# TencentARC/ViT-Lens

Measured on AMD Instinct MI355X. Metric: modality-pairs/sec (ViT-L, 224^2 patches), higher is better.
Workload: dtype bf16; 1 GPU; C3: ViT-L Lens(depth)->ViT + image + text tri-modal InfoNCE TRAINING step (fwd+bwd+AdamW), batch 1024/GPU in micro-batches of 256, first 4 blocks + adapter trainable; global_batch=1024, residual_dtype=bf16, accumulate=fp32, parallelism=dp1, gemm_cfg=-1, via=step, text_tower_operands=fp16, layernorm=folded into the GEMMs (frozen blocks), frozen_towers=second HIP stream beside the trainable tower's forward, backward=two halves of the micro-batches on two HIP streams

## Files before the change

include/vitlens_hip.h:

```cpp
#ifndef VITLENS_HIP_H
#define VITLENS_HIP_H

#include <stdint.h>

#ifdef __cplusplus
extern "C" {
#endif

#ifndef __HIP_PLATFORM_AMD__
typedef struct ihipStream_t* hipStream_t;
#endif

#define VL_EPI_BF16 0
#define VL_EPI_F32 1
#define VL_EPI_RES_F32 2
#define VL_EPI_RES_BF16 3
#define VL_EPI_GEGLU 5
#define VL_EPI_DGELU 6
#define VL_EPI_DGEGLU 7
#define VL_ACT_NONE 0
#define VL_ACT_GELU 1
#define VL_ACT_RELU 2
#define VL_ACT_GELU_DSAVE 4
#define VL_ACT_QGELU 5
#define VL_ACT_QGELU_DSAVE 6

#define VL_F32 0
#define VL_BF16 1
#define VL_F16 2

#define VL_GEMM_AUTO (-1)
#define VL_GEMM_PERSIST 8
#define VL_GEMM_PINGPONG 10

const char* vl_last_error(void);
#define VL_ABI_VERSION 607
int vl_version(void);

int vl_gemm_bf16(const void* A, const void* W, const float* bias, void* out, const void* res,
                 int M, int N, int K, int lda, int ldw, int ldo, float alpha, int epi, int act,
                 int cfg, hipStream_t stream);

int vl_gemm_splitk_accum_f32(const void* A, const void* W, float* out, int M, int N, int K, int lda, int ldw, long ldo,
                             float alpha, int splits, float* ws, hipStream_t stream);
int vl_gemm_tn_splitk_accum_f32(const void* At, const void* Bt, float* out, int M, int N, int K, int lda, int ldb, long ldo,
                                float alpha, int splits, float* ws, hipStream_t stream);
int vl_gemm_bf16_ex(const void* A, const void* W, const float* bias, void* out, const void* res, void* out2,
                    int M, int N, int K, int lda, int ldw, int ldo, float alpha, int epi, int act,
                    int res_div, int cfg, hipStream_t stream);

int vl_gemm_f16(const void* A, const void* W, const float* bias, void* out, const void* res, int M, int N, int K,
                int lda, int ldw, int ldo, float alpha, int epi, int act, hipStream_t stream);
int vl_attn_fwd_f16(const void* q, const void* k, const void* v, const long* strides, void* out, float* lse,
                    int B, int H, int Lq, int Lk, int dh, float qscale, int causal, hipStream_t stream);

int vl_gemm_f32(const float* A, const float* W, const float* bias, float* out, const float* res, int M, int N, int K,
                int lda, int ldw, int ldo, float alpha, int act, hipStream_t stream);
int vl_attn_fwd_f32(const float* q, const float* k, const float* v, const long* strides, float* out, float* lse,
                    int B, int H, int Lq, int Lk, int dh, float scale, int causal, hipStream_t stream);
int vl_im2col_f32(const float* x, float* patches, int N, int C, int H, int W, int kh, int kw, int sh, int sw,
                  int Kp, int transpose_hw, hipStream_t stream);
int vl_gemm_f32_ex(const float* A, const float* W, const float* bias, float* out, const float* res, int M, int N, int K,
                   int lda, int ldw, int ldo, float alpha, int act, int res_div, int res_pre, int geglu, hipStream_t stream);
int vl_knn_group_f32(const float* xyz, const int64_t* center_idx, int* nidx, float* patches, int B, int N, int G,
                     int k, int Kp, hipStream_t stream);
int vl_group_max_f32(const float* x, long ldx, float* out, long ldo, long groups, int M, int C, hipStream_t stream);
int vl_pad3_f32(const float* c, float* out, long R, int Kp, hipStream_t stream);

int vl_device_info(int device, char* arch, int arch_len, int* cus, int* clock_khz, long* hbm_bytes);

int vl_attn_fwd_bf16(const void* q, const void* k, const void* v, const long* strides, void* out, float* lse,
                     int B, int H, int Lq, int Lk, int dh, float qscale, int causal, hipStream_t stream);

int vl_gemm_main_rows(int M, int N);
int vl_gemm_lnfold_bf16(const void* A, const void* Wg, const float* bias_f, const float* ln_c, const float* ln_mean,
                        const float* ln_rstd, void* out, void* out2, int M, int N, int K, int lda, int ldw, int ldo, int act,
                        hipStream_t stream);
int vl_gemm_res_rowstats_bf16(const void* A, const void* W, const float* bias, void* out, const void* res, float* row_part,
                              int M, int N, int K, int lda, int ldw, int ldo, hipStream_t stream);
int vl_ln_row_stats(const float* row_part, int P, const void* x_bf16, long x_row_stride, int D, int m_main, int rows, float eps,
                    float* mean, float* rstd, const float* ln_w, const float* ln_b, void* y_left, long y_row_stride, int y_row0,
                    hipStream_t stream);

int vl_layernorm_fwd(const void* x, int x_dtype, long x_row_stride, const int64_t* row_index, long row_mul,
                     const float* w, const float* b, void* y, int y_dtype, long y_row_stride,
                     float* mean, float* rstd, int rows, int D, float eps, hipStream_t stream);

int vl_assemble_ln_pre(const void* tokens, int tok_dtype, const float* cls, const float* pos, const float* pos2,
                       const float* w, const float* b, void* y, int y_dtype, float* xpre, float* mean, float* rstd,
                       int B, int T, int D, float eps, hipStream_t stream);

int vl_l2_normalize(const float* x, float* y, void* y_bf16, float* norms, int rows, int D, float eps,
                    hipStream_t stream);
int vl_l2_normalize_bwd(const float* f, const float* df, const float* norms, float* dx, int rows, int D, float eps,
                        hipStream_t stream);

int vl_im2col_bf16(const float* x, void* patches, int N, int C, int H, int W, int kh, int kw, int sh, int sw,
                   int Kp, int transpose_hw, hipStream_t stream);

int vl_text_embed(const int64_t* ids, const float* tok_emb, const float* pos, void* out, int out_dtype,
                  int B, int L, int D, int vocab, hipStream_t stream);

int vl_cast_f32_bf16(const float* x, void* y, long n, hipStream_t stream);
int vl_add_rows(const void* x, int x_dtype, const float* table, void* y, int y_dtype, long rows, int T, int D,
                hipStream_t stream);
int vl_transpose_to_bf16(const void* in, int in_dtype, long ldi, int R, int C, void* out, long ldo, hipStream_t stream);
int vl_transpose_colsum_bf16(const void* in, int in_dtype, long ldi, int R, int C, void* out, long ldo,
                             float* colsum_out, float colsum_scale, float* ws, hipStream_t stream);

int vl_split_bf16x3(const float* x, void* out, long rows, int D, int pattern, hipStream_t stream);
int vl_ce_stats(const float* logits, long ld, int R, int C, int label_off, float* row_lse, float* col_lse,
                float* diag, float* col_ws, hipStream_t stream);
int vl_ce_loss_accum(const float* row_lse, const float* col_lse, const float* diag, int R, int C, int label_off,
                     float w_row, float w_col, float* loss_inout, hipStream_t stream);
int vl_ce_grad(const float* logits, long ld, int R, int C, int label_off, const float* row_lse, const float* col_lse,
               float w_row, float w_col, void* G, long ldg, void* GT, long ldgt, float logit_scale,
               float* dscale_inout, float* ws, hipStream_t stream);
long vl_ce_grad_ws_floats(int R, int C, long ldg, long ldgt);
int vl_ce_stats_masked(const float* logits, long ld, int R, int C, int label_off, float* row_lse, float* col_lse,
                       float* diag, float* col_ws, const float* sim, long ld_sim, float thres, hipStream_t stream);
int vl_ce_grad_masked(const float* logits, long ld, int R, int C, int label_off, const float* row_lse, const float* col_lse,
                      float w_row, float w_col, void* G, long ldg, void* GT, long ldgt, float logit_scale,
                      float* dscale_inout, float* ws, const float* sim, long ld_sim, float thres, hipStream_t stream);

int vl_layernorm_bwd(const void* dy, int dy_dtype, long dy_stride, const void* x, int x_dtype, long x_stride,
                     const float* mean, const float* rstd, const float* w, const float* dres, float* dx,
                     void* dx_bf16, long dx_stride, int rows, int D, hipStream_t stream);
int vl_layernorm_bwd_g(const void* dy, int dy_dtype, long dy_stride, const void* x, int x_dtype, long x_stride,
                       const float* mean, const float* rstd, const float* w, const void* dres, void* dx, int g_dtype,
                       void* dx_bf16, long dx_stride, int rows, int D, hipStream_t stream);
int vl_layernorm_bwd_sres(const void* dy, int dy_dtype, long dy_stride, const void* x, int x_dtype, long x_stride,
                          const float* mean, const float* rstd, const float* w, const void* dres, int dres_every,
                          long dres_stride, void* dx, int g_dtype, void* dx_bf16, long dx_stride, int rows, int D,
                          hipStream_t stream);
long vl_colreduce_ws_floats(int rows, int cols, int planes);
int vl_layernorm_bwd_params(const void* dy, int dy_dtype, long dy_stride, const void* x, int x_dtype, long x_stride,
                            const float* mean, const float* rstd, float* dw, float* db, int rows, int D,
                            float* ws, hipStream_t stream);
int vl_colsum(const void* a, int a_dtype, long lda, float* out, int rows, int cols, float scale, float* ws, hipStream_t stream);
int vl_gelu_bf16(const void* u, void* y, long n, hipStream_t stream);
int vl_geglu_bf16(const void* h, void* y, long rows, int n_out, hipStream_t stream);
int vl_attn_bwd_bf16(const void* q, const void* k, const void* v, const void* dO, const void* o, const long* strides,
                     const float* lse, float* delta, void* dq, void* dk, void* dv, long ld_dq, long ld_dkv,
                     int B, int H, int Lq, int Lk, int dh, float qscale, int causal, float scale, hipStream_t stream);
int vl_attn_bwd_fused_supported(int Lq, int Lk, int dh, int causal);
int vl_attn_bwd_fused_bf16(const void* q, const void* k, const void* v, const void* dO, const void* o, const long* strides,
                           const float* lse, void* dq, void* dk, void* dv, long ld_dq, long ld_dkv, int B, int H, int L, int dh,
                           float qscale, float scale, hipStream_t stream);
int vl_attn_fwd_q1(const void* q, const void* k, const void* v, const long* strides, void* out, long ld_out, float* lse,
                   int B, int H, int L, int dh, int qrow, float qscale, hipStream_t stream);
int vl_attn_bwd_q1(const void* q, const void* k, const void* v, const long* strides, const void* dO, long ld_do,
                   const void* o, long ld_o, const float* lse, void* dq, void* dk, void* dv, long ld_dq, long ld_dkv,
                   int B, int H, int L, int dh, int qrow, float qscale, float scale, hipStream_t stream);
int vl_kaldi_fbank(const float* wave, long wave_stride, int batch, long n_samples, const float* window, const float* banks,
                   float* out, int target_len, int win, int shift, int nfft, int nmel, float preemph, float mean, float std,
                   hipStream_t stream);
int vl_resample_sinc(const float* in, long in_stride, int batch, long n_in, const int* offsets, const float* taps, int o, int n,
                     int K, float* out, long out_stride, long out_first, long n_out, hipStream_t stream);
int vl_fbank_augment(const float* in, float* out, int batch, int T, int F, const void* params, float mean, float std,
                     hipStream_t stream);
int vl_fps(const float* xyz, const int64_t* start, int64_t* idx, float* centers, int B, int N, int G, hipStream_t stream);
int vl_pc_gather_normalize(const float* pts, const int64_t* idx, float* out, int B, int N, int G, int C, hipStream_t stream);
int vl_resample_h_u8(const uint8_t* src, long row_stride, int W, int C, int row0, int nrows, const int* bounds,
                     const int* kk, int ksize, int xout0, int nxout, uint8_t* dst, hipStream_t stream);
int vl_resample_v_u8_norm(const uint8_t* src, int W, int C, int row0, int nrows, const int* bounds, const int* kk,
                          int ksize, int yout0, int nyout, const float* mean, const float* stdv, float* out,
                          uint8_t* out_u8, hipStream_t stream);
int vl_resample_batch_u8_norm(const int64_t* desc, int n, int C, int crop_h, int crop_w, int max_nrows, const int* tables,
                              uint8_t* tmp, const float* mean, const float* stdv, float* out, hipStream_t stream);
int vl_resample_h_f32(const float* src, long row_stride, int W, int row0, int nrows, const int* bounds,
                      const float* weights, int ksize, int xout0, int nxout, int clamp_on, float clamp_lo,
                      float clamp_hi, float divide_by, float* dst, hipStream_t stream);
int vl_resample_v_f32_norm(const float* src, int W, int H, int row0, const int* bounds, const float* weights, int ksize,
                           int yout0, int nyout, float mean, float stdv, float* out, hipStream_t stream);
int vl_knn_group(const float* xyz, const int64_t* center_idx, int* nidx, void* patches, int B, int N, int G,
                 int k, int Kp, hipStream_t stream);
int vl_ball_group(const float* xyz, const float* feats, const int64_t* center_idx, int* idx, void* patches, int B, int N,
                  int S, int D, float radius2, int nsample, int Kp, hipStream_t stream);
int vl_group_max(const void* x, long ldx, void* out, int out_dtype, long ldo, long groups, int M, int C, hipStream_t stream);
int vl_pad3_bf16(const float* c, void* out, long R, int Kp, hipStream_t stream);
int vl_bn_stats(const void* x, long ldx, int R, int C, float* ws, int nchunk, float* mean, float* var,
                float* running_mean, float* running_var, float momentum, hipStream_t stream);
int vl_bn_stats_local(const void* x, long ldx, int R, int C, float* ws, int nchunk, float* local, hipStream_t stream);
int vl_bn_stats_merge(const float* gathered, int W, int C, float* mean, float* var, float* running_mean,
                      float* running_var, float momentum, int* total, hipStream_t stream);
int vl_bn_bwd_reduce(const void* dy, long lddy, const void* x, long ldx, const float* mean, const float* var,
                     const float* gamma, const float* beta, float eps, int relu, float* ws, int nchunk, float* dgamma,
                     float* dbeta, float* sums, int R, int C, hipStream_t stream);
int vl_bn_bwd_apply(const void* dy, long lddy, const void* x, long ldx, const float* mean, const float* var,
                    const float* gamma, const float* beta, float eps, int relu, const float* sums, const int* total,
                    void* dx, long lddx, int R, int C, hipStream_t stream);
int vl_bn_apply(const void* x, long ldx, const float* mean, const float* var, const float* gamma, const float* beta,
                float eps, int relu, void* out, long ldo, long R, int C, hipStream_t stream);
int vl_bn_bwd(const void* dy, long lddy, const void* x, long ldx, const float* mean, const float* var,
              const float* gamma, const float* beta, float eps, int relu, int train, float* ws, int nchunk,
              float* dgamma, float* dbeta, void* dx, long lddx, int R, int C, hipStream_t stream);
int vl_group_max_bwd(const void* f, long ldf, const void* dg, long lddg, const void* base, long ldb, void* out,
                     long ldo, long groups, int M, int C, hipStream_t stream);
int vl_group_sum(const void* x, long ldx, void* out, long ldo, long groups, int M, int C, hipStream_t stream);
int vl_adamw_step(float* p, const float* g, float* m, float* v, long n, float lr, float beta1, float beta2,
                  float eps, float weight_decay, int step, float grad_scale, hipStream_t stream);
long vl_sumsq_ws_floats(void);
int vl_sumsq_f32(const float* x, long n, float* out, float* ws, hipStream_t stream);
typedef struct vl_adamw_slot {
  float* p; const float* g; float* m; float* v;
  long n;
  float weight_decay;
// ... 24 lines not shown
```

vit-lens_amd/csrc/vl_attn.hip:

```cpp
#include "vl_attn_common.h"
#include "vitlens_hip.h"

namespace {
using namespace vlattn;

constexpr int KC = 288;
constexpr int VSP = KC + 8;
constexpr int NWMAX = 8;
constexpr float RESCALE_THR = 8.0f;

struct AttnP {
  TV q, k, v;
  float qscale;
  bf16_t* out;
  float* lse;
  int B, H, Lq, Lk, causal;
  int dh;
  VL_PROF_FIELD
  int lq_main;
};

template <int DH, bool TAILQ, bool MULTI, bool F16 = false, bool DMA = false>
__global__ void __launch_bounds__(NWMAX * 64, DH == 128 ? 2 : 4) attn_fwd_kernel(const AttnP p) {
  static_assert(!F16 || (!TAILQ && DH == 64), "half operands: head dim 64, no shared last row (the text tower's shape)");
  static_assert(!DMA || (DH == 64 && !MULTI && !F16), "LDS-DMA staging: head dim 64, one key chunk, bf16");
  constexpr int RB = DH * 2;
  constexpr int CH = RB / 16;
  constexpr int RSH = Rsh<DH>::v;
  constexpr bool PAD = DH == 128;
  constexpr int KS = DH / 16;
  constexpr int DT = DH / 32;
  extern __shared__ __attribute__((aligned(16))) unsigned char smem[];
  unsigned char* sK = smem;
  bf16_t* sV = (bf16_t*)(smem + KC * RB);
  float* sP = (float*)(sV + DH * VSP);
  float* sPart = sP + NWMAX * 32;
  bf16_t* sTailQ = (bf16_t*)(sPart + (KC / 32) * (2 + DH));

  const int b = blockIdx.z, h = blockIdx.y;
  const int tid = threadIdx.x, nthr = blockDim.x;
  const int lane = tid & 63;
  const int wid = __builtin_amdgcn_readfirstlane(tid >> 6);
  const int nwq = nthr >> 6;
  const int fr = lane & 31, fg = lane >> 5;
  const size_t bh = (size_t)b * p.H + h;
  const bf16_t* Kg = p.k.p + b * p.k.sb + h * p.k.sh;
  const bf16_t* Vg = p.v.p + b * p.v.sb + h * p.v.sh;
  const bf16_t* Qb = p.q.p + b * p.q.sb + h * p.q.sh;

  const int q0 = (blockIdx.x * nwq + wid) * 32;
  const bool wave_active = q0 < p.lq_main;
  int qrow = q0 + fr; if (qrow >= p.lq_main) qrow = p.lq_main - 1;
  const int qidx = q0 + fr;
  const int dhr = PAD ? p.dh : DH;
  const int nch = dhr >> 3;

  VL_PROF_STAMP(p, 0);
  u32x4 qraw[KS];
  {
    const bf16_t* Qg = Qb + (long)qrow * p.q.sr;
#pragma unroll
    for (int ks = 0; ks < KS; ++ks) {
      qraw[ks] = u32x4{0u, 0u, 0u, 0u};
      if (!PAD || ks * 2 + fg < nch) qraw[ks] = *(const u32x4*)(Qg + ks * 16 + fg * 8);
    }
  }
  [[maybe_unused]] u32x4 tailraw = {0u, 0u, 0u, 0u};
  if constexpr (TAILQ) {
    if constexpr (!PAD) tailraw = *(const u32x4*)(Qb + (long)(p.Lq - 1) * p.q.sr + (tid & (CH - 1)) * 8);
    else if (tid < nch) tailraw = *(const u32x4*)(Qb + (long)(p.Lq - 1) * p.q.sr + tid * 8);
  }
  unsigned char* const sVr = (unsigned char*)sV;
  auto vswz = [](int row) { const int x = (row >> 1) & 7; return ((x & 1) << 2) | (x >> 1); };
  if constexpr (DMA) {
    typedef __attribute__((address_space(3))) void* lds_p;
    const int nrows = ((p.Lk + 31) >> 5) << 5;
    const __amdgpu_buffer_rsrc_t rsK = __builtin_amdgcn_make_buffer_rsrc((void*)Kg, 0, 0x7ffffff0, 0x00020000);
    const __amdgpu_buffer_rsrc_t rsV = __builtin_amdgcn_make_buffer_rsrc((void*)Vg, 0, 0x7ffffff0, 0x00020000);
    for (int u = wid; u * 8 < p.Lk; u += nwq) {
      const int row = u * 8 + (lane >> 3), sl = lane & 7;
      if (row < p.Lk) {
        const unsigned offK = (unsigned)(row * (int)p.k.sr + ((sl ^ ((row >> 1) & 7)) << 3)) * 2u;
        const unsigned offV = (unsigned)(row * (int)p.v.sr + ((sl ^ vswz(row)) << 3)) * 2u;
        __builtin_amdgcn_raw_ptr_buffer_load_lds(rsK, (lds_p)(sK + u * 1024), 16, offK, 0, 0, 0);
        __builtin_amdgcn_raw_ptr_buffer_load_lds(rsV, (lds_p)(sVr + u * 1024), 16, offV, 0, 0, 0);
      }
    }
    for (int i = tid; i < (nrows - p.Lk) * 8; i += nthr)
      *(u32x4*)(sVr + (p.Lk + (i >> 3)) * 128 + ((i & 7) << 4)) = u32x4{0u, 0u, 0u, 0u};
    asm volatile("s_waitcnt vmcnt(0)" ::: "memory");
  } else {
  stage2<DH, KC, true, false, false, true>(StageSrc{sK, nullptr, Kg, p.k.sr, 1.f, nch}, StageSrc{nullptr, sV, Vg, p.v.sr, 1.f, nch},
                                           0, p.Lk, tid, nthr);
  }
  if constexpr (TAILQ) {
    if constexpr (!PAD) *(u32x4*)(sTailQ + (tid & (CH - 1)) * 8) = tailraw;
    else if (tid < CH) *(u32x4*)(sTailQ + tid * 8) = tailraw;
  }
  VL_PROF_STAMP(p, 1);
  [[maybe_unused]] const int li = lane & 15, lb3 = (li >> 3) & 1;
  [[maybe_unused]] const unsigned aTr = (unsigned)((fg * 4 + (li >> 2)) * 128) +
                                        (((unsigned)(((lane >> 4) & 1) * 2 + ((li >> 1) & 1)) ^ (unsigned)((lb3 << 2) | fg)) << 4) + (unsigned)((li & 1) << 3);
  auto trV = [&](int tile, int c, int t) {
    typedef __attribute__((ext_vector_type(4))) short s16x4;
    typedef __attribute__((address_space(3))) s16x4* lds_s16x4;
    struct { s16x4 lo, hi; } f;
    const unsigned a = (aTr + (unsigned)(tile * 4096)) ^ (unsigned)(t * 64);
    f.lo = __builtin_amdgcn_ds_read_tr16_b64_v4i16((lds_s16x4)(sVr + a + c * 2048));
    f.hi = __builtin_amdgcn_ds_read_tr16_b64_v4i16((lds_s16x4)(sVr + (a ^ 32u) + c * 2048 + 1024));
    return __builtin_bit_cast(bf16x8, f);
  };
  bf16x8 qf[KS];
#pragma unroll
  for (int ks = 0; ks < KS; ++ks)
    qf[ks] = __builtin_bit_cast(bf16x8, p.qscale != 1.0f ? scale_x8<F16>(qraw[ks], p.qscale) : qraw[ks]);

  float m_run = 0.f;
  vl_f32x2 l2 = {0.f, 0.f};
  f32x16 negm;
  f32x16 o[DT];
#pragma unroll
  for (int r = 0; r < 16; ++r) negm[r] = 0.f;
#pragma unroll
  for (int t = 0; t < DT; ++t)
#pragma unroll
    for (int r = 0; r < 16; ++r) o[t][r] = 0.f;
  bool first = true;

  auto tail_partials = [&]() {
    if constexpr (TAILQ) {
    const int qT = p.Lq - 1;
    const int ntile = (p.Lk + 31) >> 5;
    const int ksw = (fr >> RSH) & (CH - 1);
    bf16x8 qa[KS];
#pragma unroll
    for (int ks = 0; ks < KS; ++ks) {
#pragma unroll
      for (int e = 0; e < 8; ++e) qa[ks][e] = (__bf16)0.f;
      if (fr == 0) {
        u32x4 raw = *(const u32x4*)(sTailQ + ks * 16 + fg * 8);
        if (p.qscale != 1.0f) raw = scale_bf16x8(raw, p.qscale);
        qa[ks] = __builtin_bit_cast(bf16x8, raw);
      }
    }
    for (int kt = wid; kt < ntile; kt += nwq) {
      f32x16 st;
#pragma unroll
      for (int r = 0; r < 16; ++r) st[r] = 0.f;
      const unsigned char* kbase = sK + (kt * 32 + fr) * RB;
#pragma unroll
      for (int ks = 0; ks < KS; ++ks)
        st = __builtin_amdgcn_mfma_f32_32x32x16_bf16(qa[ks], *(const bf16x8*)(kbase + (((ks * 2 + fg) ^ ksw) * 16)), st, 0, 0, 0);
      const bool valid = fg == 0 && kt * 32 + fr < p.Lk;
      const float sv = valid ? st[0] : -INFINITY;
      const float mw = wave_max_dpp(sv);
      const float pw = valid ? __builtin_amdgcn_exp2f(sv - mw) : 0.f;
      const float lw = wave_sum_dpp(pw);
      float* myP = sP + wid * 32;
      if (fg == 0) myP[fr] = pw;
      __builtin_amdgcn_fence(__ATOMIC_RELEASE, "wavefront");
      __builtin_amdgcn_wave_barrier();
      __builtin_amdgcn_fence(__ATOMIC_ACQUIRE, "wavefront");
      f32x16 ot[DT];
#pragma unroll
      for (int t = 0; t < DT; ++t)
#pragma unroll
        for (int r = 0; r < 16; ++r) ot[t][r] = 0.f;
#pragma unroll
      for (int c = 0; c < 2; ++c) {
        bf16x8 pa;
#pragma unroll
        for (int e = 0; e < 8; ++e) pa[e] = (__bf16)0.f;
        if (fr == 0) {
          const f32x4 lo = *(const f32x4*)(myP + c * 16 + fg * 4);
          const f32x4 hi = *(const f32x4*)(myP + c * 16 + 8 + fg * 4);
#pragma unroll
          for (int e = 0; e < 4; ++e) { pa[e] = (__bf16)lo[e]; pa[4 + e] = (__bf16)hi[e]; }
        }
#pragma unroll
        for (int t = 0; t < DT; ++t)
          ot[t] = __builtin_amdgcn_mfma_f32_32x32x16_bf16(
              pa, DMA ? trV(kt, c, t) : *(const bf16x8*)(sV + (t * 32 + fr) * VSP + kt * 32 + c * 16 + fg * 8), ot[t], 0, 0, 0);
      }
      __builtin_amdgcn_wave_barrier();
      float* part = sPart + kt * (2 + DH);
      if (lane == 0) { part[0] = mw; part[1] = lw; }
      if (fg == 0) {
#pragma unroll
        for (int t = 0; t < DT; ++t) part[2 + t * 32 + fr] = ot[t][0];
      }
    }
    }
  };
  auto tail_merge = [&]() {
    if constexpr (TAILQ) {
      const int qT = p.Lq - 1;
      const int ntile = (p.Lk + 31) >> 5;
      if (wid == 0) {
        float M = -INFINITY;
        for (int kt = 0; kt < ntile; ++kt) M = fmaxf(M, sPart[kt * (2 + DH)]);
        for (int d = lane; d < dhr; d += 64) {
          float L = 0.f, acc = 0.f;
          for (int kt = 0; kt < ntile; ++kt) {
            const float* part = sPart + kt * (2 + DH);
            const float w = __builtin_amdgcn_exp2f(part[0] - M);
            L = fmaf(part[1], w, L);
            acc = fmaf(part[2 + d], w, acc);
          }
          p.out[((size_t)b * p.Lq + qT) * (p.H * dhr) + h * dhr + d] = f2bf(acc / L);
          if (p.lse && d == 0) p.lse[bh * p.Lq + qT] = (M + __log2f(L)) * 0.6931471805599453f;
        }
      }
    }
  };
  const int q_hi = q0 + 31;
  const int blk_q_hi = min(p.lq_main - 1, (int)(blockIdx.x * nwq + nwq) * 32 - 1);

  for (int kc0 = 0; kc0 < (MULTI ? p.Lk : 1); kc0 += KC) {
    if (MULTI && p.causal && kc0 > blk_q_hi) break;
    if constexpr (MULTI) {
      if (kc0 > 0) {
        __syncthreads();
        stage2<DH, KC, true, false, false, true, 1>(StageSrc{sK, nullptr, Kg, p.k.sr, 1.f, nch},
                                                    StageSrc{nullptr, sV, Vg, p.v.sr, 1.f, nch}, kc0, p.Lk, tid, nthr);
      }
    }
    __syncthreads();
    VL_PROF_STAMP(p, 2);
    if constexpr (TAILQ) { tail_partials(); __syncthreads(); }
    if (!wave_active) continue;

    int ntile = (min(p.Lk - kc0, KC) + 31) >> 5;
    if (p.causal) ntile = min(ntile, ((q_hi - kc0) >> 5) + 1);
    const int ksw = (fr >> RSH) & (CH - 1);
    for (int kt = 0; kt < ntile; ++kt) {
      const unsigned char* kbase = sK + (kt * 32 + fr) * RB;
      bf16x8 kf[KS];
#pragma unroll
      for (int ks = 0; ks < KS; ++ks) kf[ks] = *(const bf16x8*)(kbase + (((ks * 2 + fg) ^ ksw) * 16));
      f32x16 s = mfma32<F16>(kf[0], qf[0], negm);
#pragma unroll
      for (int ks = 1; ks < KS; ++ks) s = mfma32<F16>(kf[ks], qf[ks], s);
      bf16x8 vf0[DT];
#pragma unroll
      for (int t = 0; t < DT; ++t) {
        if constexpr (DMA) vf0[t] = trV(kt, 0, t);
        else vf0[t] = *(const bf16x8*)(sV + (t * 32 + fr) * VSP + kt * 32 + fg * 8);
      }
      const int key0 = kc0 + kt * 32 + fg * 4;
      const bool need_mask = (key0 - fg * 4 + 32 > p.Lk) || (p.causal && key0 - fg * 4 + 31 > q0);
      if (need_mask) {
#pragma unroll
        for (int r = 0; r < 16; ++r) {
          const int key = key0 + (r & 3) + 8 * (r >> 2);
          if (key >= p.Lk || (p.causal && key > qidx)) s[r] = -INFINITY;
        }
      }
      float mx = fmaxf(fmaxf(s[0], s[1]), s[2]);
#pragma unroll
      for (int r = 3; r < 15; r += 2) mx = fmaxf(fmaxf(mx, s[r]), s[r + 1]);
      mx = fmaxf(mx, s[15]);
      mx = xhalf_max(mx);
      if (__builtin_amdgcn_ballot_w64(first || mx > RESCALE_THR) != 0) {
        const float d = first ? mx : fmaxf(mx, 0.f);
        const float alpha = first ? 0.f : __builtin_amdgcn_exp2f(-d);
        m_run += d;
#pragma unroll
        for (int r = 0; r < 16; ++r) { s[r] -= d; negm[r] -= d; }
#pragma unroll
        for (int t = 0; t < DT; ++t)
#pragma unroll
          for (int r = 0; r < 16; ++r) o[t][r] *= alpha;
        l2 *= alpha;
        first = false;
      }
      float pv[16];
#pragma unroll
      for (int r = 0; r < 16; ++r) pv[r] = __builtin_amdgcn_exp2f(s[r]);
      {
        vl_f32x2 a0 = {pv[0], pv[1]}, a1 = {pv[2], pv[3]}, a2 = {pv[4], pv[5]}, a3 = {pv[6], pv[7]};
        const vl_f32x2 a4 = {pv[8], pv[9]}, a5 = {pv[10], pv[11]}, a6 = {pv[12], pv[13]}, a7 = {pv[14], pv[15]};
        a0 += a4; a1 += a5; a2 += a6; a3 += a7;
        a0 += a2; a1 += a3;
        l2 += a0 + a1;
      }
      bf16x8 vf1[DT];
#pragma unroll
      for (int t = 0; t < DT; ++t) {
        if constexpr (DMA) vf1[t] = trV(kt, 1, t);
        else vf1[t] = *(const bf16x8*)(sV + (t * 32 + fr) * VSP + kt * 32 + 16 + fg * 8);
      }
      {
        const bf16x8 pf = pack8x<F16>(pv);
#pragma unroll
        for (int t = 0; t < DT; ++t) o[t] = mfma32<F16>(vf0[t], pf, o[t]);
      }
      {
        const bf16x8 pf = pack8x<F16>(pv + 8);
#pragma unroll
        for (int t = 0; t < DT; ++t) o[t] = mfma32<F16>(vf1[t], pf, o[t]);
      }
    }
  }

  VL_PROF_STAMP(p, 3);
  if (wave_active) {
    const float l_tot = xhalf_sum(l2[0] + l2[1]);
    const float inv = 1.0f / l_tot;
    store_rows_t<DT, F16>(o, inv, p.out + ((size_t)b * p.Lq + qrow) * (p.H * dhr) + h * dhr, fg, qidx < p.lq_main, nch);
    if (p.lse && fg == 0 && qidx < p.lq_main)
      p.lse[bh * p.Lq + qidx] = (m_run + __log2f(l_tot)) * 0.6931471805599453f;
  }

  VL_PROF_STAMP(p, 4);
  tail_merge();
  VL_PROF_STAMP(p, 5);
}

}

extern "C" int vl_set_error(const char* msg);

template <int DH, bool TAILQ, bool MULTI, bool F16 = false, bool DMA = false>
static int launch_fwd(const AttnP& p, int gx, int nwq, hipStream_t stream) {
  const size_t smem = (size_t)KC * DH * 2 + (size_t)DH * VSP * 2 + (size_t)NWMAX * 32 * 4 + (size_t)(KC / 32) * (2 + DH) * 4 +
                      (size_t)DH * 2;
  static const hipError_t attr = hipFuncSetAttribute((const void*)attn_fwd_kernel<DH, TAILQ, MULTI, F16, DMA>,
                                                     hipFuncAttributeMaxDynamicSharedMemorySize, (int)smem);
  if (attr != hipSuccess) return vl_set_error(hipGetErrorString(attr));
  hipLaunchKernelGGL((attn_fwd_kernel<DH, TAILQ, MULTI, F16, DMA>), dim3(gx, p.H, p.B), dim3(nwq * 64), smem, stream, p);
  const hipError_t e = hipGetLastError();
  return e == hipSuccess ? 0 : vl_set_error(hipGetErrorString(e));
}

extern "C" int vl_attn_fwd_bf16(const void* q, const void* k, const void* v, const long* strides, void* out, float* lse,
                                int B, int H, int Lq, int Lk, int dh, float qscale, int causal, hipStream_t stream) {
  if (B <= 0 || H <= 0 || Lq <= 0 || Lk <= 0) return vl_set_error("vl_attn_fwd_bf16: empty problem");
  if (dh != 32 && dh != 64 && !(dh > 64 && dh <= 128 && (dh & 7) == 0))
    return vl_set_error("vl_attn_fwd_bf16: head dim must be 32, 64, or a multiple of 8 in (64, 128] (run zero-padded to 128)");
  if (!strides) return vl_set_error("vl_attn_fwd_bf16: strides required");
  for (int i = 0; i < 9; ++i)
    if (strides[i] & 7) return vl_set_error("vl_attn_fwd_bf16: operand strides must be multiples of 8 elements (16-byte rows)");
  if ((((uintptr_t)q) | ((uintptr_t)k) | ((uintptr_t)v)) & 15) return vl_set_error("vl_attn_fwd_bf16: operands must be 16-byte aligned");
  AttnP p{TV{(const bf16_t*)q, strides[0], strides[1], strides[2]}, TV{(const bf16_t*)k, strides[3], strides[4], strides[5]},
          TV{(const bf16_t*)v, strides[6], strides[7], strides[8]}, qscale, (bf16_t*)out, lse, B, H, Lq, Lk, causal, dh,
#ifdef VL_ATTN_PROF
          vl_attn_prof_buf,
#endif
          Lq};
  const bool tailq = (Lq % 32 == 1) && Lq > 32 && Lq - 1 <= NWMAX * 32 && Lk <= KC && (!causal || Lk <= Lq);
  if (tailq) p.lq_main = Lq - 1;
  const int qtiles = (p.lq_main + 31) / 32;
  const int nwq = qtiles < NWMAX ? qtiles : NWMAX;
  const int gx = (qtiles + nwq - 1) / nwq;
  const bool multi = Lk > KC;
#define VL_FWD(DHV)                                                                  \
  (tailq ? launch_fwd<DHV, true, false>(p, gx, nwq, stream)                          \
         : (multi ? launch_fwd<DHV, false, true>(p, gx, nwq, stream) : launch_fwd<DHV, false, false>(p, gx, nwq, stream)))
  if (dh == 64 && !multi)
    return tailq ? launch_fwd<64, true, false, false, true>(p, gx, nwq, stream) : launch_fwd<64, false, false, false, true>(p, gx, nwq, stream);
  return dh == 64 ? VL_FWD(64) : (dh == 32 ? VL_FWD(32) : VL_FWD(128));
#undef VL_FWD
}

extern "C" int vl_attn_fwd_f16(const void* q, const void* k, const void* v, const long* strides, void* out, float* lse,
                               int B, int H, int Lq, int Lk, int dh, float qscale, int causal, hipStream_t stream) {
  if (B <= 0 || H <= 0 || Lq <= 0 || Lk <= 0) return vl_set_error("vl_attn_fwd_f16: empty problem");
  if (dh != 64) return vl_set_error("vl_attn_fwd_f16: head dim must be 64");
  if (Lk > KC) return vl_set_error("vl_attn_fwd_f16: at most 288 keys");
  if (!strides) return vl_set_error("vl_attn_fwd_f16: strides required");
  for (int i = 0; i < 9; ++i)
    if (strides[i] & 7) return vl_set_error("vl_attn_fwd_f16: operand strides must be multiples of 8 elements (16-byte rows)");
  if ((((uintptr_t)q) | ((uintptr_t)k) | ((uintptr_t)v)) & 15) return vl_set_error("vl_attn_fwd_f16: operands must be 16-byte aligned");
  AttnP p{TV{(const bf16_t*)q, strides[0], strides[1], strides[2]}, TV{(const bf16_t*)k, strides[3], strides[4], strides[5]},
          TV{(const bf16_t*)v, strides[6], strides[7], strides[8]}, qscale, (bf16_t*)out, lse, B, H, Lq, Lk, causal, dh,
#ifdef VL_ATTN_PROF
          vl_attn_prof_buf,
#endif
          Lq};
  const int qtiles = (Lq + 31) / 32;
  const int nwq = qtiles < NWMAX ? qtiles : NWMAX;
  const int gx = (qtiles + nwq - 1) / nwq;
  return launch_fwd<64, false, false, true>(p, gx, nwq, stream);
}
```

vit-lens_amd/csrc/vl_attn_common.h:

```cpp
#pragma once
#include "vl_common.h"

#ifdef VL_ATTN_PROF
extern "C" long* vl_attn_prof_buf;
#define VL_PROF_FIELD long* prof;
#define VL_PROF_STAMP(p, i)                                                                                    \
  do {                                                                                                         \
    if ((p).prof && threadIdx.x == 0)                                                                          \
      (p).prof[((blockIdx.z * gridDim.y + blockIdx.y) * gridDim.x + blockIdx.x) * 8 + (i)] = __builtin_amdgcn_s_memtime(); \
  } while (0)
#else
#define VL_PROF_FIELD
#define VL_PROF_STAMP(p, i) do { } while (0)
#endif

namespace vlattn {

struct TV {
  const bf16_t* p;
  long sb, sh, sr;
};

__device__ __forceinline__ int vpos16(int j) { return (j & 3) | ((j & 4) << 1) | ((j & 8) >> 1); }

__device__ __forceinline__ u32x4 scale_bf16x8(u32x4 v, float s) {
#pragma unroll
  for (int e = 0; e < 4; ++e)
    v[e] = pack2bf(bf2f((bf16_t)(v[e] & 0xffffu)) * s, bf2f((bf16_t)(v[e] >> 16)) * s);
  return v;
}

template <bool F16>
__device__ __forceinline__ u32x4 scale_x8(u32x4 v, float s) {
  if constexpr (F16) {
#pragma unroll
    for (int e = 0; e < 4; ++e) v[e] = pack2h(h2f((uint16_t)(v[e] & 0xffffu)) * s, h2f((uint16_t)(v[e] >> 16)) * s);
    return v;
  } else {
    return scale_bf16x8(v, s);
  }
}
template <bool F16>
__device__ __forceinline__ f32x16 mfma32(bf16x8 a, bf16x8 b, f32x16 c) {
  if constexpr (F16) return __builtin_amdgcn_mfma_f32_32x32x16_f16(__builtin_bit_cast(f16x8, a), __builtin_bit_cast(f16x8, b), c, 0, 0, 0);
  else return __builtin_amdgcn_mfma_f32_32x32x16_bf16(a, b, c, 0, 0, 0);
}

struct StageSrc {
  unsigned char* rows;
  bf16_t* t;
  const bf16_t* src;
  long sr;
  float scale;
  int nch = 0;
};

template <int DH> struct Rsh { static constexpr int v = DH == 32 ? 2 : (DH == 64 ? 1 : 0); };

template <int DH, int NR, bool ROWS, bool TRANS>
__device__ __forceinline__ void stage_write(const StageSrc& m, int i, u32x4 a, u32x4 bq) {
  constexpr int RB = DH * 2, CH = RB / 16, RSH = Rsh<DH>::v, TS = NR + 8;
  const int rp = i / CH, c = i % CH;
  const int rl = 2 * rp;
  if (m.scale != 1.0f) { a = scale_bf16x8(a, m.scale); bq = scale_bf16x8(bq, m.scale); }
  if constexpr (ROWS) {
    *(u32x4*)(m.rows + rl * RB + ((c ^ ((rl >> RSH) & (CH - 1))) * 16)) = a;
    *(u32x4*)(m.rows + (rl + 1) * RB + ((c ^ (((rl + 1) >> RSH) & (CH - 1))) * 16)) = bq;
  }
  if constexpr (TRANS) {
    unsigned int* dst = (unsigned int*)(m.t + (c * 8) * TS + (rl & ~15) + vpos16(rl & 15));
#pragma unroll
    for (int w = 0; w < 4; ++w) {
      dst[(2 * w) * (TS / 2)] = (a[w] & 0xffffu) | (bq[w] << 16);
      dst[(2 * w + 1) * (TS / 2)] = (a[w] >> 16) | (bq[w] & 0xffff0000u);
    }
  }
}

template <int DH, int NR, bool ROWS0, bool TRANS0, bool ROWS1, bool TRANS1, int U = 3>
__device__ __forceinline__ void stage2(const StageSrc& m0, const StageSrc& m1, int row0, int L, int tid, int nthr) {
  constexpr int CH = DH / 8, NP = (NR / 2) * CH;
  for (int base = 0; base < NP; base += U * nthr) {
    u32x4 a0[U], b0[U], a1[U], b1[U];
#pragma unroll
    for (int u = 0; u < U; ++u) {
      const int i = base + u * nthr + tid;
      const int rp = i / CH, c = i % CH;
      const int row = row0 + 2 * rp;
      const u32x4 z = {0u, 0u, 0u, 0u};
      a0[u] = z; b0[u] = z; a1[u] = z; b1[u] = z;
      const unsigned o0 = ((unsigned)row * (unsigned)m0.sr + c * 8) * 2u, o1 = ((unsigned)row * (unsigned)m1.sr + c * 8) * 2u;
      const bool cok = DH != 128 || c < m0.nch;
      if (i < NP && row < L && cok) {
        a0[u] = *(const u32x4*)((const unsigned char*)m0.src + o0);
        a1[u] = *(const u32x4*)((const unsigned char*)m1.src + o1);
      }
      if (i < NP && row + 1 < L && cok) {
        b0[u] = *(const u32x4*)((const unsigned char*)m0.src + (o0 + (unsigned)m0.sr * 2u));
        b1[u] = *(const u32x4*)((const unsigned char*)m1.src + (o1 + (unsigned)m1.sr * 2u));
      }
    }
#pragma unroll
    for (int u = 0; u < U; ++u) {
      const int i = base + u * nthr + tid;
      if (i >= NP) continue;
      stage_write<DH, NR, ROWS0, TRANS0>(m0, i, a0[u], b0[u]);
      stage_write<DH, NR, ROWS1, TRANS1>(m1, i, a1[u], b1[u]);
    }
  }
}

__device__ __forceinline__ float xhalf_max(float v) {
  const unsigned u = __builtin_bit_cast(unsigned, v);
  auto r = __builtin_amdgcn_permlane32_swap(u, u, false, false);
  const unsigned lo = r[0], hi = r[1];
  return fmaxf(__builtin_bit_cast(float, lo), __builtin_bit_cast(float, hi));
}
__device__ __forceinline__ float xhalf_sum(float v) {
  const unsigned u = __builtin_bit_cast(unsigned, v);
  auto r = __builtin_amdgcn_permlane32_swap(u, u, false, false);
  const unsigned lo = r[0], hi = r[1];
  return __builtin_bit_cast(float, lo) + __builtin_bit_cast(float, hi);
}
template <int CTRL>
__device__ __forceinline__ float dpp_f(float v) {
  return __builtin_bit_cast(float, __builtin_amdgcn_update_dpp(0, __builtin_bit_cast(int, v), CTRL, 0xf, 0xf, true));
}
__device__ __forceinline__ float lane_f(float v, int lane) {
  return __builtin_bit_cast(float, __builtin_amdgcn_readlane(__builtin_bit_cast(int, v), lane));
}
__device__ __forceinline__ float wave_max_dpp(float v) {
  v = fmaxf(v, dpp_f<0xB1>(v)); v = fmaxf(v, dpp_f<0x4E>(v)); v = fmaxf(v, dpp_f<0x141>(v)); v = fmaxf(v, dpp_f<0x140>(v));
  return fmaxf(fmaxf(lane_f(v, 0), lane_f(v, 16)), fmaxf(lane_f(v, 32), lane_f(v, 48)));
}
__device__ __forceinline__ float wave_sum_dpp(float v) {
  v += dpp_f<0xB1>(v); v += dpp_f<0x4E>(v); v += dpp_f<0x141>(v); v += dpp_f<0x140>(v);
  return (lane_f(v, 0) + lane_f(v, 16)) + (lane_f(v, 32) + lane_f(v, 48));
}

template <int DT, bool F16 = false>
__device__ __forceinline__ void store_rows_t(const f32x16* acc, float mul, bf16_t* dst, int fg, bool valid, int npiece = 4 * DT) {
  auto pk = [](float a, float b) { if constexpr (F16) return pack2h(a, b); else return pack2bf(a, b); };
#pragma unroll
  for (int t = 0; t < DT; ++t)
#pragma unroll
    for (int pp = 0; pp < 2; ++pp) {
      unsigned ev[2], od[2];
#pragma unroll
      for (int j = 0; j < 2; ++j) {
        ev[j] = pk(acc[t][(2 * pp) * 4 + 2 * j] * mul, acc[t][(2 * pp) * 4 + 2 * j + 1] * mul);
        od[j] = pk(acc[t][(2 * pp + 1) * 4 + 2 * j] * mul, acc[t][(2 * pp + 1) * 4 + 2 * j + 1] * mul);
      }
      auto r0 = __builtin_amdgcn_permlane32_swap(ev[0], od[0], false, false);
      auto r1 = __builtin_amdgcn_permlane32_swap(ev[1], od[1], false, false);
      const unsigned w0 = r0[0], w1 = r1[0], w2 = r0[1], w3 = r1[1];
      const u32x4 w = {w0, w1, w2, w3};
      if (valid && t * 4 + 2 * pp + fg < npiece) *(u32x4*)(dst + t * 32 + (2 * pp + fg) * 8) = w;
    }
}

template <int DH>
__device__ __forceinline__ bf16x8 frag_rows(const unsigned char* base, int row, int ks, int fg) {
  constexpr int RB = DH * 2, CH = RB / 16, RSH = Rsh<DH>::v;
  return *(const bf16x8*)(base + row * RB + (((ks * 2 + fg) ^ ((row >> RSH) & (CH - 1))) * 16));
}
template <int NR>
__device__ __forceinline__ bf16x8 frag_t(const bf16_t* base, int d, int tile, int c, int fg) {
  return *(const bf16x8*)(base + d * (NR + 8) + tile * 32 + c * 16 + fg * 8);
}

__device__ __forceinline__ f32x16 zero16() {
  f32x16 z;
#pragma unroll
  for (int r = 0; r < 16; ++r) z[r] = 0.f;
  return z;
}
__device__ __forceinline__ bf16x8 zero_bf8() {
  bf16x8 z;
#pragma unroll
  for (int e = 0; e < 8; ++e) z[e] = (__bf16)0.f;
  return z;
}
__device__ __forceinline__ bf16x8 pack8(const float* v) {
  bf16x8 r;
#pragma unroll
  for (int e = 0; e < 8; ++e) r[e] = (__bf16)v[e];
  return r;
}
template <bool F16>
__device__ __forceinline__ bf16x8 pack8x(const float* v) {
  if constexpr (F16) {
    f16x8 r;
#pragma unroll
    for (int e = 0; e < 8; ++e) r[e] = (_Float16)v[e];
    return __builtin_bit_cast(bf16x8, r);
  } else {
    return pack8(v);
  }
}
__device__ __forceinline__ float dot8(bf16x8 a, bf16x8 b, float acc) {
#pragma unroll
  for (int e = 0; e < 8; ++e) acc = fmaf((float)a[e], (float)b[e], acc);
  return acc;
}

}
```

vit-lens_amd/vitlens_hip/_lib.py:

```python
import ctypes as C
import os

_HERE = os.path.dirname(os.path.abspath(__file__))
_LIB = None


class LibraryNotBuilt(ImportError):
    pass


def lib_path() -> str:
    return os.path.join(_HERE, "libvitlens_hip.so")


P, I, L, F = C.c_void_p, C.c_int, C.c_long, C.c_float

ABI_VERSION = 607

SIGNATURES = {
    "vl_version": [],
    "vl_device_info": [I, C.c_char_p, I, C.POINTER(I), C.POINTER(I), C.POINTER(L)],
    "vl_gemm_bf16": [P, P, P, P, P, I, I, I, I, I, I, F, I, I, I, P],
    "vl_gemm_splitk_accum_f32": [P, P, P, I, I, I, I, I, L, F, I, P, P],
    "vl_gemm_tn_splitk_accum_f32": [P, P, P, I, I, I, I, I, L, F, I, P, P],
    "vl_attn_fwd_bf16": [P, P, P, P, P, P, I, I, I, I, I, F, I, P],
    "vl_gemm_f16": [P, P, P, P, P, I, I, I, I, I, I, F, I, I, P],
    "vl_gemm_f32": [P, P, P, P, P, I, I, I, I, I, I, F, I, P],
    "vl_attn_fwd_f32": [P, P, P, P, P, P, I, I, I, I, I, F, I, P],
    "vl_im2col_f32": [P, P, I, I, I, I, I, I, I, I, I, I, P],
    "vl_gemm_f32_ex": [P, P, P, P, P, I, I, I, I, I, I, F, I, I, I, I, P],
    "vl_knn_group_f32": [P, P, P, P, I, I, I, I, I, P],
    "vl_group_max_f32": [P, L, P, L, L, I, I, P],
    "vl_pad3_f32": [P, P, L, I, P],
    "vl_attn_fwd_f16": [P, P, P, P, P, P, I, I, I, I, I, F, I, P],
    "vl_layernorm_fwd": [P, I, L, P, L, P, P, P, I, L, P, P, I, I, F, P],
    "vl_gemm_main_rows": [I, I],
    "vl_gemm_lnfold_bf16": [P, P, P, P, P, P, P, P, I, I, I, I, I, I, I, P],
    "vl_gemm_res_rowstats_bf16": [P, P, P, P, P, P, I, I, I, I, I, I, P],
    "vl_ln_row_stats": [P, I, P, L, I, I, I, F, P, P, P, P, P, L, I, P],
    "vl_assemble_ln_pre": [P, I, P, P, P, P, P, P, I, P, P, P, I, I, I, F, P],
    "vl_l2_normalize": [P, P, P, P, I, I, F, P],
    "vl_l2_normalize_bwd": [P, P, P, P, I, I, F, P],
    "vl_im2col_bf16": [P, P, I, I, I, I, I, I, I, I, I, I, P],
    "vl_text_embed": [P, P, P, P, I, I, I, I, I, P],
    "vl_cast_f32_bf16": [P, P, L, P],
    "vl_add_rows": [P, I, P, P, I, L, I, I, P],
    "vl_transpose_to_bf16": [P, I, L, I, I, P, L, P],
    "vl_transpose_colsum_bf16": [P, I, L, I, I, P, L, P, F, P, P],
    "vl_split_bf16x3": [P, P, L, I, I, P],
    "vl_ce_stats": [P, L, I, I, I, P, P, P, P, P],
    "vl_ce_loss_accum": [P, P, P, I, I, I, F, F, P, P],
    "vl_ce_grad": [P, L, I, I, I, P, P, F, F, P, L, P, L, F, P, P, P],
    "vl_ce_grad_ws_floats": [I, I, L, L],
    "vl_ce_stats_masked": [P, L, I, I, I, P, P, P, P, P, L, F, P],
    "vl_ce_grad_masked": [P, L, I, I, I, P, P, F, F, P, L, P, L, F, P, P, P, L, F, P],
    "vl_gemm_bf16_ex": [P, P, P, P, P, P, I, I, I, I, I, I, F, I, I, I, I, P],
    "vl_kaldi_fbank": [P, L, I, L, P, P, P, I, I, I, I, I, F, F, F, P],
    "vl_resample_sinc": [P, L, I, L, P, P, I, I, I, P, L, L, L, P],
    "vl_fbank_augment": [P, P, I, I, I, P, F, F, P],
    "vl_fps": [P, P, P, P, I, I, I, P],
    "vl_pc_gather_normalize": [P, P, P, I, I, I, I, P],
    "vl_resample_h_u8": [P, L, I, I, I, I, P, P, I, I, I, P, P],
    "vl_resample_v_u8_norm": [P, I, I, I, I, P, P, I, I, I, P, P, P, P, P],
    "vl_resample_batch_u8_norm": [P, I, I, I, I, I, P, P, P, P, P, P],
    "vl_resample_h_f32": [P, L, I, I, I, P, P, I, I, I, I, F, F, F, P, P],
    "vl_resample_v_f32_norm": [P, I, I, I, P, P, I, I, I, F, F, P, P],
    "vl_knn_group": [P, P, P, P, I, I, I, I, I, P],
    "vl_ball_group": [P, P, P, P, P, I, I, I, I, F, I, I, P],
    "vl_group_max": [P, L, P, I, L, L, I, I, P],
    "vl_pad3_bf16": [P, P, L, I, P],
    "vl_bn_stats": [P, L, I, I, P, I, P, P, P, P, F, P],
    "vl_bn_stats_local": [P, L, I, I, P, I, P, P],
    "vl_bn_stats_merge": [P, I, I, P, P, P, P, F, P, P],
    "vl_bn_bwd_reduce": [P, L, P, L, P, P, P, P, F, I, P, I, P, P, P, I, I, P],
    "vl_bn_bwd_apply": [P, L, P, L, P, P, P, P, F, I, P, P, P, L, I, I, P],
    "vl_bn_apply": [P, L, P, P, P, P, F, I, P, L, L, I, P],
    "vl_bn_bwd": [P, L, P, L, P, P, P, P, F, I, I, P, I, P, P, P, L, I, I, P],
    "vl_group_max_bwd": [P, L, P, L, P, L, P, L, L, I, I, P],
    "vl_group_sum": [P, L, P, L, L, I, I, P],
    "vl_layernorm_bwd": [P, I, L, P, I, L, P, P, P, P, P, P, L, I, I, P],
    "vl_layernorm_bwd_g": [P, I, L, P, I, L, P, P, P, P, P, I, P, L, I, I, P],
    "vl_layernorm_bwd_sres": [P, I, L, P, I, L, P, P, P, P, I, L, P, I, P, L, I, I, P],
    "vl_colreduce_ws_floats": [I, I, I],
    "vl_layernorm_bwd_params": [P, I, L, P, I, L, P, P, P, P, I, I, P, P],
    "vl_colsum": [P, I, L, P, I, I, F, P, P],
    "vl_gelu_bf16": [P, P, L, P],
    "vl_geglu_bf16": [P, P, L, I, P],
    "vl_attn_bwd_bf16": [P, P, P, P, P, P, P, P, P, P, P, L, L, I, I, I, I, I, F, I, F, P],
    "vl_attn_bwd_fused_supported": [I, I, I, I],
    "vl_attn_bwd_fused_bf16": [P, P, P, P, P, P, P, P, P, P, L, L, I, I, I, I, F, F, P],
    "vl_attn_fwd_q1": [P, P, P, P, P, L, P, I, I, I, I, I, F, P],
    "vl_attn_bwd_q1": [P, P, P, P, P, L, P, L, P, P, P, P, L, L, I, I, I, I, I, F, F, P],
    "vl_adamw_step": [P, P, P, P, L, F, F, F, F, F, I, F, P],
    "vl_sumsq_ws_floats": [],
    "vl_sumsq_f32": [P, L, P, P, P],
    "vl_adamw_multi_step": [P, I, F, F, F, F, I, F, F, P, P, P],
    "vl_clamp_scalar": [P, F, F, P],
    "vl_axpy_f32": [P, P, F, L, P],
    "vl_scale_exp_f32": [P, P, L, P, F, P],
    "vl_batch_rowsum": [P, P, I, I, I, L, L, P],
    "vl_comm_unique_id": [P],
    "vl_comm_create": [C.POINTER(P), P, I, I],
    "vl_comm_destroy": [P],
    "vl_allgather_embed": [P, P, P, L, P],
    "vl_reducescatter_grad": [P, P, P, L, P],
    "vl_allreduce_grad": [P, P, L, P],
}


_RET = {"vl_colreduce_ws_floats": L, "vl_ce_grad_ws_floats": L, "vl_sumsq_ws_floats": L}


def load_library():
    global _LIB
    if _LIB is not None:
        return _LIB
    path = lib_path()
    if not os.path.exists(path):
        raise LibraryNotBuilt(
            f"{path} is missing: build it with `python -c 'import __graft_entry__ as g; g.build()'` "
            "or `make -C vit-lens_amd/csrc` (hipcc --offload-arch=gfx950). No CPU/eager fallback exists.")
    lib = C.CDLL(path)
    lib.vl_last_error.restype = C.c_char_p
    lib.vl_last_error.argtypes = []
    for name, args in SIGNATURES.items():
        fn = getattr(lib, name)
        fn.argtypes = args
        fn.restype = _RET.get(name, I)
    got = int(lib.vl_version())
    if got != ABI_VERSION:
        raise RuntimeError(f"{path} reports ABI version {got}, this binding was written for {ABI_VERSION} "
                           "(include/vitlens_hip.h: VL_ABI_VERSION): rebuild the library (`make -C vit-lens_amd/csrc`)")
    _LIB = lib
    return lib


def check(status: int):
    if status != 0:
        raise RuntimeError("libvitlens_hip: " + load_library().vl_last_error().decode())
```

vit-lens_amd/vitlens_hip/engine.py:

```python
from dataclasses import dataclass
from typing import Dict, Optional

import os

import torch

from . import ops


@dataclass
class TowerCfg:
    width: int = 1024
    layers: int = 24
    heads: int = 16
    mlp_ratio: float = 4.0
    patch: int = 14
    image_size: int = 224
    embed_dim: int = 768
    in_chans: int = 3
    quick_gelu: bool = False


@dataclass
class TextCfg:
# ... 104 lines not shown

def run_blocks(blocks, ws: _Workspace, B, L, D, H, causal=False, cfg=-1, fold=None, quick_gelu=False, pooled_only=False):
    dh = D // H
    prune = prune_last_ok(D, H, ws.x.dtype, L, pooled_only, causal)
    act = ops.mlp_act(quick_gelu)
    res_epi = ops.EPI_RES_F32 if ws.x.dtype == torch.float32 else ops.EPI_RES_BF16
    if fold is None:
        fold = LN_FOLD
    can_fold = bool(fold) and ws.x.dtype == torch.bfloat16 and ws.part is not None
    folded = [can_fold and "in_f" in w for w in blocks]
    mm = 0
    r_in = r_fc = 0
    if any(folded):
        r_in, r_fc = ops.fold_rows(ws.x, ws.qkv, 3 * D), ops.fold_rows(ws.x, ws.hid, ws.hid.shape[1])
    for i, w in enumerate(blocks):
        nxt = i + 1 < len(blocks) and folded[i + 1]
        pruned = prune and i + 1 == len(blocks)
        if folded[i]:
            k_in = dict(ln_w=w["ln1_w"], ln_b=w["ln1_b"], h_left=ws.h, h_row0=r_in) if mm <= r_in else {}
            ops.ln_row_stats(ws.part, ws.x, mm, ws.mean, ws.rstd, **k_in)
            ops.gemm_lnfold(ws.x, w["in_f"], ws.mean, ws.rstd, ws.qkv, w["in_w"], w["in_b"], w["ln1_w"], w["ln1_b"], ws.h, cfg=cfg,
                            h_ready=bool(k_in))
            if pruned:
                _pooled_block_tail(w, ws, B, L, D, H, act, cfg)
                break
            ops.attn_fwd(ws.q, ws.k, ws.v, ws.a, causal=causal, qscale=dh ** -0.5 * ops.LOG2E)
            mm = ops.gemm_res_rowstats(ws.a, w["out_w"], w["out_b"], ws.x, ws.x, ws.part, cfg=cfg)
            k_fc = dict(ln_w=w["ln2_w"], ln_b=w["ln2_b"], h_left=ws.h, h_row0=r_fc) if mm <= r_fc else {}
            ops.ln_row_stats(ws.part, ws.x, mm, ws.mean, ws.rstd, **k_fc)
            ops.gemm_lnfold(ws.x, w["fc_f"], ws.mean, ws.rstd, ws.hid, w["fc_w"], w["fc_b"], w["ln2_w"], w["ln2_b"], ws.h,
                            act=act, cfg=cfg, h_ready=bool(k_fc))
        else:
            ops.layernorm(ws.x, w["ln1_w"], w["ln1_b"], ws.h, B * L, D)
            ops.gemm(ws.h, w["in_w"], w["in_b"], out=ws.qkv, epi=ops.EPI_BF16, cfg=cfg)
            if pruned:
                _pooled_block_tail(w, ws, B, L, D, H, act, cfg)
                break
            ops.attn_fwd(ws.q, ws.k, ws.v, ws.a, causal=causal, qscale=dh ** -0.5 * ops.LOG2E)
            ops.gemm(ws.a, w["out_w"], w["out_b"], out=ws.x, res=ws.x, epi=res_epi, cfg=cfg)
            ops.layernorm(ws.x, w["ln2_w"], w["ln2_b"], ws.h, B * L, D)
            ops.gemm(ws.h, w["fc_w"], w["fc_b"], out=ws.hid, epi=ops.EPI_BF16, act=act, cfg=cfg)
        if nxt:
            mm = ops.gemm_res_rowstats(ws.hid, w["proj_w"], w["proj_b"], ws.x, ws.x, ws.part, cfg=cfg)
        else:
            ops.gemm(ws.hid, w["proj_w"], w["proj_b"], out=ws.x, res=ws.x, epi=res_epi, cfg=cfg)
            mm = 0


def _hi_lo(w: torch.Tensor, device):
    w = w.detach().float().to(device)
    hi = w.bfloat16()
    lo = (w - hi.float()).bfloat16()
    return hi.contiguous(), lo.contiguous()


def prep_block_wsplit(sd: Dict[str, torch.Tensor], p: str, device) -> Dict[str, torch.Tensor]:
    blk = prep_block(sd, p, device)
    for key, name in (("in_w", "attn.in_proj_weight"), ("fc_w", "mlp.c_fc.weight")):
        hi, lo = _hi_lo(sd[p + name], device)
        blk[key + "2"] = torch.cat([hi, lo], dim=1).contiguous()
    for key, name in (("out_w", "attn.out_proj.weight"), ("proj_w", "mlp.c_proj.weight")):
        blk[key], blk[key + "_lo"] = _hi_lo(sd[p + name], device)
    return blk


def run_blocks_wsplit(blocks, ws: "_Workspace", B, L, D, H, causal=False, cfg=-1, quick_gelu=False):
    dh = D // H
    act = ops.mlp_act(quick_gelu)
    h2 = ws.h2
    for w in blocks:
        ops.layernorm(ws.x, w["ln1_w"], w["ln1_b"], h2[:, :D], B * L, D)
        ops.layernorm(ws.x, w["ln1_w"], w["ln1_b"], h2[:, D:], B * L, D)
        ops.gemm(h2, w["in_w2"], w["in_b"], out=ws.qkv, epi=ops.EPI_BF16, cfg=cfg)
        ops.attn_fwd(ws.q, ws.k, ws.v, ws.a, causal=causal, qscale=dh ** -0.5 * ops.LOG2E)
        ops.gemm(ws.a, w["out_w"], w["out_b"], out=ws.x, res=ws.x, epi=ops.EPI_RES_F32, cfg=cfg)
        ops.gemm(ws.a, w["out_w_lo"], None, out=ws.x, res=ws.x, epi=ops.EPI_RES_F32, cfg=cfg)
        ops.layernorm(ws.x, w["ln2_w"], w["ln2_b"], h2[:, :D], B * L, D)
        ops.layernorm(ws.x, w["ln2_w"], w["ln2_b"], h2[:, D:], B * L, D)
        ops.gemm(h2, w["fc_w2"], w["fc_b"], out=ws.hid, epi=ops.EPI_BF16, act=act, cfg=cfg)
        ops.gemm(ws.hid, w["proj_w"], w["proj_b"], out=ws.x, res=ws.x, epi=ops.EPI_RES_F32, cfg=cfg)
        ops.gemm(ws.hid, w["proj_w_lo"], None, out=ws.x, res=ws.x, epi=ops.EPI_RES_F32, cfg=cfg)


class VitEngine:

    def __init__(self, sd, prefix: str, cfg: TowerCfg, device, res_dtype=torch.float32, gemm_cfg: int = -1,
                 n_tokens: Optional[int] = None):
        self.cfg, self.device, self.res_dtype, self.gemm_cfg = cfg, torch.device(device), res_dtype, gemm_cfg
        self.prefix = prefix
        D = cfg.width
        self.cls = _dev(sd[prefix + "class_embedding"], device)
        self.pos = _dev(sd[prefix + "positional_embedding"], device)
        self.T = self.pos.shape[0] - 1
        self.ln_pre = (_dev(sd[prefix + "ln_pre.weight"], device), _dev(sd[prefix + "ln_pre.bias"], device))
        self.ln_post = (_dev(sd[prefix + "ln_post.weight"], device), _dev(sd[prefix + "ln_post.bias"], device))
        self.projT = _dev(sd[prefix + "proj"].t(), device, torch.bfloat16) if prefix + "proj" in sd else None
        self.blocks = [prep_block(sd, f"{prefix}transformer.resblocks.{i}.", device) for i in range(cfg.layers)]
        self.conv_w = None
        if prefix + "conv1.weight" in sd:
            self.conv_w = conv_weight_as_gemm(sd[prefix + "conv1.weight"], device)
        self._ws = {}

    def update_params(self, sd, names):
        p, dev = self.prefix, self.device
        top = {n for n in names if not n.startswith("transformer.resblocks.")}
        if "class_embedding" in top:
            self.cls.copy_(sd[p + "class_embedding"])
        if "positional_embedding" in top:
            self.pos.copy_(sd[p + "positional_embedding"])
        for nm, pair in (("ln_pre", self.ln_pre), ("ln_post", self.ln_post)):
            if nm + ".weight" in top or nm + ".bias" in top:
                pair[0].copy_(sd[p + nm + ".weight"]); pair[1].copy_(sd[p + nm + ".bias"])
        if "proj" in top and self.projT is not None:
            self.projT.copy_(sd[p + "proj"].t())
        if "conv1.weight" in top and self.conv_w is not None:
            self.conv_w.copy_(conv_weight_as_gemm(sd[p + "conv1.weight"], dev))
        for l in sorted({int(n.split(".")[2]) for n in names if n.startswith("transformer.resblocks.")}):
            copy_tree(self.blocks[l], prep_block(sd, f"{p}transformer.resblocks.{l}.", dev))

    def workspace(self, B, L):
        key = (B, L)
        if key not in self._ws:
            self._ws[key] = _Workspace(B, L, self.cfg.width, self.cfg.heads, int(self.cfg.width * self.cfg.mlp_ratio),
                                       self.device, self.res_dtype)
        return self._ws[key]

    def patch_tokens(self, image: torch.Tensor) -> torch.Tensor:
        p = self.cfg.patch
        cols, gh, gw = ops.im2col(image.contiguous().float(), p, p, p, p, self.conv_w.shape[1])
        return ops.gemm(cols, self.conv_w, None, epi=ops.EPI_BF16, cfg=self.gemm_cfg)

    def trunk(self, tokens: torch.Tensor, B: int, pos2: Optional[torch.Tensor] = None, use_orig_pos=True):
        cfg = self.cfg
        D, T = cfg.width, tokens.shape[0] // B
        L = T + 1
        ws = self.workspace(B, L)
        pos = self.pos if use_orig_pos else torch.zeros_like(self.pos)
        ops.assemble_ln_pre(tokens, self.cls, pos, pos2, self.ln_pre[0], self.ln_pre[1], ws.x, B, T, D)
        run_blocks(self.blocks, ws, B, L, D, cfg.heads, causal=False, cfg=self.gemm_cfg, quick_gelu=cfg.quick_gelu, pooled_only=True)
        pooled = torch.empty(B, D, device=self.device, dtype=torch.bfloat16)
        if self.projT is None:
            pooled = torch.empty(B, D, device=self.device, dtype=torch.float32)
        ops.layernorm(ws.x, self.ln_post[0], self.ln_post[1], pooled, B, D, x_row_stride=L * D)
        if self.projT is None:
            return pooled
        return ops.gemm(pooled, self.projT, None, epi=ops.EPI_F32, cfg=self.gemm_cfg)

    def encode_image(self, image: torch.Tensor, normalize: bool = False) -> torch.Tensor:
        B = image.shape[0]
        f = self.trunk(self.patch_tokens(image), B)
        return ops.l2_normalize(f) if normalize else f


def prep_block_f16(sd: Dict[str, torch.Tensor], p: str, device) -> Dict[str, torch.Tensor]:
    hf = torch.float16
    return {
        "ln1_w": _dev(sd[p + "ln_1.weight"], device), "ln1_b": _dev(sd[p + "ln_1.bias"], device),
        "in_w": _dev(sd[p + "attn.in_proj_weight"], device, hf), "in_b": _dev(sd[p + "attn.in_proj_bias"], device),
        "out_w": _dev(sd[p + "attn.out_proj.weight"], device, hf), "out_b": _dev(sd[p + "attn.out_proj.bias"], device),
        "ln2_w": _dev(sd[p + "ln_2.weight"], device), "ln2_b": _dev(sd[p + "ln_2.bias"], device),
        "fc_w": _dev(sd[p + "mlp.c_fc.weight"], device, hf), "fc_b": _dev(sd[p + "mlp.c_fc.bias"], device),
        "proj_w": _dev(sd[p + "mlp.c_proj.weight"], device, hf), "proj_b": _dev(sd[p + "mlp.c_proj.bias"], device),
    }


class _WorkspaceF16:

    def __init__(self, B, L, D, H, device):
        hf = torch.float16
        self.rows = B * L
        self.Mp = (self.rows + 255) // 256 * 256
        self.Bp = (B + 255) // 256 * 256
        z = lambda *shape, dt=hf: torch.zeros(*shape, device=device, dtype=dt)
        self.x = z(self.Mp, D, dt=torch.float32)
        self.h, self.qkv, self.a, self.hid = z(self.Mp, D), z(self.Mp, 3 * D), z(self.Mp, D), z(self.Mp, 4 * D)
        dh = D // H
        hv = lambda i: ops.heads_view(self.qkv, B, L, H, dh, i * D)
        self.q, self.k, self.v = hv(0), hv(1), hv(2)
        self.pooled = z(self.Bp, D)


class TextEngine:

    def __init__(self, sd, cfg: TextCfg, device, res_dtype=torch.float32, gemm_cfg: int = -1, wsplit: Optional[bool] = None,
                 arith: str = "f16"):
        self.cfg, self.device, self.gemm_cfg = cfg, torch.device(device), gemm_cfg
        if wsplit is not None:
            arith = "bf16x2" if wsplit else "bf16"
        if arith not in ("f16", "bf16x2", "bf16"):
            raise ValueError(f"TextEngine: arith must be 'f16', 'bf16x2' or 'bf16', got {arith!r}")
        if arith == "f16" and (cfg.width % 256 or cfg.width < 512 or cfg.width // cfg.heads != 64 or cfg.embed_dim % 256
                               or cfg.context_length > 288):
            arith = "bf16x2"
        self.arith = arith
        self.wsplit = arith == "bf16x2"
        self.res_dtype = res_dtype if arith == "bf16" else torch.float32
        self.tok = _dev(sd["token_embedding.weight"], device)
        self.pos = _dev(sd["positional_embedding"], device)
        self.ln_final = (_dev(sd["ln_final.weight"], device), _dev(sd["ln_final.bias"], device))
        if arith == "f16":
            self.projT = _dev(sd["text_projection"].t(), device, torch.float16)
            self.blocks = [prep_block_f16(sd, f"transformer.resblocks.{i}.", device) for i in range(cfg.layers)]
        elif self.wsplit:
            hi, lo = _hi_lo(sd["text_projection"].t(), device)
            self.projT = torch.cat([hi, lo], dim=1).contiguous()
            self.blocks = [prep_block_wsplit(sd, f"transformer.resblocks.{i}.", device) for i in range(cfg.layers)]
        else:
            self.projT = _dev(sd["text_projection"].t(), device, torch.bfloat16)
            self.blocks = [_prep_block_plain(sd, f"transformer.resblocks.{i}.", device) for i in range(cfg.layers)]
        self._ws = {}

    def _encode_f16(self, text: torch.Tensor) -> torch.Tensor:
        cfg = self.cfg
        B, L = text.shape
        D, H = cfg.width, cfg.heads
        key = ("f16", B, L)
        if key not in self._ws:
            self._ws[key] = _WorkspaceF16(B, L, D, H, self.device)
        ws = self._ws[key]
        rows = ws.rows
        ops.text_embed(text, self.tok, self.pos, ws.x[:rows])
        eot = text.argmax(dim=-1).contiguous()
        qs = (D // H) ** -0.5 * ops.LOG2E
        act = ops.mlp_act(cfg.quick_gelu)
        for w in self.blocks:
            ops.layernorm(ws.x, w["ln1_w"], w["ln1_b"], ws.h, rows, D)
            ops.gemm_f16(ws.h, w["in_w"], w["in_b"], out=ws.qkv)
            ops.attn_fwd(ws.q, ws.k, ws.v, ws.a, causal=True, qscale=qs)
            ops.gemm_f16(ws.a, w["out_w"], w["out_b"], out=ws.x, res=ws.x, epi=ops.EPI_RES_F32)
            ops.layernorm(ws.x, w["ln2_w"], w["ln2_b"], ws.h, rows, D)
            ops.gemm_f16(ws.h, w["fc_w"], w["fc_b"], out=ws.hid, act=act)
            ops.gemm_f16(ws.hid, w["proj_w"], w["proj_b"], out=ws.x, res=ws.x, epi=ops.EPI_RES_F32)
        ops.layernorm(ws.x, self.ln_final[0], self.ln_final[1], ws.pooled, B, D, x_row_stride=D, row_index=eot, row_mul=L)
        f = torch.zeros(ws.Bp, self.projT.shape[0], device=self.device, dtype=torch.float32)
        ops.gemm_f16(ws.pooled, self.projT, None, out=f, res=f, epi=ops.EPI_RES_F32)
        return f[:B]

    def encode_text(self, text: torch.Tensor, normalize: bool = False) -> torch.Tensor:
        cfg = self.cfg
        B, L = text.shape
        D = cfg.width
        text = text.to(self.device).contiguous()
        if self.arith == "f16":
            f = self._encode_f16(text)
            return ops.l2_normalize(f) if normalize else f.contiguous()
        key = (B, L)
        if key not in self._ws:
            self._ws[key] = _Workspace(B, L, D, cfg.heads, 4 * D, self.device, self.res_dtype)
        ws = self._ws[key]
        ops.text_embed(text, self.tok, self.pos, ws.x)
        eot = text.argmax(dim=-1).contiguous()
        if self.wsplit:
            if not hasattr(ws, "h2"):
                ws.h2 = torch.empty(B * L, 2 * D, device=self.device, dtype=torch.bfloat16)
            run_blocks_wsplit(self.blocks, ws, B, L, D, cfg.heads, causal=True, cfg=self.gemm_cfg, quick_gelu=cfg.quick_gelu)
            pooled = torch.empty(B, 2 * D, device=self.device, dtype=torch.bfloat16)
            for half in (pooled[:, :D], pooled[:, D:]):
                ops.layernorm(ws.x, self.ln_final[0], self.ln_final[1], half, B, D, x_row_stride=D, row_index=eot, row_mul=L)
        else:
            run_blocks(self.blocks, ws, B, L, D, cfg.heads, causal=True, cfg=self.gemm_cfg, fold=False, quick_gelu=cfg.quick_gelu)
            pooled = torch.empty(B, D, device=self.device, dtype=torch.bfloat16)
            ops.layernorm(ws.x, self.ln_final[0], self.ln_final[1], pooled, B, D, x_row_stride=D, row_index=eot, row_mul=L)
        f = ops.gemm(pooled, self.projT, None, epi=ops.EPI_F32, cfg=self.gemm_cfg)
        return ops.l2_normalize(f) if normalize else f


@dataclass
class LensCfg:
    modality: str = "depth"
    perceiver_identity: bool = True
    depth: int = 2
    self_per_cross: int = 3
    num_latents: int = 256
    latent_dim: int = 1024
    input_chan: int = 1024
    cross_heads: int = 1
    cross_dim_head: int = 64
    latent_heads: int = 16
    latent_dim_head: int = 64
    audio_fstride: int = 10
    audio_tstride: int = 10
    audio_mel_bins: int = 128
    audio_target_length: int = 512
    pc_num_group: int = 512
    pc_group_size: int = 32
    pc_encoder_dims: int = 256
    pc_trans_dim: int = 384
    pc_tokenizer: str = "pointbert"
    pc_radius: float = 0.2
    pc_in_dim: int = 3
    use_orig_pos: bool = True
    disable_adapter_pos: bool = False
    eeg_chans: int = 128
    eeg_time_len: int = 512
    eeg_window_size: int = 1
    eeg_stride: int = 1
    weight_tie_layers: bool = False


def _interleave_geglu(w: torch.Tensor, b: torch.Tensor):
    half = w.shape[0] // 2
    wi = torch.stack([w[:half], w[half:]], dim=1).reshape(w.shape[0], w.shape[1])
    bi = torch.stack([b[:half], b[half:]], dim=1).reshape(-1)
    return wi, bi


def prep_lens_attn(sd, p, device, packed_self: bool):
    bf = torch.bfloat16
    d = {"to_out_w": _dev(sd[p + "to_out.weight"], device, bf), "to_out_b": _dev(sd[p + "to_out.bias"], device)}
    if packed_self:
        d["qkv_w"] = _dev(torch.cat([sd[p + "to_q.weight"], sd[p + "to_kv.weight"]], 0), device, bf)
    else:
        d["q_w"] = _dev(sd[p + "to_q.weight"], device, bf)
        d["kv_w"] = _dev(sd[p + "to_kv.weight"], device, bf)
    return d


def prep_lens_ff(sd, p, device):
    w0, b0 = _interleave_geglu(sd[p + "net.0.weight"].detach().float(), sd[p + "net.0.bias"].detach().float())
    return {"w0": _dev(w0, device, torch.bfloat16), "b0": _dev(b0, device),
            "w2": _dev(sd[p + "net.2.weight"], device, torch.bfloat16), "b2": _dev(sd[p + "net.2.bias"], device)}


class PerceiverEngine:

    def __init__(self, sd, prefix: str, cfg: LensCfg, device, gemm_cfg=-1):
        self.cfg, self.device, self.gemm_cfg = cfg, torch.device(device), gemm_cfg
        self.latents = _dev(sd[prefix + "latents"], device)
        ln = lambda q: (_dev(sd[q + ".weight"], device), _dev(sd[q + ".bias"], device))
        self.layers = []
        for i in range(cfg.depth):
            if cfg.weight_tie_layers and i >= 2:
                self.layers.append(self.layers[1])
                continue
            q = f"{prefix}layers.{i}."
            lay = {"x_norm": ln(q + "0.norm"), "x_norm_ctx": ln(q + "0.norm_context"),
                   "x_attn": prep_lens_attn(sd, q + "0.fn.", device, False),
                   "x_ff_norm": ln(q + "1.norm"), "x_ff": prep_lens_ff(sd, q + "1.fn.", device), "selfs": []}
            for j in range(cfg.self_per_cross):
                r = f"{q}2.{j}."
                lay["selfs"].append({"norm": ln(r + "0.norm"), "attn": prep_lens_attn(sd, r + "0.fn.", device, True),
                                     "ff_norm": ln(r + "1.norm"), "ff": prep_lens_ff(sd, r + "1.fn.", device)})
            self.layers.append(lay)
        self._ws = {}

    def update_params(self, sd, prefix: str):
        fresh = PerceiverEngine(sd, prefix, self.cfg, self.device, self.gemm_cfg)
        self.latents.copy_(fresh.latents)
        copy_tree(self.layers, fresh.layers)

    def _workspace(self, B, Tc):
        key = (B, Tc)
        if key in self._ws:
            return self._ws[key]
        c, dev, bf = self.cfg, self.device, torch.bfloat16
        n, D = c.num_latents, c.latent_dim
        f = lambda *s, dt=bf: torch.empty(*s, device=dev, dtype=dt)
        ws = {
            "x": f(B * n, D, dt=torch.float32), "h": f(B * n, D), "ctx": f(B * Tc, c.input_chan),
            "xq2": f(B * n, c.cross_heads * c.cross_dim_head), "xkv2": f(B * Tc, 2 * c.cross_heads * c.cross_dim_head),
            "xa": f(B * n, c.cross_heads * c.cross_dim_head),
            "sqkv2": f(B * n, 3 * c.latent_heads * c.latent_dim_head),
            "sa": f(B * n, c.latent_heads * c.latent_dim_head), "hid": f(B * n, 4 * D),
        }
        xi, si = c.cross_heads * c.cross_dim_head, c.latent_heads * c.latent_dim_head
        ws["xq"] = ops.heads_view(ws["xq2"], B, n, c.cross_heads, c.cross_dim_head)
        ws["xk"] = ops.heads_view(ws["xkv2"], B, Tc, c.cross_heads, c.cross_dim_head)
        ws["xv"] = ops.heads_view(ws["xkv2"], B, Tc, c.cross_heads, c.cross_dim_head, xi)
        for i, nm in enumerate(("sq", "sk", "sv")):
            ws[nm] = ops.heads_view(ws["sqkv2"], B, n, c.latent_heads, c.latent_dim_head, i * si)
        self._ws[key] = ws
        return ws

    def _ff(self, ws, norm, ff, rows, D):
        ops.layernorm(ws["x"], norm[0], norm[1], ws["h"], rows, D)
        ops.gemm(ws["h"], ff["w0"], ff["b0"], out=ws["hid"], epi=ops.EPI_GEGLU, cfg=self.gemm_cfg)
        ops.gemm(ws["hid"], ff["w2"], ff["b2"], out=ws["x"], res=ws["x"], epi=ops.EPI_RES_F32, cfg=self.gemm_cfg)

    def forward(self, data: torch.Tensor, B: int) -> torch.Tensor:
        c = self.cfg
        Tc, n, D = data.shape[0] // B, c.num_latents, c.latent_dim
        ws = self._workspace(B, Tc)
        ws["x"].view(B, n, D).copy_(self.latents)
        rows = B * n
        for lay in self.layers:
            a = lay["x_attn"]
            ops.layernorm(ws["x"], lay["x_norm"][0], lay["x_norm"][1], ws["h"], rows, D)
            ops.layernorm(data, lay["x_norm_ctx"][0], lay["x_norm_ctx"][1], ws["ctx"], B * Tc, c.input_chan)
            ops.gemm(ws["h"], a["q_w"], None, out=ws["xq2"], epi=ops.EPI_BF16, cfg=self.gemm_cfg)
            ops.gemm(ws["ctx"], a["kv_w"], None, out=ws["xkv2"], epi=ops.EPI_BF16, cfg=self.gemm_cfg)
            ops.attn_fwd(ws["xq"], ws["xk"], ws["xv"], ws["xa"], qscale=c.cross_dim_head ** -0.5 * ops.LOG2E)
            ops.gemm(ws["xa"], a["to_out_w"], a["to_out_b"], out=ws["x"], res=ws["x"], epi=ops.EPI_RES_F32, cfg=self.gemm_cfg)
            self._ff(ws, lay["x_ff_norm"], lay["x_ff"], rows, D)
            for sl in lay["selfs"]:
                a = sl["attn"]
                ops.layernorm(ws["x"], sl["norm"][0], sl["norm"][1], ws["h"], rows, D)
# ... 97 lines not shown
```

vit-lens_amd/vitlens_hip/ops.py:

```python
import ctypes as C
import threading

import torch

from ._lib import load_library, check

F32, BF16, F16 = 0, 1, 2
EPI_BF16, EPI_F32, EPI_RES_F32, EPI_RES_BF16, EPI_GEGLU, EPI_DGELU, EPI_DGEGLU = 0, 1, 2, 3, 5, 6, 7
ACT_NONE, ACT_GELU, ACT_RELU = 0, 1, 2
ACT_GELU_DSAVE = 4
ACT_QGELU = 5
ACT_QGELU_DSAVE = 6


def mlp_act(quick_gelu: bool, dsave: bool = False) -> int:
    if quick_gelu:
        return ACT_QGELU_DSAVE if dsave else ACT_QGELU
    return ACT_GELU_DSAVE if dsave else ACT_GELU
LOG2E = 1.4426950408889634

_lib = load_library()


def _stream():
# ... 198 lines not shown
    if mm < M:
        gemm(a[mm:], w, b, out=out[mm:], res=res[mm:], epi=EPI_RES_BF16, cfg=_leftover_cfg(M - mm, N, cfg) if mm else cfg)
    return mm


def fold_rows(x, out, N):
    return _fold_rows(x, out, N, x.shape[1])


def ln_row_stats(part, x, m_main, mean, rstd, eps=1e-5, ln_w=None, ln_b=None, h_left=None, h_row0=None):
    rows, D = x.shape
    if h_left is not None:
        if h_row0 is None or h_row0 < m_main or h_left.dtype != torch.bfloat16 or h_left.shape[0] < rows - h_row0:
            raise ValueError("ln_row_stats: h_left needs h_row0 >= m_main and a bf16 buffer of at least rows - h_row0 rows")
    check(_lib.vl_ln_row_stats(_p(part) if m_main else None, D // 64, _p(x), x.stride(0), D, m_main, rows, float(eps), _p(mean),
                               _p(rstd), _p(ln_w), _p(ln_b), _p(h_left), h_left.stride(0) if h_left is not None else 0,
                               int(h_row0 or 0), _stream()))


def logits_gemm(xb, yb, scale):
    Cn = yb.shape[0]
    Cp = (Cn + 3) // 4 * 4
    if Cp != Cn:
        yb = torch.cat([yb, torch.zeros(Cp - Cn, yb.shape[1], device=yb.device, dtype=yb.dtype)], 0)
    out = gemm(xb, yb, None, epi=EPI_F32, alpha=scale)
    return out if Cp == Cn else out[:, :Cn]


def gemm_dw(dyt, xt, g, cfg=-1, alpha=1.0):
    _chk2d(dyt, "dyt", torch.bfloat16); _chk2d(xt, "xt", torch.bfloat16); _chk2d(g, "g", torch.float32)
    M, K = dyt.shape
    N = xt.shape[0]
    nk = K // 64
    if K % 64 == 0 and M % 256 == 0 and N % 256 == 0 and nk >= 64:
        t256 = (M // 256) * (N // 256)
        for splits in (1, 2, 4, 8, 16):
            if nk % splits == 0 and t256 * splits >= 192 and nk // splits >= 16:
                ws = torch.empty(splits * M * N, device=g.device, dtype=torch.float32)
                check(_lib.vl_gemm_splitk_accum_f32(_p(dyt), _p(xt), _p(g), M, N, K, dyt.stride(0), xt.stride(0), g.stride(0),
                                                    float(alpha), splits, _p(ws), _stream()))
                return g
    tiles = ((M + 127) // 128) * ((N + 127) // 128)
    if K % 64 == 0 and tiles * 2 <= 256 and nk >= 32:
        splits = max(1, min(512 // tiles, nk // 16))
        if splits > 1:
            ws = torch.empty(splits * M * N, device=g.device, dtype=torch.float32)
            check(_lib.vl_gemm_splitk_accum_f32(_p(dyt), _p(xt), _p(g), M, N, K, dyt.stride(0), xt.stride(0), g.stride(0),
                                                float(alpha), splits, _p(ws), _stream()))
            return g
    return gemm(dyt, xt, None, out=g, res=g, epi=EPI_RES_F32, cfg=cfg, alpha=alpha)


def gemm_dw_tn(dy, x, g, alpha=1.0):
    if dy.dtype != torch.bfloat16 or x.dtype != torch.bfloat16 or g.dtype != torch.float32 or dy.dim() != 2 or x.dim() != 2:
        return False
    R, M = dy.shape
    N = x.shape[1]
    if x.shape[0] != R or R % 64 or M % 256 or N % 256 or dy.stride(1) != 1 or x.stride(1) != 1 or g.stride(1) != 1:
        return False
    if dy.stride(0) % 8 or x.stride(0) % 8 or g.stride(0) % 4 or dy.data_ptr() % 16 or x.data_ptr() % 16 or tuple(g.shape) != (M, N):
        return False
    splits = tn_splits(R // 64, (M // 256) * (N // 256))
    if not splits:
        return False
    ws = torch.empty(splits * M * N, device=g.device, dtype=torch.float32)
    check(_lib.vl_gemm_tn_splitk_accum_f32(_p(dy), _p(x), _p(g), M, N, R, dy.stride(0), x.stride(0), g.stride(0),
                                           float(alpha), splits, _p(ws), _stream()))
    return True


def tn_splits(nk: int, tiles: int, few_tiles_ok: bool = False) -> int:
    valid = lambda splits: (nk // splits >= 16 and nk - (-(-nk // (-(-nk // splits))) - 1) * (-(-nk // splits)) >= 4)
    cands = (1, 2, 4, 8, 16, 32, 64) if few_tiles_ok else (1, 2, 4, 8, 16)
    best = 0
    for splits in cands:
        if not valid(splits):
            continue
        if tiles * splits >= 192:
            return splits
        best = splits
    return best if few_tiles_ok else 0


_pad_cache = {}


def _zero_padded(t, cols, tag):
    key = (tag, t.device, torch.cuda.current_stream(t.device).cuda_stream, threading.get_ident(), t.shape[0], t.shape[1], cols)
    buf = _pad_cache.get(key)
    if buf is None:
        buf = torch.zeros(t.shape[0], cols, device=t.device, dtype=torch.bfloat16)
        _pad_cache[key] = buf
    buf[:, :t.shape[1]].copy_(t)
    return buf


def gemm_dw_tn_any(dy, x, g, alpha=1.0):
    if dy.dtype != torch.bfloat16 or x.dtype != torch.bfloat16 or g.dtype != torch.float32 or dy.dim() != 2 or x.dim() != 2:
        return False
    R, M = dy.shape
    N = x.shape[1]
    if x.shape[0] != R or R % 64 or tuple(g.shape) != (M, N) or dy.stride(1) != 1 or x.stride(1) != 1:
        return False
    Mp, Np = (M + 255) // 256 * 256, (N + 255) // 256 * 256
    if Mp == M and Np == N and gemm_dw_tn(dy, x, g, alpha):
        return True
    if dy.stride(0) % 8 or x.stride(0) % 8 or dy.data_ptr() % 16 or x.data_ptr() % 16:
        return False
    splits = tn_splits(R // 64, (Mp // 256) * (Np // 256), few_tiles_ok=True)
    if not splits:
        return False
    dyp = dy if Mp == M else _zero_padded(dy, Mp, "dy")
    xp = x if Np == N else _zero_padded(x, Np, "x")
    direct = Mp == M and Np == N and g.stride(1) == 1 and g.stride(0) % 4 == 0
    gp = g if direct else torch.zeros(Mp, Np, device=g.device, dtype=torch.float32)
    ws = torch.empty(splits * Mp * Np, device=g.device, dtype=torch.float32)
    check(_lib.vl_gemm_tn_splitk_accum_f32(_p(dyp), _p(xp), _p(gp), Mp, Np, R, dyp.stride(0), xp.stride(0), gp.stride(0),
                                           float(alpha), splits, _p(ws), _stream()))
    if not direct:
        g += gp[:M, :N]
    return True


def _bhld_strides(*views):
    import ctypes
    vals = []
    for t in views:
        if t.dim() != 4 or t.stride(3) != 1 or t.dtype != views[0].dtype or t.dtype not in (torch.bfloat16, torch.float16):
            raise ValueError("attention operands must be bf16 (or, forward only, fp16) [B,H,L,dh] views of one dtype with unit last stride")
        vals += [t.stride(0), t.stride(1), t.stride(2)]
    return (ctypes.c_long * len(vals))(*vals)


def heads_view(x2d, B, L, H, dh, col0=0):
    W = x2d.stride(0)
    return x2d.as_strided((B, H, L, dh), (L * W, dh, W, 1), x2d.storage_offset() + col0)


def attn_fwd(q, k, v, out, lse=None, causal=False, qscale=1.0):
    B, H, Lq, dh = q.shape
    Lk = k.shape[2]
    st = _bhld_strides(q, k, v)
    if q.dtype == torch.float16:
        if k.dtype != q.dtype or v.dtype != q.dtype or out.dtype != q.dtype:
            raise TypeError("attn_fwd: fp16 q needs fp16 k, v and out")
        check(_lib.vl_attn_fwd_f16(_p(q), _p(k), _p(v), st, _p(out), _p(lse), B, H, Lq, Lk, dh, float(qscale),
                                   1 if causal else 0, _stream()))
        return out
    check(_lib.vl_attn_fwd_bf16(_p(q), _p(k), _p(v), st, _p(out), _p(lse), B, H, Lq, Lk, dh, float(qscale),
                                1 if causal else 0, _stream()))
    return out


def _q1_rows(t, H, name):
    if t.dim() != 2 or t.stride(1) != 1 or t.dtype != torch.bfloat16 or t.shape[1] != H * 64:
        raise ValueError(f"{name}: need a bf16 [B, H*64] matrix with unit column stride, got {tuple(t.shape)} {t.dtype}")


def attn_fwd_q1(q, k, v, out, lse=None, qrow=0, qscale=1.0):
    B, H, L, dh = q.shape
    if k.shape != q.shape or v.shape != q.shape or q.dtype != torch.bfloat16:
        raise ValueError("attn_fwd_q1: q, k, v must be bf16 views of one [B,H,L,dh] shape (self-attention)")
    _q1_rows(out, H, "attn_fwd_q1: out")
    if out.shape[0] != B or (lse is not None and (lse.dtype != torch.float32 or not lse.is_contiguous() or lse.numel() != B * H)):
        raise ValueError("attn_fwd_q1: out must have B rows, lse must be a contiguous f32 [B, H]")
    check(_lib.vl_attn_fwd_q1(_p(q), _p(k), _p(v), _bhld_strides(q, k, v), _p(out), out.stride(0), _p(lse), B, H, L, dh,
                              int(qrow), float(qscale), _stream()))
    return out


def layernorm(x, w, b, out, rows, D, x_row_stride=None, row_index=None, row_mul=0, mean=None, rstd=None,
              eps=1e-5):
    xs = D if x_row_stride is None else x_row_stride
    check(_lib.vl_layernorm_fwd(_p(x), _dt(x), xs, _p(row_index), row_mul, _p(w), _p(b), _p(out), _dt(out),
                                out.stride(-2) if out.dim() >= 2 else D, _p(mean), _p(rstd), rows, D,
                                float(eps), _stream()))
    return out


def assemble_ln_pre(tokens, cls, pos, pos2, w, b, out, B, T, D, eps=1e-5, xpre=None, mean=None, rstd=None):
    check(_lib.vl_assemble_ln_pre(_p(tokens), _dt(tokens), _p(cls), _p(pos), _p(pos2), _p(w), _p(b), _p(out),
                                  _dt(out), _p(xpre), _p(mean), _p(rstd), B, T, D, float(eps), _stream()))
    return out


def l2_normalize(x, out=None, out_bf16=None, norms=None, eps=1e-12):
    _chk2d(x, "x", torch.float32)
    if out is None:
        out = torch.empty_like(x)
    check(_lib.vl_l2_normalize(_p(x), _p(out), _p(out_bf16), _p(norms), x.shape[0], x.shape[1], float(eps),
                               _stream()))
    return out


def l2_normalize_bwd(f, df, norms, eps=1e-12):
    dx = torch.empty_like(f)
    check(_lib.vl_l2_normalize_bwd(_p(f), _p(df), _p(norms), _p(dx), f.shape[0], f.shape[1], float(eps),
                                   _stream()))
    return dx


def im2col(x, kh, kw, sh, sw, Kp, transpose_hw=False, out=None):
    if x.dtype != torch.float32 or not x.is_contiguous():
        raise ValueError("im2col: need contiguous f32 input")
    N, Cc = x.shape[0], x.shape[1]
    H, W = (x.shape[3], x.shape[2]) if transpose_hw else (x.shape[2], x.shape[3])
    gh, gw = (H - kh) // sh + 1, (W - kw) // sw + 1
    if out is None:
        out = torch.empty(N * gh * gw, Kp, device=x.device, dtype=torch.bfloat16)
    check(_lib.vl_im2col_bf16(_p(x), _p(out), N, Cc, H, W, kh, kw, sh, sw, Kp, 1 if transpose_hw else 0,
                              _stream()))
    return out, gh, gw


def text_embed(ids, tok_emb, pos, out):
    B, L = ids.shape
    check(_lib.vl_text_embed(_p(ids), _p(tok_emb), _p(pos), _p(out), _dt(out), B, L, tok_emb.shape[1],
                             tok_emb.shape[0], _stream()))
    return out


def cast_bf16(x, out=None):
    if out is None:
        out = torch.empty(x.shape, device=x.device, dtype=torch.bfloat16)
    check(_lib.vl_cast_f32_bf16(_p(x), _p(out), x.numel(), _stream()))
    return out


def add_rows(x, table, out, rows, T, D):
    check(_lib.vl_add_rows(_p(x), _dt(x), _p(table), _p(out), _dt(out), rows, T, D, _stream()))
    return out


def transpose_to_bf16(x, ldo=None, out=None):
    _chk2d(x, "x")
    R, Cc = x.shape
    ldo = R if ldo is None else ldo
    if out is None:
        out = torch.empty(Cc, ldo, device=x.device, dtype=torch.bfloat16)
    check(_lib.vl_transpose_to_bf16(_p(x), _dt(x), x.stride(0), R, Cc, _p(out), ldo, _stream()))
    return out


def transpose_colsum(x, ldo, colsum_out=None, scale=1.0, out=None):
    _chk2d(x, "x")
    R, Cc = x.shape
    ok = Cc % 64 == 0 and ldo % 8 == 0 and x.stride(0) % 8 == 0 and R >= 256 and x.data_ptr() % 16 == 0
    if not ok:
        out = transpose_to_bf16(x, ldo=ldo, out=out)
        if colsum_out is not None:
            colsum(x, colsum_out, scale)
        return out
    if out is None:
        out = torch.empty(Cc, ldo, device=x.device, dtype=torch.bfloat16)
    ws = _ws_for(x.device, ldo, Cc, 1) if colsum_out is not None else None
    check(_lib.vl_transpose_colsum_bf16(_p(x), _dt(x), x.stride(0), R, Cc, _p(out), ldo, _p(colsum_out), float(scale), _p(ws),
                                        _stream()))
    return out


def split_bf16x3(x, pattern):
    _chk2d(x, "x", torch.float32)
    out = torch.empty(x.shape[0], 3 * x.shape[1], device=x.device, dtype=torch.bfloat16)
    check(_lib.vl_split_bf16x3(_p(x.contiguous()), _p(out), x.shape[0], x.shape[1], pattern, _stream()))
    return out


def _chk_sim(logits, sim, thres, who):
    if thres is None:
        raise ValueError(f"{who}: sim needs thres")
    if not torch.is_tensor(sim) or sim.dtype != torch.float32 or sim.dim() != 2 or tuple(sim.shape) != tuple(logits.shape):
        raise ValueError(f"{who}: sim must be an f32 tensor of the logits' shape {tuple(logits.shape)}")
    if sim.device != logits.device or sim.stride(1) != 1:
        raise ValueError(f"{who}: sim must live on the logits' device with contiguous rows")


def ce_stats(logits, label_off=0, want_cols=True, sim=None, thres=None):
    _chk2d(logits, "logits", torch.float32)
    if sim is None and thres is not None:
        raise ValueError("ce_stats: thres needs sim")
    if sim is not None:
        _chk_sim(logits, sim, thres, "ce_stats")
    R, Cc = logits.shape
    dev = logits.device
    row_lse = torch.empty(R, device=dev, dtype=torch.float32)
    diag = torch.empty(R, device=dev, dtype=torch.float32)
    col_lse = torch.empty(Cc, device=dev, dtype=torch.float32) if want_cols else None
    ws = torch.empty(2 * ((R + 63) // 64) * Cc, device=dev, dtype=torch.float32) if want_cols else None
    if sim is None:
        check(_lib.vl_ce_stats(_p(logits), logits.stride(0), R, Cc, label_off, _p(row_lse), _p(col_lse), _p(diag),
                               _p(ws), _stream()))
    else:
        check(_lib.vl_ce_stats_masked(_p(logits), logits.stride(0), R, Cc, label_off, _p(row_lse), _p(col_lse), _p(diag),
                                      _p(ws), _p(sim), sim.stride(0), float(thres), _stream()))
    return row_lse, col_lse, diag


def ce_loss_accum(loss, row_lse, col_lse, diag, R, Cc, label_off, w_row, w_col):
    check(_lib.vl_ce_loss_accum(_p(row_lse), _p(col_lse), _p(diag), R, Cc, label_off, float(w_row), float(w_col),
                                _p(loss), _stream()))


def ce_grad(logits, row_lse, col_lse, label_off, w_row, w_col, logit_scale, dscale, need_g=True, need_gt=True, sim=None,
            thres=None):
    if sim is None and thres is not None:
        raise ValueError("ce_grad: thres needs sim")
# ... 356 lines not shown
```

vit-lens_amd/vitlens_hip/step.py:

```python
import math
from typing import Dict, Optional

import torch

from . import ops
from .engine import LensCfg, LensEngine, TextCfg, TextEngine, TowerCfg, VitEngine
from .train import AdamW, DepthLensTrainer


class TorchComm:

    def all_gather(self, out: torch.Tensor, inp: torch.Tensor):
        import torch.distributed as dist
        if inp.is_cuda:
            dist.all_gather_into_tensor(out, inp)
        else:
            dist.all_gather(list(out.chunk(dist.get_world_size(), dim=0)), inp.contiguous())

    def all_reduce_sum(self, t: torch.Tensor):
        import torch.distributed as dist
        dist.all_reduce(t, op=dist.ReduceOp.SUM)

    def reduce_scatter_sum(self, out: torch.Tensor, inp: torch.Tensor):
        import torch.distributed as dist
# ... 16 lines not shown
        import ctypes as C
        from ._lib import check, load_library
        self._lib, self._check, self._C = load_library(), check, C
        self.rank, self.world = rank, world
        if device is not None:
            torch.cuda.set_device(device)
        if unique_id is None:
            if world != 1:
                raise ValueError("AbiComm: ranks > 0 need the unique id rank 0 made (AbiComm.make_unique_id / over_torch_distributed)")
            unique_id = self.make_unique_id()
        if len(unique_id) != 128:
            raise ValueError("AbiComm: the unique id is 128 bytes")
        self._h = C.c_void_p()
        buf = C.create_string_buffer(bytes(unique_id), 128)
        check(self._lib.vl_comm_create(C.byref(self._h), buf, rank, world))
        self._stream = None

    @staticmethod
    def make_unique_id() -> bytes:
        import ctypes as C
        from ._lib import check, load_library
        buf = C.create_string_buffer(128)
        check(load_library().vl_comm_unique_id(buf))
        return buf.raw

    @classmethod
    def over_torch_distributed(cls, device=None):
        import torch.distributed as dist
        rank, world = dist.get_rank(), dist.get_world_size()
        box = [cls.make_unique_id() if rank == 0 else None]
        dist.broadcast_object_list(box, src=0)
        return cls(rank, world, box[0], device)

    def close(self):
        if getattr(self, "_h", None) is not None and self._h.value:
            self._lib.vl_comm_destroy(self._h)
            self._h = self._C.c_void_p()

    def __del__(self):
        try:
            self.close()
        except Exception:
            pass

    def _s(self):
        return self._C.c_void_p(torch.cuda.current_stream().cuda_stream)

    @staticmethod
    def _f32(t, name):
        if t.dtype != torch.float32 or not t.is_contiguous() or not t.is_cuda:
            raise ValueError(f"AbiComm.{name}: contiguous fp32 GPU tensors only")
        return t

    def all_gather(self, out: torch.Tensor, inp: torch.Tensor):
        self._f32(out, "all_gather"); inp = self._f32(inp.contiguous(), "all_gather")
        self._check(self._lib.vl_allgather_embed(self._h, inp.data_ptr(), out.data_ptr(), inp.numel(), self._s()))

    def all_reduce_sum(self, t: torch.Tensor):
        self._f32(t, "all_reduce_sum")
        self._check(self._lib.vl_allreduce_grad(self._h, t.data_ptr(), t.numel(), self._s()))

    def reduce_scatter_sum(self, out: torch.Tensor, inp: torch.Tensor):
        self._f32(out, "reduce_scatter_sum"); inp = self._f32(inp.contiguous(), "reduce_scatter_sum")
        self._check(self._lib.vl_reducescatter_grad(self._h, inp.data_ptr(), out.data_ptr(), out.numel(), self._s()))

    def all_reduce_sum_async(self, t: torch.Tensor):
        self._f32(t, "all_reduce_sum_async")
        if self._stream is None:
            self._stream = torch.cuda.Stream()
        main = torch.cuda.current_stream()
        ready, done = torch.cuda.Event(), torch.cuda.Event()
        ready.record(main)
        self._stream.wait_event(ready)
        with torch.cuda.stream(self._stream):
            self.all_reduce_sum(t)
            done.record(self._stream)

        class _Handle:
            def wait(self_h):
                torch.cuda.current_stream().wait_event(done)
        return _Handle()


def _master_from_sd(name: str, sd, like: torch.Tensor) -> torch.Tensor:
    from .engine import _interleave_geglu, conv_weight_as_gemm
    dev = like.device
    f32 = lambda k: sd[k].detach().float().to(dev).clone()
    if name.endswith("conv1.weight_gemm"):
        return conv_weight_as_gemm(sd[name[:-5]], dev, torch.float32)
    if name.endswith("net.0.weight_il") or name.endswith("net.0.bias_il"):
        base = name[:name.rindex("net.0.")] + "net.0."
        w, b = _interleave_geglu(f32(base + "weight"), f32(base + "bias"))
        return (w if name.endswith("weight_il") else b).contiguous()
    if name.endswith("fn.to_qkv.weight"):
        return torch.cat([f32(name.replace("to_qkv", "to_q")), f32(name.replace("to_qkv", "to_kv"))], 0).contiguous()
    return f32(name).reshape(like.shape).contiguous()


def _master_to_sd(name: str, m: torch.Tensor, base_sd, cfg) -> Dict[str, torch.Tensor]:
    from .train import deinterleave_geglu
    if name.endswith("conv1.weight_gemm"):
        ref = base_sd[name[:-5]]
        return {name[:-5]: m[:, :ref[0].numel()].reshape(ref.shape)}
    if name.endswith("_il"):
        return {name[:-3]: deinterleave_geglu(m)}
    if name.endswith("fn.to_qkv.weight"):
        inner = cfg.latent_heads * cfg.latent_dim_head
        return {name.replace("to_qkv", "to_q"): m[:inner], name.replace("to_qkv", "to_kv"): m[inner:]}
    return {name: m.reshape(base_sd[name].shape)}


class _StepState:

    def _init_host(self, sd, device, micro_batch, rank, world_size, comm=None, local_loss=False, gather_with_grad=False,
                   force_comm=False, overlap_frozen=False, overlap_backward=True, grad_clip_norm=None):
        self.dev, self.mb, self.rank, self.world = torch.device(device), micro_batch, rank, world_size
        self._force_comm = bool(force_comm)
        self.comm = comm or TorchComm()
        self.local_loss, self.gather_with_grad = local_loss, gather_with_grad
        self.overlap_frozen = bool(overlap_frozen)
        self.overlap_backward = bool(overlap_backward)
        self._side = None
        self._base_sd = {k: v.detach() for k, v in sd.items()}
        self.logit_scale = sd["logit_scale"].detach().float().reshape(1).to(device).clone()
        self.masters: Dict[str, torch.Tensor] = {"logit_scale": self.logit_scale}
        self.bf16_targets = {}
        self.refresh = []
        self.trainers = []
        self.flat_grad, self.grads = None, {}
        self._pending, self._reduced_upto, self._reduce_done = [], None, False
        if grad_clip_norm is not None and not float(grad_clip_norm) > 0.0:
            raise ValueError(f"grad_clip_norm must be positive (or None), got {grad_clip_norm}")
        self.grad_clip_norm = None if grad_clip_norm is None else float(grad_clip_norm)
        self._sumsq = None

    @property
    def last_grad_norm(self):
        return self.opt.last_grad_norm

    def _clipped_optimizer_step(self):
        self.finish_reduce()
        if self._sumsq is None:
            self._sumsq = torch.zeros(1, device=self.dev, dtype=torch.float32)
        ops.grad_sumsq(self.flat_grad, out=self._sumsq)
        self.opt.step(self.grads, grad_scale=1.0 / self.world, max_norm=self.grad_clip_norm, sumsq=self._sumsq)

    @property
    def dist(self) -> bool:
        return self.world > 1 or self._force_comm

    @property
    def _overlap_active(self) -> bool:
        return self.overlap_frozen and self.dev.type == "cuda"

    def _side_by_side(self, beside, here):
        frozen, trainable = beside, here
        if not self._overlap_active:
            frozen(); trainable()
            return
        if self._side is None:
            self._side = torch.cuda.Stream(device=self.dev)
        main = torch.cuda.current_stream(self.dev)
        ready, done = torch.cuda.Event(), torch.cuda.Event()
        ready.record(main)
        self._side.wait_event(ready)
        with torch.cuda.stream(self._side):
            frozen()
            done.record(self._side)
        trainable()
        main.wait_event(done)

    def state_dict(self) -> Dict[str, torch.Tensor]:
        out = {k: v.detach().clone() for k, v in self._base_sd.items()}
        cfg = getattr(self.lens, "lens", None)
        for name, m in self.masters.items():
            for k, v in _master_to_sd(name, m.detach(), self._base_sd, cfg).items():
                out[k] = v.to(device=self._base_sd[k].device, dtype=self._base_sd[k].dtype).clone()
        if cfg is not None and getattr(cfg, "weight_tie_layers", False):
            P1 = "visual.perceiver.layers.1."
            for k in [k for k in out if k.startswith(P1)]:
                for li in range(2, cfg.depth):
                    out[f"visual.perceiver.layers.{li}." + k[len(P1):]] = out[k].clone()
        tok = getattr(self, "tok", None)
        if tok is not None:
            for k, (rm, rv) in tok.running.items():
                out["visual.visual_adapter." + k + ".running_mean"] = rm.detach().cpu().clone()
                out["visual.visual_adapter." + k + ".running_var"] = rv.detach().cpu().clone()
        return out

    def optimizer_state_dict(self):
        return {"step": self.opt.t, "exp_avg": {k: v.detach().clone() for k, v in self.opt.m.items()},
                "exp_avg_sq": {k: v.detach().clone() for k, v in self.opt.v.items()}}

    def load_state_dict(self, sd):
        for name, m in self.masters.items():
            m.copy_(_master_from_sd(name, sd, m))
        tok = getattr(self, "tok", None)
        if tok is not None:
            for k, (rm, rv) in tok.running.items():
                rm.copy_(sd["visual.visual_adapter." + k + ".running_mean"].float()); rv.copy_(sd["visual.visual_adapter." + k + ".running_var"].float())
        if not self.trainers:
            self._trainer(0)
        self._refresh_operands()
        self._base_sd = {k: v.detach() for k, v in sd.items()}

    def load_optimizer_state_dict(self, st):
        self.opt.t = int(st["step"])
        for k in self.opt.m:
            self.opt.m[k].copy_(st["exp_avg"][k]); self.opt.v[k].copy_(st["exp_avg_sq"][k])


LOGITS_CHUNK_ELEMS = 1 << 26
LOGITS_CHUNK_ROWS = 2048


def _chunk_rows(R: int, Cn: int, chunk_rows: Optional[int]) -> int:
    if chunk_rows is None:
        chunk_rows = LOGITS_CHUNK_ROWS if R * Cn >= LOGITS_CHUNK_ELEMS else 0
    return 0 if chunk_rows <= 0 or chunk_rows >= R else int(chunk_rows)


def _is_dev_scale(scale) -> bool:
    return torch.is_tensor(scale)


def _mask_operands(mask, R: int, Cn: int):
    trow, tcol, thres = mask
    if trow.shape[0] != R or tcol.shape[0] != Cn or trow.shape[1] != tcol.shape[1]:
        raise ValueError(f"pair loss mask: teacher features {tuple(trow.shape)} x {tuple(tcol.shape)} do not describe the "
                         f"{R} x {Cn} logits")
    return (ops.split_bf16x3(trow.detach().float().contiguous(), 0), ops.split_bf16x3(tcol.detach().float().contiguous(), 1),
            float(thres))


def _label_columns_only(col_lse, label_off: int, R: int):
    if col_lse is not None and (label_off > 0 or label_off + R < col_lse.shape[0]):
        col_lse[:max(label_off, 0)] = float("inf")
        col_lse[label_off + R:] = float("inf")
    return col_lse


def pair_forward(x, y, scale, label_off: int = 0, w_row: float = 0.5, w_col: float = 0.5,
                 chunk_rows: Optional[int] = None, mask=None):
    R, Cn = x.shape[0], y.shape[0]
    rb = _chunk_rows(R, Cn, chunk_rows)
    dev_scale = _is_dev_scale(scale)
    alpha = 1.0 if dev_scale else scale
    xb = ops.split_bf16x3(ops.scale_exp(x.contiguous(), scale) if dev_scale else x, 0)
    yb = ops.split_bf16x3(y, 1)
    tr = tc = thres = None
    if mask is not None:
        tr, tc, thres = _mask_operands(mask, R, Cn)
    if rb == 0:
        logits = ops.logits_gemm(xb, yb, alpha)
        if mask is None:
            sim = None
            row_lse, col_lse, diag = ops.ce_stats(logits, label_off, want_cols=(w_col != 0.0))
        else:
            sim = ops.logits_gemm(tr, tc, 1.0)
            row_lse, col_lse, diag = ops.ce_stats(logits, label_off, want_cols=(w_col != 0.0), sim=sim, thres=thres)
        col_lse = _label_columns_only(col_lse, label_off, R)
        loss = torch.zeros(1, device=x.device, dtype=torch.float32)
        ops.ce_loss_accum(loss, row_lse if w_row != 0.0 else None, col_lse, diag, R, Cn, label_off, w_row, w_col)
        return loss, (x, y, logits, row_lse, col_lse, label_off, w_row, w_col, scale, 0, None, None, sim, None, thres)
    row_lse = torch.empty(R, device=x.device); diag = torch.empty(R, device=x.device)
    col_parts = []
    for r0 in range(0, R, rb):
        r1 = min(R, r0 + rb)
        lg = ops.logits_gemm(xb[r0:r1], yb, alpha)
        if mask is None:
            rl, cl, dg = ops.ce_stats(lg, label_off + r0, want_cols=(w_col != 0.0))
        else:
            sm = ops.logits_gemm(tr[r0:r1], tc, 1.0)
            rl, cl, dg = ops.ce_stats(lg, label_off + r0, want_cols=(w_col != 0.0), sim=sm, thres=thres)
            del sm
        row_lse[r0:r1] = rl; diag[r0:r1] = dg
        if cl is not None:
            col_parts.append(cl)
        del lg
    col_lse = _label_columns_only(torch.logsumexp(torch.stack(col_parts), dim=0), label_off, R) if col_parts else None
    loss = torch.zeros(1, device=x.device, dtype=torch.float32)
    ops.ce_loss_accum(loss, row_lse if w_row != 0.0 else None, col_lse, diag, R, Cn, label_off, w_row, w_col)
    return loss, (x, y, None, row_lse, col_lse, label_off, w_row, w_col, scale, rb, xb, yb, tr, tc, thres)


def pair_backward(ctx, g: float = 1.0, need_dx=True, need_dy=True):
    x, y, logits, row_lse, col_lse, label_off, w_row, w_col, scale, rb, xb, yb, sim, tc, thres = ctx
    mk = (lambda sm: {}) if thres is None else (lambda sm: dict(sim=sm, thres=thres))
    dscale = torch.zeros(1, device=x.device, dtype=torch.float32)
    dev_scale = _is_dev_scale(scale)
    alpha, cscale = (1.0, 1.0) if dev_scale else (scale, scale)
    fin = (lambda t: ops.scale_exp(t, scale, out=t)) if dev_scale else (lambda t: t)
    if rb == 0:
        G, GT = ops.ce_grad(logits, row_lse if w_row != 0.0 else None, col_lse, label_off, w_row * g, w_col * g, cscale,
                            dscale, need_g=need_dx, need_gt=need_dy, **mk(sim))
        dx = dy = None
        if need_dx:
            dx = fin(ops.gemm(G, ops.transpose_to_bf16(y, ldo=G.shape[1]), None, epi=ops.EPI_F32, alpha=alpha))
        if need_dy:
            dy = fin(ops.gemm(GT, ops.transpose_to_bf16(x, ldo=GT.shape[1]), None, epi=ops.EPI_F32, alpha=alpha))
        return dx, dy, dscale
    R, Cn = x.shape[0], y.shape[0]
    dx = torch.empty(R, x.shape[1], device=x.device) if need_dx else None
    dy = torch.zeros(Cn, y.shape[1], device=x.device) if need_dy else None
    yt = None
    tr = sim
# ... 32 lines not shown
        dxl, d_ay, ds1 = pair_backward(c1, need_dx=need_x, need_dy=need_y and gather_with_grad)
        dyl, d_ax, ds2 = pair_backward(c2, need_dx=need_y, need_dy=need_x and gather_with_grad)
        loss, ds = l1 + l2, ds1 + ds2
    else:
        loss, c = pair_forward(ax, ay, scale, **({} if ta is None else dict(mask=(ta, ta, sim_thres))))
        d_ax, d_ay, ds = pair_backward(c, need_dx=need_x, need_dy=need_y)
        dxl = dyl = None

    def fold(dl, d_all):
        if d_all is None:
            return dl
        if not dist:
            g = d_all
        elif gather_with_grad:
            g = torch.empty(b, d_all.shape[1], device=d_all.device, dtype=d_all.dtype)
            comm.reduce_scatter_sum(g, d_all.contiguous())
        else:
            g = d_all[rank * b:(rank + 1) * b].contiguous()
        return g if dl is None else dl + g
    return loss, (fold(dxl, d_ax) if need_x else None), (fold(dyl, d_ay) if need_y else None), ds


class TriModalDepthStep(_StepState):
    def __init__(self, sd: Dict[str, torch.Tensor], tower: TowerCfg, text: TextCfg, device, micro_batch: int = 256,
                 unlock_first_n: int = 4, lr: float = 5e-4, betas=(0.9, 0.98), eps: float = 1e-6, weight_decay: float = 0.2,
                 rank: int = 0, world_size: int = 1, gemm_cfg: int = -1, comm=None, frozen_res_dtype=torch.float32,
                 local_loss: bool = False, gather_with_grad: bool = False, train_res_dtype=torch.float32,
                 grad_checkpointing: bool = False, force_comm: bool = False, text_wsplit: Optional[bool] = None, text_arith: str = "f16",
                 overlap_frozen: bool = True, overlap_backward: bool = True,
                 grad_clip_norm: Optional[float] = None):
        self._init_host(sd, device, micro_batch, rank, world_size, comm, local_loss, gather_with_grad, force_comm, overlap_frozen,
                        overlap_backward, grad_clip_norm)
        self.grad_checkpointing = bool(grad_checkpointing)
        self.unlock_first_n = unlock_first_n
        self._build(sd, tower, text, gemm_cfg=gemm_cfg, frozen_res_dtype=frozen_res_dtype, train_res_dtype=train_res_dtype,
                    text_wsplit=text_wsplit, text_arith=text_arith)
        self.opt = AdamW(self.masters, lr=lr, betas=betas, eps=eps, weight_decay=weight_decay)

    def _build(self, sd, tower, text, gemm_cfg=-1, frozen_res_dtype=torch.float32, train_res_dtype=torch.float32,
               text_wsplit=None, text_arith="f16"):
        device, unlock_first_n = self.dev, self.unlock_first_n
        self.image = VitEngine(sd, "image.", tower, device, gemm_cfg=gemm_cfg, res_dtype=frozen_res_dtype)
        self.text = TextEngine(sd, text, device, gemm_cfg=gemm_cfg, res_dtype=frozen_res_dtype, wsplit=text_wsplit, arith=text_arith)
        self.lens = LensEngine(sd, "visual.", tower, LensCfg(modality="depth", perceiver_identity=True), device, gemm_cfg=gemm_cfg,
                               res_dtype=train_res_dtype)
        eng = self.lens.vit
        for l in range(unlock_first_n):
            p = f"visual.transformer.resblocks.{l}."
            w = eng.blocks[l]
            w.pop("in_f", None); w.pop("fc_f", None)
            for nm, key in (("attn.in_proj_weight", "in_w"), ("attn.out_proj.weight", "out_w"), ("mlp.c_fc.weight", "fc_w"),
                            ("mlp.c_proj.weight", "proj_w")):
                self.masters[p + nm] = sd[p + nm].detach().float().to(device).contiguous().clone()
                self.bf16_targets[p + nm] = (l, key)
            for nm, key in (("ln_1.weight", "ln1_w"), ("ln_1.bias", "ln1_b"), ("ln_2.weight", "ln2_w"), ("ln_2.bias", "ln2_b"),
                            ("attn.in_proj_bias", "in_b"), ("attn.out_proj.bias", "out_b"), ("mlp.c_fc.bias", "fc_b"),
                            ("mlp.c_proj.bias", "proj_b")):
                self.masters[p + nm] = w[key]
        self.masters["visual.visual_adapter.pos_emb"] = self.lens.adapter_pos
        from .engine import conv_weight_as_gemm
        self.masters["visual.visual_adapter.conv1.weight_gemm"] = conv_weight_as_gemm(
            sd["visual.visual_adapter.conv1.weight"], device, torch.float32)

    def _trainer(self, i):
        while len(self.trainers) <= i:
            t = DepthLensTrainer(self.lens, tower_kw=dict(train_blocks=range(self.unlock_first_n), checkpoint=self.grad_checkpointing))
            if self.trainers:
                t.tower.wT = self.trainers[0].tower.wT
                t.tower.proj = self.trainers[0].tower.proj
                t.tower.grads = self.trainers[0].tower.grads
            self.trainers.append(t)
        return self.trainers[i]

    def _alloc_flat_grads(self):
        al = lambda n: (n + 3) // 4 * 4
        self.flat_grad = torch.zeros(sum(al(v.numel()) for v in self.masters.values()), device=self.dev, dtype=torch.float32)
        off = 0
        for k, v in self.masters.items():
            self.grads[k] = self.flat_grad[off:off + v.numel()].view(v.shape)
            off += al(v.numel())
        self.flat_grad_b = torch.zeros_like(self.flat_grad)
        self.grads_b, off = {}, 0
        for k, v in self.masters.items():
            self.grads_b[k] = self.flat_grad_b[off:off + v.numel()].view(v.shape)
            off += al(v.numel())
        for t in self.trainers:
            t.tower.grads = self.grads

    def _refresh_operands(self):
        eng = self.lens.vit
        if not self.trainers:
            self._trainer(0)
        for name, (l, key) in self.bf16_targets.items():
            m = self.masters[name]
            ops.cast_bf16(m, out=eng.blocks[l][key])
            ops.transpose_to_bf16(m, ldo=m.shape[0], out=self.trainers[0].tower.wT[l][key])
        ops.cast_bf16(self.masters["visual.visual_adapter.conv1.weight_gemm"], out=self.lens.conv_w)

    def step(self, images: torch.Tensor, texts: torch.Tensor, depths: torch.Tensor) -> torch.Tensor:
        loss = self.forward_backward(images, texts, depths)
        self.optimizer_step()
        return loss

    def finish_reduce(self):
        if not self.dist or self._reduce_done:
            return
        for h in self._pending:
            h.wait()
        self._pending = []
        if self._reduced_upto is None:
            self.comm.all_reduce_sum(self.flat_grad)
        else:
            lo, hi = self._rest_ranges()
            for a, b in ((0, lo), (hi, self.flat_grad.numel())):
                if b > a:
                    self.comm.all_reduce_sum(self.flat_grad[a:b])
        self._reduced_upto = None
        self._reduce_done = True

    def reduced_grads(self):
        self.finish_reduce()
        return self.grads

    def optimizer_step(self):
        if self.grad_clip_norm is not None:
            self._clipped_optimizer_step()
        elif self.dist:
            self.finish_reduce()
            self.opt.step(self.grads, grad_scale=1.0 / self.world)
        else:
            self.opt.step(self.grads)
        self._refresh_operands()
        ops.clamp_scalar(self.logit_scale, 0.0, math.log(100.0))

    def _block_range(self, l):
        p = f"visual.transformer.resblocks.{l}."
        names = [k for k in self.masters if k.startswith(p)]
        base = self.flat_grad.data_ptr()
        lo = min((self.grads[k].data_ptr() - base) // 4 for k in names)
        hi = max((self.grads[k].data_ptr() - base) // 4 + self.grads[k].numel() for k in names)
        return lo, min((hi + 3) // 4 * 4, self.flat_grad.numel())

    def _rest_ranges(self):
        rs = [self._block_range(l) for l in range(self.unlock_first_n)]
        return min(r[0] for r in rs), max(r[1] for r in rs)

    def _start_block_reduce(self, l):
        if self.dist and hasattr(self.comm, "all_reduce_sum_async"):
            lo, hi = self._block_range(l)
            self._pending.append(self.comm.all_reduce_sum_async(self.flat_grad[lo:hi]))
            self._reduced_upto = l

    def forward_backward(self, images: torch.Tensor, texts: torch.Tensor, depths: torch.Tensor) -> torch.Tensor:
        B = images.shape[0]
        mb = min(self.mb, B)
        assert B % mb == 0, "per-GPU batch must be a multiple of the micro-batch"
        nmb = B // mb
        if self.flat_grad is None:
            for i in range(nmb):
                self._trainer(i)
            self._alloc_flat_grads()
        for h in self._pending:
            h.wait()
        self._pending, self._reduced_upto, self._reduce_done = [], None, False
        self.flat_grad.zero_()
        E = self.image.cfg.embed_dim
        fi = torch.empty(B, E, device=self.dev); ft = torch.empty(B, E, device=self.dev)
        fv = torch.empty(B, E, device=self.dev); vraw = torch.empty(B, E, device=self.dev)
        vnorm = torch.empty(B, device=self.dev)
        def frozen():
            ops.l2_normalize(self.text.encode_text(texts), out=ft)
            for i in range(nmb):
                s = slice(i * mb, (i + 1) * mb)
                ops.l2_normalize(self.image.encode_image(images[s]), out=fi[s])

        def trainable():
            for i in range(nmb):
                s = slice(i * mb, (i + 1) * mb)
                vraw[s] = self._trainer(i).forward(depths[s])
        self._side_by_side(frozen, trainable)
        ops.l2_normalize(vraw, out=fv, norms=vnorm)
        scale = self.logit_scale
        if self.dist:
            packed = torch.cat([fi, ft, fv], dim=1)
            allp = torch.empty(self.world * B, 3 * E, device=self.dev)
            self.comm.all_gather(allp, packed)
            ai, at, av = [t.contiguous() for t in allp.split(E, dim=1)]
        else:
            ai, at, av = fi, ft, fv
        kw = dict(local_loss=self.local_loss, gather_with_grad=self.gather_with_grad, need_x=False, dist=self.dist)
        l1, _, dv1, ds1 = pair_loss_and_grads(self.comm, self.rank, self.world, fi, fv, ai, av, scale, **kw)
        l2, _, dv2, ds2 = pair_loss_and_grads(self.comm, self.rank, self.world, ft, fv, at, av, scale, **kw)
        loss = l1 + l2
        dvraw = ops.l2_normalize_bwd(fv, dv1 + dv2, vnorm)
        self._backward_all(dvraw, nmb, mb)
        self.grads["logit_scale"] += ds1 + ds2
        return loss

    def _backward_all(self, dvraw, nmb, mb):
        dist_cb = self.dist and self.unlock_first_n > 0
        dv = lambda i: dvraw[i * mb:(i + 1) * mb].contiguous()
        half = nmb // 2
        for i in range(nmb):
            self._trainer(i).tower.grads = self.grads_b if i < half else self.grads
        if half == 0:
            self._trainer(0).backward(dv(0), self._start_block_reduce if dist_cb else None)
            return
        self.flat_grad_b.zero_()
        two_streams = self._overlap_active and self.overlap_backward
        passed = {}

        def first_done(l):
            if two_streams:
                passed[l] = torch.cuda.Event()
                passed[l].record()

        def second_done(l):
            if two_streams:
                torch.cuda.current_stream(self.dev).wait_event(passed[l])
            lo, hi = self._block_range(l)
            ops.axpy(self.flat_grad[lo:hi], self.flat_grad_b[lo:hi])
            if dist_cb:
                self._start_block_reduce(l)

        def first_half():
            for i in range(half):
                self._trainer(i).backward(dv(i), first_done if i == half - 1 else None)

        def second_half():
            for i in range(half, nmb):
                self._trainer(i).backward(dv(i), second_done if i == nmb - 1 else None)
        if two_streams:
            self._side_by_side(first_half, second_half)
        else:
            first_half(); second_half()
        n = self.flat_grad.numel()
        lo, hi = self._rest_ranges() if self.unlock_first_n > 0 else (0, 0)
        for a, b in ((0, lo), (hi, n)):
            if b > a:
                ops.axpy(self.flat_grad[a:b], self.flat_grad_b[a:b])


class _PerceiverLensStep(_StepState):

    def _collect_perceiver(self, sd):
        pe, P = self.lens.perceiver, "visual.perceiver."
        f32 = lambda k: sd[k].detach().float().to(self.dev).contiguous().clone()
        self.masters[P + "latents"] = pe.latents
        for li, lay in enumerate(pe.layers):
            if li >= 2 and lay is pe.layers[1]:
                continue
            q = f"{P}layers.{li}."
            self._attn(q + "0.", lay["x_attn"], lay["x_norm"], (li, "x"), sd, f32, ctx_norm=lay["x_norm_ctx"])
            self._ff(q + "1.", lay["x_ff"], lay["x_ff_norm"], (li, "xff"), sd, f32)
            for sj, sl in enumerate(lay["selfs"]):
                r = f"{q}2.{sj}."
                self._attn(r + "0.", sl["attn"], sl["norm"], (li, "selfs", sj), sd, f32)
                self._ff(r + "1.", sl["ff"], sl["ff_norm"], (li, "selfs", sj), sd, f32)

    def _attn(self, p, a, norm, path, sd, f32, ctx_norm=None):
        self.masters[p + "norm.weight"], self.masters[p + "norm.bias"] = norm
        if ctx_norm is not None:
            self.masters[p + "norm_context.weight"], self.masters[p + "norm_context.bias"] = ctx_norm
            self.masters[p + "fn.to_q.weight"] = f32(p + "fn.to_q.weight"); self.refresh.append((p + "fn.to_q.weight", a["q_w"], path + ("q",)))
            self.masters[p + "fn.to_kv.weight"] = f32(p + "fn.to_kv.weight"); self.refresh.append((p + "fn.to_kv.weight", a["kv_w"], path + ("kv",)))
        else:
            self.masters[p + "fn.to_qkv.weight"] = torch.cat([f32(p + "fn.to_q.weight"), f32(p + "fn.to_kv.weight")], 0)
            self.refresh.append((p + "fn.to_qkv.weight", a["qkv_w"], path + ("qkv",)))
        self.masters[p + "fn.to_out.weight"] = f32(p + "fn.to_out.weight"); self.refresh.append((p + "fn.to_out.weight", a["to_out_w"], path + ("out",)))
        self.masters[p + "fn.to_out.bias"] = a["to_out_b"]

    def _ff(self, p, ff, norm, path, sd, f32):
        from .engine import _interleave_geglu
        self.masters[p + "norm.weight"], self.masters[p + "norm.bias"] = norm
        w0, _ = _interleave_geglu(f32(p + "fn.net.0.weight"), f32(p + "fn.net.0.bias"))
        self.masters[p + "fn.net.0.weight_il"] = w0.contiguous(); self.refresh.append((p + "fn.net.0.weight_il", ff["w0"], path + ("w0",)))
        self.masters[p + "fn.net.0.bias_il"] = ff["b0"]
        self.masters[p + "fn.net.2.weight"] = f32(p + "fn.net.2.weight"); self.refresh.append((p + "fn.net.2.weight", ff["w2"], path + ("w2",)))
        self.masters[p + "fn.net.2.bias"] = ff["b2"]

    def _trainer(self, i):
        while len(self.trainers) <= i:
            t = self._mk()
            if self.trainers:
                t.tower.wT, t.tower.proj = self.trainers[0].tower.wT, self.trainers[0].tower.proj
                t.perc.wT = self.trainers[0].perc.wT
            self.trainers.append(t)
        return self.trainers[i]

    def _bind_grads(self, t, grads=None):
        g = self.grads if grads is None else grads
        t.tower.grads = g; t.perc.grads = g

    def _alloc_flat_grads(self):
        al = lambda n: (n + 3) // 4 * 4
        self.flat_grad = torch.zeros(sum(al(v.numel()) for v in self.masters.values()), device=self.dev, dtype=torch.float32)
        self.flat_grad_b = torch.zeros_like(self.flat_grad)
        self.grads_b, off = {}, 0
        for k, v in self.masters.items():
            self.grads[k] = self.flat_grad[off:off + v.numel()].view(v.shape)
            self.grads_b[k] = self.flat_grad_b[off:off + v.numel()].view(v.shape)
            off += al(v.numel())
        for t in self.trainers:
            self._bind_grads(t)

    def reference_named_grads(self):
        return self.trainers[0].perc.reference_named_grads(self.grads)

    def _backward_all(self, dvraw, nmb, mb):
        dv = lambda i: dvraw[i * mb:(i + 1) * mb].contiguous()
        half = nmb // 2
        for i in range(nmb):
            self._bind_grads(self._trainer(i), self.grads_b if i < half else self.grads)
        if half == 0:
            self._trainer(0).backward(dv(0))
            return
        self.flat_grad_b.zero_()

        def first_half():
            for i in range(half):
                self._trainer(i).backward(dv(i))

        def second_half():
            for i in range(half, nmb):
                self._trainer(i).backward(dv(i))
        if getattr(self, "_one_stream_backward", False) or not self.overlap_backward:
            first_half(); second_half()
        else:
            self._side_by_side(first_half, second_half)
        ops.axpy(self.flat_grad, self.flat_grad_b)

    def _prepare(self, B):
        mb = min(self.mb, B)
        assert B % mb == 0, "per-GPU batch must be a multiple of the micro-batch"
        nmb = B // mb
        if self.flat_grad is None:
            for i in range(nmb):
                self._trainer(i)
            self._alloc_flat_grads()
        self._reduce_done = False
        self.flat_grad.zero_()
        return mb, nmb

    def _refresh_perceiver(self):
        wT = self.trainers[0].perc.wT
        for name, fwd, path in self.refresh:
            m = self.masters[name]
            ops.cast_bf16(m, out=fwd)
            node = wT[path[0]]
            for k in path[1:-1]:
                node = node[k]
            ops.transpose_to_bf16(m, ldo=m.shape[0], out=node[path[-1]])

    def _refresh_operands(self):
        self._refresh_perceiver()

    def finish_reduce(self):
        if self.dist and not self._reduce_done:
            self.comm.all_reduce_sum(self.flat_grad)
            self._reduce_done = True

    def reduced_grads(self):
        self.finish_reduce()
        return self.grads

    def optimizer_step(self):
        if self.grad_clip_norm is not None:
            self._clipped_optimizer_step()
        elif self.dist:
            self.finish_reduce()
            self.opt.step(self.grads, grad_scale=1.0 / self.world)
        else:
            self.opt.step(self.grads)
        self._refresh_operands()
        ops.clamp_scalar(self.logit_scale, 0.0, math.log(100.0))


class DualAudioStep(_PerceiverLensStep):

    def __init__(self, sd, tower: TowerCfg, text: TextCfg, lens: LensCfg, device, micro_batch: int = 256, lr: float = 2e-4,
                 betas=(0.9, 0.98), eps: float = 1e-6, weight_decay: float = 0.2, rank: int = 0, world_size: int = 1,
                 gemm_cfg: int = -1, comm=None, frozen_res_dtype=torch.float32, local_loss: bool = False,
                 gather_with_grad: bool = False, train_res_dtype=torch.float32, force_comm: bool = False, text_wsplit: Optional[bool] = None, text_arith: str = "f16",
                 overlap_frozen: bool = True, overlap_backward: bool = True,
                 grad_clip_norm: Optional[float] = None, contra_loss_type: str = "general", sim_thres: float = 0.8):
        if contra_loss_type not in ("general", "sim_mask"):
            raise NotImplementedError(f"DualAudioStep: contra_loss_type is 'general' or 'sim_mask', got {contra_loss_type!r} "
                                      "(label_mask cannot run in the reference's drivers either)")
        self.contra_loss_type, self.sim_thres = contra_loss_type, float(sim_thres)
        self._init_host(sd, device, micro_batch, rank, world_size, comm, local_loss, gather_with_grad, force_comm, overlap_frozen,
                        overlap_backward, grad_clip_norm)
        self._build(sd, tower, text, lens, gemm_cfg=gemm_cfg, frozen_res_dtype=frozen_res_dtype, train_res_dtype=train_res_dtype,
                    text_wsplit=text_wsplit, text_arith=text_arith)
        self.opt = AdamW(self.masters, lr=lr, betas=betas, eps=eps, weight_decay=weight_decay)

    def _build(self, sd, tower, text, lens, gemm_cfg=-1, frozen_res_dtype=torch.float32, train_res_dtype=torch.float32,
               text_wsplit=None, text_arith="f16"):
        from .train import AudioLensTrainer
        device = self.dev
        self.text = TextEngine(sd, text, device, gemm_cfg=gemm_cfg, res_dtype=frozen_res_dtype, wsplit=text_wsplit, arith=text_arith)
        self.lens = LensEngine(sd, "visual.", tower, lens, device, gemm_cfg=gemm_cfg, res_dtype=train_res_dtype)
        self._mk = lambda: AudioLensTrainer(self.lens)
        self.masters["visual.class_embedding"] = self.lens.vit.cls
        self.masters["visual.visual_adapter.pos_emb"] = self.lens.adapter_pos
        from .engine import conv_weight_as_gemm
        self.masters["visual.visual_adapter.conv1.weight_gemm"] = conv_weight_as_gemm(
            sd["visual.visual_adapter.conv1.weight"], device, torch.float32)
        self._collect_perceiver(sd)

    def _refresh_operands(self):
        self._refresh_perceiver()
        ops.cast_bf16(self.masters["visual.visual_adapter.conv1.weight_gemm"], out=self.lens.conv_w)

    def forward_backward(self, audio: torch.Tensor, texts: torch.Tensor) -> torch.Tensor:
        B = audio.shape[0]
        mb, nmb = self._prepare(B)
        E = self.lens.tower.embed_dim
        ft = torch.empty(B, E, device=self.dev); fv = torch.empty(B, E, device=self.dev)
        vraw = torch.empty(B, E, device=self.dev); vnorm = torch.empty(B, device=self.dev)
        def frozen():
            ops.l2_normalize(self.text.encode_text(texts), out=ft)

        def trainable():
            for i in range(nmb):
                s = slice(i * mb, (i + 1) * mb)
                vraw[s] = self._trainer(i).forward(audio[s])
        self._side_by_side(frozen, trainable)
        ops.l2_normalize(vraw, out=fv, norms=vnorm)
        scale = self.logit_scale
        if self.dist:
            allp = torch.empty(self.world * B, 2 * E, device=self.dev)
            self.comm.all_gather(allp, torch.cat([fv, ft], dim=1))
            av, at = [t.contiguous() for t in allp.split(E, dim=1)]
        else:
            av, at = fv, ft
        mk = dict(sim_teacher="y", sim_thres=self.sim_thres) if self.contra_loss_type == "sim_mask" else {}
        loss, dv, _, ds = pair_loss_and_grads(self.comm, self.rank, self.world, fv, ft, av, at, scale,
                                              local_loss=self.local_loss, gather_with_grad=self.gather_with_grad, need_y=False, dist=self.dist,
                                              **mk)
        dvraw = ops.l2_normalize_bwd(fv, dv, vnorm)
        self._backward_all(dvraw, nmb, mb)
        self.grads["logit_scale"] += ds
        return loss

    def step(self, audio, texts):
        loss = self.forward_backward(audio, texts)
        self.optimizer_step()
        return loss


class TriModalPCStep(_PerceiverLensStep):

    def __init__(self, sd, tower: TowerCfg, text: TextCfg, lens: LensCfg, device, micro_batch: int = 32, lr: float = 2e-4,
                 betas=(0.9, 0.98), eps: float = 1e-6, weight_decay: float = 0.2, rank: int = 0, world_size: int = 1,
                 gemm_cfg: int = -1, bn_training: bool = True, unlock_cls: bool = False, comm=None,
                 frozen_res_dtype=torch.float32, local_loss: bool = False, gather_with_grad: bool = False,
                 train_res_dtype=torch.float32, bn_sync: bool = False, force_comm: bool = False, text_wsplit: Optional[bool] = None, text_arith: str = "f16",
                 overlap_frozen: bool = True, overlap_backward: bool = True,
                 grad_clip_norm: Optional[float] = None):
        self._init_host(sd, device, micro_batch, rank, world_size, comm, local_loss, gather_with_grad, force_comm, overlap_frozen,
                        overlap_backward, grad_clip_norm)
        self._build(sd, tower, text, lens, gemm_cfg=gemm_cfg, frozen_res_dtype=frozen_res_dtype, train_res_dtype=train_res_dtype,
                    text_wsplit=text_wsplit, text_arith=text_arith, bn_training=bn_training, bn_sync=bn_sync, unlock_cls=unlock_cls)
        self.opt = AdamW(self.masters, lr=lr, betas=betas, eps=eps, weight_decay=weight_decay)

    def _build(self, sd, tower, text, lens, gemm_cfg=-1, frozen_res_dtype=torch.float32, train_res_dtype=torch.float32,
               text_wsplit=None, text_arith="f16", bn_training=True, bn_sync=False, unlock_cls=False):
        from .points import PointTokenizerTrainer
        from .train import PCLensTrainer
        device = self.dev
        self.image = VitEngine(sd, "image.", tower, device, gemm_cfg=gemm_cfg, res_dtype=frozen_res_dtype)
        self.text = TextEngine(sd, text, device, gemm_cfg=gemm_cfg, res_dtype=frozen_res_dtype, wsplit=text_wsplit, arith=text_arith)
        self.lens = LensEngine(sd, "visual.", tower, lens, device, gemm_cfg=gemm_cfg, res_dtype=train_res_dtype)
        self.tok = PointTokenizerTrainer(sd, "visual.visual_adapter.", lens, device, gemm_cfg=gemm_cfg, bn_training=bn_training,
                                         bn_sync=self.comm if bn_sync and self.dist else None, world_size=self.world)
        self._one_stream_backward = bool(bn_sync and self.dist)
        self._mk = lambda: PCLensTrainer(self.lens, self.tok, train_cls=unlock_cls)
        if unlock_cls:
            self.masters["visual.class_embedding"] = self.lens.vit.cls
        self.masters.update(self.tok.masters)
        self._collect_perceiver(sd)

    def _bind_grads(self, t, grads=None):
        g = self.grads if grads is None else grads
        t.tower.grads = g; t.perc.grads = g; t.tok.grads = g
        self.tok.grads = self.grads

    def _refresh_operands(self):
        self._refresh_perceiver()
        self.tok.refresh_operands()
        for t in self.trainers:
            t.tok.op = self.tok.op

    def forward_backward(self, images, texts, points, fps_start=None) -> torch.Tensor:
        B = images.shape[0]
        mb, nmb = self._prepare(B)
        E = self.image.cfg.embed_dim
        fi = torch.empty(B, E, device=self.dev); ft = torch.empty(B, E, device=self.dev)
        fv = torch.empty(B, E, device=self.dev); vraw = torch.empty(B, E, device=self.dev)
        vnorm = torch.empty(B, device=self.dev)
        def frozen():
            ops.l2_normalize(self.text.encode_text(texts), out=ft)
            for i in range(nmb):
                s = slice(i * mb, (i + 1) * mb)
                ops.l2_normalize(self.image.encode_image(images[s]), out=fi[s])

        def trainable():
            for i in range(nmb):
                s = slice(i * mb, (i + 1) * mb)
                vraw[s] = self._trainer(i).forward(points[s], None if fps_start is None else fps_start[s])
        self._side_by_side(frozen, trainable)
        ops.l2_normalize(vraw, out=fv, norms=vnorm)
        scale = self.logit_scale
        if self.dist:
            allp = torch.empty(self.world * B, 3 * E, device=self.dev)
            self.comm.all_gather(allp, torch.cat([fi, ft, fv], dim=1))
            ai, at, av = [t.contiguous() for t in allp.split(E, dim=1)]
        else:
            ai, at, av = fi, ft, fv
        kw = dict(local_loss=self.local_loss, gather_with_grad=self.gather_with_grad, need_x=False, dist=self.dist)
        l1, _, dv1, ds1 = pair_loss_and_grads(self.comm, self.rank, self.world, fi, fv, ai, av, scale, **kw)
        l2, _, dv2, ds2 = pair_loss_and_grads(self.comm, self.rank, self.world, ft, fv, at, av, scale, **kw)
        dvraw = ops.l2_normalize_bwd(fv, dv1 + dv2, vnorm)
        self._backward_all(dvraw, nmb, mb)
        self.grads["logit_scale"] += ds1 + ds2
        return l1 + l2

    def step(self, images, texts, points, fps_start=None):
        loss = self.forward_backward(images, texts, points, fps_start)
        self.optimizer_step()
        return loss
```

Measured before the change: 1820 modality-pairs/sec.

## Pack text tokens by actual length and run varlen attention in the text tower

Adds a packing plan that computes per-caption token lengths on device, embeds only the real tokens into a packed row buffer, and runs the frozen text tower's GEMMs, layernorms and a new variable-length fp16 attention kernel over packed rows rather than padded B×77. The aim is to skip compute on padding tokens in the frozen text encoder, which runs on a side stream next to the trainable tower. The attention body is moved into a shared include so the dense and varlen kernels reuse it. The cost is extra plan and embed kernels, and possibly a host sync to learn the packed row count. Any gain depends on how much the text stream sits on the critical path.

Result: faster. 1858 modality-pairs/sec (median of 6 runs) (+2.1%).

```diff
diff --git a/include/vitlens_hip.h b/include/vitlens_hip.h
--- a/include/vitlens_hip.h
+++ b/include/vitlens_hip.h
@@ -34,7 +34,7 @@
 #define VL_GEMM_PINGPONG 10
 
 const char* vl_last_error(void);
-#define VL_ABI_VERSION 607
+#define VL_ABI_VERSION 608
 int vl_version(void);
 
 int vl_gemm_bf16(const void* A, const void* W, const float* bias, void* out, const void* res,
@@ -53,6 +53,14 @@
                 int lda, int ldw, int ldo, float alpha, int epi, int act, hipStream_t stream);
 int vl_attn_fwd_f16(const void* q, const void* k, const void* v, const long* strides, void* out, float* lse,
                     int B, int H, int Lq, int Lk, int dh, float qscale, int causal, hipStream_t stream);
+
+int vl_text_pack_plan(const int64_t* ids, int* len, int* start, int64_t* last_row, int* total, int B, int L,
+                      hipStream_t stream);
+int vl_text_embed_packed(const int64_t* ids, const int* start, const int* len, const float* tok_emb, const float* pos,
+                         float* out, int B, int L, int D, int vocab, int rows, int rows_pad, hipStream_t stream);
+int vl_attn_fwd_varlen_f16(const void* q, const void* k, const void* v, const long* strides, const int* start,
+                           const int* len, void* out, float* lse, int B, int H, int max_len, int dh, float qscale,
+                           hipStream_t stream);
 
 int vl_gemm_f32(const float* A, const float* W, const float* bias, float* out, const float* res, int M, int N, int K,
                 int lda, int ldw, int ldo, float alpha, int act, hipStream_t stream);
diff --git a/vit-lens_amd/csrc/vl_attn.hip b/vit-lens_amd/csrc/vl_attn.hip
--- a/vit-lens_amd/csrc/vl_attn.hip
+++ b/vit-lens_amd/csrc/vl_attn.hip
@@ -5,6 +5,7 @@
 using namespace vlattn;
 
 constexpr int KC = 288;
+constexpr int KC_DENSE = KC;
 constexpr int VSP = KC + 8;
 constexpr int NWMAX = 8;
 constexpr float RESCALE_THR = 8.0f;
@@ -19,302 +20,40 @@
   VL_PROF_FIELD
   int lq_main;
 };
+struct AttnPV : AttnP {
+  const int* vstart;
+  const int* vlen;
+};
 
 template <int DH, bool TAILQ, bool MULTI, bool F16 = false, bool DMA = false>
 __global__ void __launch_bounds__(NWMAX * 64, DH == 128 ? 2 : 4) attn_fwd_kernel(const AttnP p) {
   static_assert(!F16 || (!TAILQ && DH == 64), "half operands: head dim 64, no shared last row (the text tower's shape)");
   static_assert(!DMA || (DH == 64 && !MULTI && !F16), "LDS-DMA staging: head dim 64, one key chunk, bf16");
-  constexpr int RB = DH * 2;
-  constexpr int CH = RB / 16;
-  constexpr int RSH = Rsh<DH>::v;
-  constexpr bool PAD = DH == 128;
-  constexpr int KS = DH / 16;
-  constexpr int DT = DH / 32;
-  extern __shared__ __attribute__((aligned(16))) unsigned char smem[];
-  unsigned char* sK = smem;
-  bf16_t* sV = (bf16_t*)(smem + KC * RB);
-  float* sP = (float*)(sV + DH * VSP);
-  float* sPart = sP + NWMAX * 32;
-  bf16_t* sTailQ = (bf16_t*)(sPart + (KC / 32) * (2 + DH));
+  constexpr bool VARLEN = false;
+  [[maybe_unused]] constexpr long row0 = 0;
+#include "vl_attn_fwd_body.inc"
+}
 
-  const int b = blockIdx.z, h = blockIdx.y;
-  const int tid = threadIdx.x, nthr = blockDim.x;
-  const int lane = tid & 63;
-  const int wid = __builtin_amdgcn_readfirstlane(tid >> 6);
-  const int nwq = nthr >> 6;
-  const int fr = lane & 31, fg = lane >> 5;
-  const size_t bh = (size_t)b * p.H + h;
-  const bf16_t* Kg = p.k.p + b * p.k.sb + h * p.k.sh;
-  const bf16_t* Vg = p.v.p + b * p.v.sb + h * p.v.sh;
-  const bf16_t* Qb = p.q.p + b * p.q.sb + h * p.q.sh;
-
-  const int q0 = (blockIdx.x * nwq + wid) * 32;
-  const bool wave_active = q0 < p.lq_main;
-  int qrow = q0 + fr; if (qrow >= p.lq_main) qrow = p.lq_main - 1;
-  const int qidx = q0 + fr;
-  const int dhr = PAD ? p.dh : DH;
-  const int nch = dhr >> 3;
-
-  VL_PROF_STAMP(p, 0);
-  u32x4 qraw[KS];
+template <int KCT>
+__global__ void __launch_bounds__(NWMAX * 64, 4) attn_fwd_varlen_kernel(const AttnPV pin) {
+  static_assert(KCT % 32 == 0 && KCT >= 32 && KCT <= KC_DENSE, "LDS chunk: whole key tiles, at most the dense chunk");
+  constexpr int DH = 64;
+  constexpr bool TAILQ = false, MULTI = false, F16 = true, DMA = false, VARLEN = true;
+  constexpr int KC = KCT;
+  constexpr int VSP = KC + 8;
+  AttnP pcap = pin;
+  long row0;
   {
-    const bf16_t* Qg = Qb + (long)qrow * p.q.sr;
-#pragma unroll
-    for (int ks = 0; ks < KS; ++ks) {
-      qraw[ks] = u32x4{0u, 0u, 0u, 0u};
-      if (!PAD || ks * 2 + fg < nch) qraw[ks] = *(const u32x4*)(Qg + ks * 16 + fg * 8);
-    }
+    const int b = blockIdx.z;
+    const int len = min(pin.vlen[b], KC);
+    if (len <= 0 || (int)((blockIdx.x * (blockDim.x >> 6)) * 32) >= len) return;
+    row0 = pin.vstart[b];
+    pcap.Lq = pcap.Lk = pcap.lq_main = len;
+    pcap.q.p += row0 * pin.q.sr; pcap.k.p += row0 * pin.k.sr; pcap.v.p += row0 * pin.v.sr;
+    pcap.q.sb = pcap.k.sb = pcap.v.sb = 0;
   }
-  [[maybe_unused]] u32x4 tailraw = {0u, 0u, 0u, 0u};
-  if constexpr (TAILQ) {
-    if constexpr (!PAD) tailraw = *(const u32x4*)(Qb + (long)(p.Lq - 1) * p.q.sr + (tid & (CH - 1)) * 8);
-    else if (tid < nch) tailraw = *(const u32x4*)(Qb + (long)(p.Lq - 1) * p.q.sr + tid * 8);
-  }
-  unsigned char* const sVr = (unsigned char*)sV;
-  auto vswz = [](int row) { const int x = (row >> 1) & 7; return ((x & 1) << 2) | (x >> 1); };
-  if constexpr (DMA) {
-    typedef __attribute__((address_space(3))) void* lds_p;
-    const int nrows = ((p.Lk + 31) >> 5) << 5;
-    const __amdgpu_buffer_rsrc_t rsK = __builtin_amdgcn_make_buffer_rsrc((void*)Kg, 0, 0x7ffffff0, 0x00020000);
-    const __amdgpu_buffer_rsrc_t rsV = __builtin_amdgcn_make_buffer_rsrc((void*)Vg, 0, 0x7ffffff0, 0x00020000);
-    for (int u = wid; u * 8 < p.Lk; u += nwq) {
-      const int row = u * 8 + (lane >> 3), sl = lane & 7;
-      if (row < p.Lk) {
-        const unsigned offK = (unsigned)(row * (int)p.k.sr + ((sl ^ ((row >> 1) & 7)) << 3)) * 2u;
-        const unsigned offV = (unsigned)(row * (int)p.v.sr + ((sl ^ vswz(row)) << 3)) * 2u;
-        __builtin_amdgcn_raw_ptr_buffer_load_lds(rsK, (lds_p)(sK + u * 1024), 16, offK, 0, 0, 0);
-        __builtin_amdgcn_raw_ptr_buffer_load_lds(rsV, (lds_p)(sVr + u * 1024), 16, offV, 0, 0, 0);
-      }
-    }
-    for (int i = tid; i < (nrows - p.Lk) * 8; i += nthr)
-      *(u32x4*)(sVr + (p.Lk + (i >> 3)) * 128 + ((i & 7) << 4)) = u32x4{0u, 0u, 0u, 0u};
-    asm volatile("s_waitcnt vmcnt(0)" ::: "memory");
-  } else {
-  stage2<DH, KC, true, false, false, true>(StageSrc{sK, nullptr, Kg, p.k.sr, 1.f, nch}, StageSrc{nullptr, sV, Vg, p.v.sr, 1.f, nch},
-                                           0, p.Lk, tid, nthr);
-  }
-  if constexpr (TAILQ) {
-    if constexpr (!PAD) *(u32x4*)(sTailQ + (tid & (CH - 1)) * 8) = tailraw;
-    else if (tid < CH) *(u32x4*)(sTailQ + tid * 8) = tailraw;
-  }
-  VL_PROF_STAMP(p, 1);
-  [[maybe_unused]] const int li = lane & 15, lb3 = (li >> 3) & 1;
-  [[maybe_unused]] const unsigned aTr = (unsigned)((fg * 4 + (li >> 2)) * 128) +
-                                        (((unsigned)(((lane >> 4) & 1) * 2 + ((li >> 1) & 1)) ^ (unsigned)((lb3 << 2) | fg)) << 4) + (unsigned)((li & 1) << 3);
-  auto trV = [&](int tile, int c, int t) {
-    typedef __attribute__((ext_vector_type(4))) short s16x4;
-    typedef __attribute__((address_space(3))) s16x4* lds_s16x4;
-    struct { s16x4 lo, hi; } f;
-    const unsigned a = (aTr + (unsigned)(tile * 4096)) ^ (unsigned)(t * 64);
-    f.lo = __builtin_amdgcn_ds_read_tr16_b64_v4i16((lds_s16x4)(sVr + a + c * 2048));
-    f.hi = __builtin_amdgcn_ds_read_tr16_b64_v4i16((lds_s16x4)(sVr + (a ^ 32u) + c * 2048 + 1024));
-    return __builtin_bit_cast(bf16x8, f);
-  };
-  bf16x8 qf[KS];
-#pragma unroll
-  for (int ks = 0; ks < KS; ++ks)
-    qf[ks] = __builtin_bit_cast(bf16x8, p.qscale != 1.0f ? scale_x8<F16>(qraw[ks], p.qscale) : qraw[ks]);
-
-  float m_run = 0.f;
-  vl_f32x2 l2 = {0.f, 0.f};
-  f32x16 negm;
-  f32x16 o[DT];
-#pragma unroll
-  for (int r = 0; r < 16; ++r) negm[r] = 0.f;
-#pragma unroll
-  for (int t = 0; t < DT; ++t)
-#pragma unroll
-    for (int r = 0; r < 16; ++r) o[t][r] = 0.f;
-  bool first = true;
-
-  auto tail_partials = [&]() {
-    if constexpr (TAILQ) {
-    const int qT = p.Lq - 1;
-    const int ntile = (p.Lk + 31) >> 5;
-    const int ksw = (fr >> RSH) & (CH - 1);
-    bf16x8 qa[KS];
-#pragma unroll
-    for (int ks = 0; ks < KS; ++ks) {
-#pragma unroll
-      for (int e = 0; e < 8; ++e) qa[ks][e] = (__bf16)0.f;
-      if (fr == 0) {
-        u32x4 raw = *(const u32x4*)(sTailQ + ks * 16 + fg * 8);
-        if (p.qscale != 1.0f) raw = scale_bf16x8(raw, p.qscale);
-        qa[ks] = __builtin_bit_cast(bf16x8, raw);
-      }
-    }
-    for (int kt = wid; kt < ntile; kt += nwq) {
-      f32x16 st;
-#pragma unroll
-      for (int r = 0; r < 16; ++r) st[r] = 0.f;
-      const unsigned char* kbase = sK + (kt * 32 + fr) * RB;
-#pragma unroll
-      for (int ks = 0; ks < KS; ++ks)
-        st = __builtin_amdgcn_mfma_f32_32x32x16_bf16(qa[ks], *(const bf16x8*)(kbase + (((ks * 2 + fg) ^ ksw) * 16)), st, 0, 0, 0);
-      const bool valid = fg == 0 && kt * 32 + fr < p.Lk;
-      const float sv = valid ? st[0] : -INFINITY;
-      const float mw = wave_max_dpp(sv);
-      const float pw = valid ? __builtin_amdgcn_exp2f(sv - mw) : 0.f;
-      const float lw = wave_sum_dpp(pw);
-      float* myP = sP + wid * 32;
-      if (fg == 0) myP[fr] = pw;
-      __builtin_amdgcn_fence(__ATOMIC_RELEASE, "wavefront");
-      __builtin_amdgcn_wave_barrier();
-      __builtin_amdgcn_fence(__ATOMIC_ACQUIRE, "wavefront");
-      f32x16 ot[DT];
-#pragma unroll
-      for (int t = 0; t < DT; ++t)
-#pragma unroll
-        for (int r = 0; r < 16; ++r) ot[t][r] = 0.f;
-#pragma unroll
-      for (int c = 0; c < 2; ++c) {
-        bf16x8 pa;
-#pragma unroll
-        for (int e = 0; e < 8; ++e) pa[e] = (__bf16)0.f;
-        if (fr == 0) {
-          const f32x4 lo = *(const f32x4*)(myP + c * 16 + fg * 4);
-          const f32x4 hi = *(const f32x4*)(myP + c * 16 + 8 + fg * 4);
-#pragma unroll
-          for (int e = 0; e < 4; ++e) { pa[e] = (__bf16)lo[e]; pa[4 + e] = (__bf16)hi[e]; }
-        }
-#pragma unroll
-        for (int t = 0; t < DT; ++t)
-          ot[t] = __builtin_amdgcn_mfma_f32_32x32x16_bf16(
-              pa, DMA ? trV(kt, c, t) : *(const bf16x8*)(sV + (t * 32 + fr) * VSP + kt * 32 + c * 16 + fg * 8), ot[t], 0, 0, 0);
-      }
-      __builtin_amdgcn_wave_barrier();
-      float* part = sPart + kt * (2 + DH);
-      if (lane == 0) { part[0] = mw; part[1] = lw; }
-      if (fg == 0) {
-#pragma unroll
-        for (int t = 0; t < DT; ++t) part[2 + t * 32 + fr] = ot[t][0];
-      }
-    }
-    }
-  };
-  auto tail_merge = [&]() {
-    if constexpr (TAILQ) {
-      const int qT = p.Lq - 1;
-      const int ntile = (p.Lk + 31) >> 5;
-      if (wid == 0) {
-        float M = -INFINITY;
-        for (int kt = 0; kt < ntile; ++kt) M = fmaxf(M, sPart[kt * (2 + DH)]);
-        for (int d = lane; d < dhr; d += 64) {
-          float L = 0.f, acc = 0.f;
-          for (int kt = 0; kt < ntile; ++kt) {
-            const float* part = sPart + kt * (2 + DH);
-            const float w = __builtin_amdgcn_exp2f(part[0] - M);
-            L = fmaf(part[1], w, L);
-            acc = fmaf(part[2 + d], w, acc);
-          }
-          p.out[((size_t)b * p.Lq + qT) * (p.H * dhr) + h * dhr + d] = f2bf(acc / L);
-          if (p.lse && d == 0) p.lse[bh * p.Lq + qT] = (M + __log2f(L)) * 0.6931471805599453f;
-        }
-      }
-    }
-  };
-  const int q_hi = q0 + 31;
-  const int blk_q_hi = min(p.lq_main - 1, (int)(blockIdx.x * nwq + nwq) * 32 - 1);
-
-  for (int kc0 = 0; kc0 < (MULTI ? p.Lk : 1); kc0 += KC) {
-    if (MULTI && p.causal && kc0 > blk_q_hi) break;
-    if constexpr (MULTI) {
-      if (kc0 > 0) {
-        __syncthreads();
-        stage2<DH, KC, true, false, false, true, 1>(StageSrc{sK, nullptr, Kg, p.k.sr, 1.f, nch},
-                                                    StageSrc{nullptr, sV, Vg, p.v.sr, 1.f, nch}, kc0, p.Lk, tid, nthr);
-      }
-    }
-    __syncthreads();
-    VL_PROF_STAMP(p, 2);
-    if constexpr (TAILQ) { tail_partials(); __syncthreads(); }
-    if (!wave_active) continue;
-
-    int ntile = (min(p.Lk - kc0, KC) + 31) >> 5;
-    if (p.causal) ntile = min(ntile, ((q_hi - kc0) >> 5) + 1);
-    const int ksw = (fr >> RSH) & (CH - 1);
-    for (int kt = 0; kt < ntile; ++kt) {
-      const unsigned char* kbase = sK + (kt * 32 + fr) * RB;
-      bf16x8 kf[KS];
-#pragma unroll
-      for (int ks = 0; ks < KS; ++ks) kf[ks] = *(const bf16x8*)(kbase + (((ks * 2 + fg) ^ ksw) * 16));
-      f32x16 s = mfma32<F16>(kf[0], qf[0], negm);
-#pragma unroll
-      for (int ks = 1; ks < KS; ++ks) s = mfma32<F16>(kf[ks], qf[ks], s);
-      bf16x8 vf0[DT];
-#pragma unroll
-      for (int t = 0; t < DT; ++t) {
-        if constexpr (DMA) vf0[t] = trV(kt, 0, t);
-        else vf0[t] = *(const bf16x8*)(sV + (t * 32 + fr) * VSP + kt * 32 + fg * 8);
-      }
-      const int key0 = kc0 + kt * 32 + fg * 4;
-      const bool need_mask = (key0 - fg * 4 + 32 > p.Lk) || (p.causal && key0 - fg * 4 + 31 > q0);
-      if (need_mask) {
-#pragma unroll
-        for (int r = 0; r < 16; ++r) {
-          const int key = key0 + (r & 3) + 8 * (r >> 2);
-          if (key >= p.Lk || (p.causal && key > qidx)) s[r] = -INFINITY;
-        }
-      }
-      float mx = fmaxf(fmaxf(s[0], s[1]), s[2]);
-#pragma unroll
-      for (int r = 3; r < 15; r += 2) mx = fmaxf(fmaxf(mx, s[r]), s[r + 1]);
-      mx = fmaxf(mx, s[15]);
-      mx = xhalf_max(mx);
-      if (__builtin_amdgcn_ballot_w64(first || mx > RESCALE_THR) != 0) {
-        const float d = first ? mx : fmaxf(mx, 0.f);
-        const float alpha = first ? 0.f : __builtin_amdgcn_exp2f(-d);
-        m_run += d;
-#pragma unroll
-        for (int r = 0; r < 16; ++r) { s[r] -= d; negm[r] -= d; }
-#pragma unroll
-        for (int t = 0; t < DT; ++t)
-#pragma unroll
-          for (int r = 0; r < 16; ++r) o[t][r] *= alpha;
-        l2 *= alpha;
-        first = false;
-      }
-      float pv[16];
-#pragma unroll
-      for (int r = 0; r < 16; ++r) pv[r] = __builtin_amdgcn_exp2f(s[r]);
-      {
-        vl_f32x2 a0 = {pv[0], pv[1]}, a1 = {pv[2], pv[3]}, a2 = {pv[4], pv[5]}, a3 = {pv[6], pv[7]};
-        const vl_f32x2 a4 = {pv[8], pv[9]}, a5 = {pv[10], pv[11]}, a6 = {pv[12], pv[13]}, a7 = {pv[14], pv[15]};
-        a0 += a4; a1 += a5; a2 += a6; a3 += a7;
-        a0 += a2; a1 += a3;
-        l2 += a0 + a1;
-      }
-      bf16x8 vf1[DT];
-#pragma unroll
-      for (int t = 0; t < DT; ++t) {
-        if constexpr (DMA) vf1[t] = trV(kt, 1, t);
-        else vf1[t] = *(const bf16x8*)(sV + (t * 32 + fr) * VSP + kt * 32 + 16 + fg * 8);
-      }
-      {
-        const bf16x8 pf = pack8x<F16>(pv);
-#pragma unroll
-        for (int t = 0; t < DT; ++t) o[t] = mfma32<F16>(vf0[t], pf, o[t]);
-      }
-      {
-        const bf16x8 pf = pack8x<F16>(pv + 8);
-#pragma unroll
-        for (int t = 0; t < DT; ++t) o[t] = mfma32<F16>(vf1[t], pf, o[t]);
-      }
-    }
-  }
-
-  VL_PROF_STAMP(p, 3);
-  if (wave_active) {
-    const float l_tot = xhalf_sum(l2[0] + l2[1]);
-    const float inv = 1.0f / l_tot;
-    store_rows_t<DT, F16>(o, inv, p.out + ((size_t)b * p.Lq + qrow) * (p.H * dhr) + h * dhr, fg, qidx < p.lq_main, nch);
-    if (p.lse && fg == 0 && qidx < p.lq_main)
-      p.lse[bh * p.Lq + qidx] = (m_run + __log2f(l_tot)) * 0.6931471805599453f;
-  }
-
-  VL_PROF_STAMP(p, 4);
-  tail_merge();
-  VL_PROF_STAMP(p, 5);
+  const AttnP& p = pcap;
+#include "vl_attn_fwd_body.inc"
 }
 
 }
@@ -329,6 +68,19 @@
                                                      hipFuncAttributeMaxDynamicSharedMemorySize, (int)smem);
   if (attr != hipSuccess) return vl_set_error(hipGetErrorString(attr));
   hipLaunchKernelGGL((attn_fwd_kernel<DH, TAILQ, MULTI, F16, DMA>), dim3(gx, p.H, p.B), dim3(nwq * 64), smem, stream, p);
+  const hipError_t e = hipGetLastError();
+  return e == hipSuccess ? 0 : vl_set_error(hipGetErrorString(e));
+}
+
+template <int KCT>
+static int launch_fwd_varlen(const AttnPV& p, int gx, int nwq, hipStream_t stream) {
+  constexpr int DH = 64;
+  const size_t smem = (size_t)KCT * DH * 2 + (size_t)DH * (KCT + 8) * 2 + (size_t)NWMAX * 32 * 4 + (size_t)(KCT / 32) * (2 + DH) * 4 +
+                      (size_t)DH * 2;
+  static const hipError_t attr = hipFuncSetAttribute((const void*)attn_fwd_varlen_kernel<KCT>,
+                                                     hipFuncAttributeMaxDynamicSharedMemorySize, (int)smem);
+  if (attr != hipSuccess) return vl_set_error(hipGetErrorString(attr));
+  hipLaunchKernelGGL((attn_fwd_varlen_kernel<KCT>), dim3(gx, p.H, p.B), dim3(nwq * 64), smem, stream, p);
   const hipError_t e = hipGetLastError();
   return e == hipSuccess ? 0 : vl_set_error(hipGetErrorString(e));
 }
@@ -383,3 +135,29 @@
   const int gx = (qtiles + nwq - 1) / nwq;
   return launch_fwd<64, false, false, true>(p, gx, nwq, stream);
 }
+
+extern "C" int vl_attn_fwd_varlen_f16(const void* q, const void* k, const void* v, const long* strides, const int* start,
+                                      const int* len, void* out, float* lse, int B, int H, int max_len, int dh, float qscale,
+                                      hipStream_t stream) {
+  if (B <= 0 || H <= 0 || max_len <= 0) return vl_set_error("vl_attn_fwd_varlen_f16: empty problem");
+  if (dh != 64) return vl_set_error("vl_attn_fwd_varlen_f16: head dim must be 64");
+  if (max_len > KC) return vl_set_error("vl_attn_fwd_varlen_f16: at most 288 rows per caption");
+  if (!q || !k || !v || !out) return vl_set_error("vl_attn_fwd_varlen_f16: q, k, v and out required");
+  if (!strides || !start || !len) return vl_set_error("vl_attn_fwd_varlen_f16: strides, start and len required");
+  for (int i = 0; i < 6; ++i)
+    if (strides[i] & 7) return vl_set_error("vl_attn_fwd_varlen_f16: operand strides must be multiples of 8 elements (16-byte rows)");
+  if ((((uintptr_t)q) | ((uintptr_t)k) | ((uintptr_t)v)) & 15) return vl_set_error("vl_attn_fwd_varlen_f16: operands must be 16-byte aligned");
+  AttnPV p{{TV{(const bf16_t*)q, 0, strides[0], strides[1]}, TV{(const bf16_t*)k, 0, strides[2], strides[3]},
+            TV{(const bf16_t*)v, 0, strides[4], strides[5]}, qscale, (bf16_t*)out, lse, B, H, max_len, max_len, 1, dh,
+#ifdef VL_ATTN_PROF
+            vl_attn_prof_buf,
+#endif
+            max_len},
+           start, len};
+  const int qtiles = (max_len + 31) / 32;
+  const int nwq = qtiles < NWMAX ? qtiles : NWMAX;
+  const int gx = (qtiles + nwq - 1) / nwq;
+  if (max_len <= 32) return launch_fwd_varlen<32>(p, gx, nwq, stream);
+  if (max_len <= 96) return launch_fwd_varlen<96>(p, gx, nwq, stream);
+  return launch_fwd_varlen<KC>(p, gx, nwq, stream);
+}
diff --git a/vit-lens_amd/csrc/vl_attn_common.h b/vit-lens_amd/csrc/vl_attn_common.h
--- a/vit-lens_amd/csrc/vl_attn_common.h
+++ b/vit-lens_amd/csrc/vl_attn_common.h
@@ -77,25 +77,38 @@
   }
 }
 
-template <int DH, int NR, bool ROWS0, bool TRANS0, bool ROWS1, bool TRANS1, int U = 3>
-__device__ __forceinline__ void stage2(const StageSrc& m0, const StageSrc& m1, int row0, int L, int tid, int nthr) {
+template <int DH, int NR, bool ROWS0, bool TRANS0, bool ROWS1, bool TRANS1, int U = 3, bool CLAMP = false>
+__device__ __forceinline__ void stage2(const StageSrc& m0, const StageSrc& m1, int row0, int L, int tid, int nthr,
+                                       int np_rt = 0) {
+  static_assert(!CLAMP || DH != 128, "the clamped form has no padded head dims (every chunk of a row is read)");
   constexpr int CH = DH / 8, NP = (NR / 2) * CH;
-  for (int base = 0; base < NP; base += U * nthr) {
+  const int np = CLAMP ? np_rt : NP;
+  for (int base = 0; base < np; base += U * nthr) {
     u32x4 a0[U], b0[U], a1[U], b1[U];
 #pragma unroll
     for (int u = 0; u < U; ++u) {
       const int i = base + u * nthr + tid;
+      if constexpr (CLAMP) {
+        const int ic = min(i, np - 1);
+        const int rp = ic / CH, c = ic % CH;
+        const unsigned ra = (unsigned)min(row0 + 2 * rp, L - 1), rb = (unsigned)min(row0 + 2 * rp + 1, L - 1);
+        a0[u] = *(const u32x4*)((const unsigned char*)m0.src + (ra * (unsigned)m0.sr + c * 8) * 2u);
+        a1[u] = *(const u32x4*)((const unsigned char*)m1.src + (ra * (unsigned)m1.sr + c * 8) * 2u);
+        b0[u] = *(const u32x4*)((const unsigned char*)m0.src + (rb * (unsigned)m0.sr + c * 8) * 2u);
+        b1[u] = *(const u32x4*)((const unsigned char*)m1.src + (rb * (unsigned)m1.sr + c * 8) * 2u);
+        continue;
+      }
       const int rp = i / CH, c = i % CH;
       const int row = row0 + 2 * rp;
       const u32x4 z = {0u, 0u, 0u, 0u};
       a0[u] = z; b0[u] = z; a1[u] = z; b1[u] = z;
       const unsigned o0 = ((unsigned)row * (unsigned)m0.sr + c * 8) * 2u, o1 = ((unsigned)row * (unsigned)m1.sr + c * 8) * 2u;
       const bool cok = DH != 128 || c < m0.nch;
-      if (i < NP && row < L && cok) {
+      if (i < np && row < L && cok) {
         a0[u] = *(const u32x4*)((const unsigned char*)m0.src + o0);
         a1[u] = *(const u32x4*)((const unsigned char*)m1.src + o1);
       }
-      if (i < NP && row + 1 < L && cok) {
+      if (i < np && row + 1 < L && cok) {
         b0[u] = *(const u32x4*)((const unsigned char*)m0.src + (o0 + (unsigned)m0.sr * 2u));
         b1[u] = *(const u32x4*)((const unsigned char*)m1.src + (o1 + (unsigned)m1.sr * 2u));
       }
@@ -103,7 +116,7 @@
 #pragma unroll
     for (int u = 0; u < U; ++u) {
       const int i = base + u * nthr + tid;
-      if (i >= NP) continue;
+      if (i >= np) continue;
       stage_write<DH, NR, ROWS0, TRANS0>(m0, i, a0[u], b0[u]);
       stage_write<DH, NR, ROWS1, TRANS1>(m1, i, a1[u], b1[u]);
     }
diff --git a/vit-lens_amd/csrc/vl_attn_fwd_body.inc b/vit-lens_amd/csrc/vl_attn_fwd_body.inc
--- /dev/null
+++ b/vit-lens_amd/csrc/vl_attn_fwd_body.inc
@@ -0,0 +1,301 @@
+  constexpr int RB = DH * 2;
+  constexpr int CH = RB / 16;
+  constexpr int RSH = Rsh<DH>::v;
+  constexpr bool PAD = DH == 128;
+  constexpr int KS = DH / 16;
+  constexpr int DT = DH / 32;
+  extern __shared__ __attribute__((aligned(16))) unsigned char smem[];
+  unsigned char* sK = smem;
+  bf16_t* sV = (bf16_t*)(smem + KC * RB);
+  float* sP = (float*)(sV + DH * VSP);
+  float* sPart = sP + NWMAX * 32;
+  bf16_t* sTailQ = (bf16_t*)(sPart + (KC / 32) * (2 + DH));
+
+  const int b = blockIdx.z, h = blockIdx.y;
+  const int tid = threadIdx.x, nthr = blockDim.x;
+  const int lane = tid & 63;
+  const int wid = __builtin_amdgcn_readfirstlane(tid >> 6);
+  const int nwq = nthr >> 6;
+  const int fr = lane & 31, fg = lane >> 5;
+  const size_t bh = (size_t)b * p.H + h;
+  const bf16_t* Kg = p.k.p + b * p.k.sb + h * p.k.sh;
+  const bf16_t* Vg = p.v.p + b * p.v.sb + h * p.v.sh;
+  const bf16_t* Qb = p.q.p + b * p.q.sb + h * p.q.sh;
+
+  const int q0 = (blockIdx.x * nwq + wid) * 32;
+  const bool wave_active = q0 < p.lq_main;
+  int qrow = q0 + fr; if (qrow >= p.lq_main) qrow = p.lq_main - 1;
+  const int qidx = q0 + fr;
+  const int dhr = PAD ? p.dh : DH;
+  const int nch = dhr >> 3;
+
+  VL_PROF_STAMP(p, 0);
+  u32x4 qraw[KS];
+  {
+    const bf16_t* Qg = Qb + (long)qrow * p.q.sr;
+#pragma unroll
+    for (int ks = 0; ks < KS; ++ks) {
+      qraw[ks] = u32x4{0u, 0u, 0u, 0u};
+      if (!PAD || ks * 2 + fg < nch) qraw[ks] = *(const u32x4*)(Qg + ks * 16 + fg * 8);
+    }
+  }
+  [[maybe_unused]] u32x4 tailraw = {0u, 0u, 0u, 0u};
+  if constexpr (TAILQ) {
+    if constexpr (!PAD) tailraw = *(const u32x4*)(Qb + (long)(p.Lq - 1) * p.q.sr + (tid & (CH - 1)) * 8);
+    else if (tid < nch) tailraw = *(const u32x4*)(Qb + (long)(p.Lq - 1) * p.q.sr + tid * 8);
+  }
+  unsigned char* const sVr = (unsigned char*)sV;
+  auto vswz = [](int row) { const int x = (row >> 1) & 7; return ((x & 1) << 2) | (x >> 1); };
+  if constexpr (DMA) {
+    typedef __attribute__((address_space(3))) void* lds_p;
+    const int nrows = ((p.Lk + 31) >> 5) << 5;
+    const __amdgpu_buffer_rsrc_t rsK = __builtin_amdgcn_make_buffer_rsrc((void*)Kg, 0, 0x7ffffff0, 0x00020000);
+    const __amdgpu_buffer_rsrc_t rsV = __builtin_amdgcn_make_buffer_rsrc((void*)Vg, 0, 0x7ffffff0, 0x00020000);
+    for (int u = wid; u * 8 < p.Lk; u += nwq) {
+      const int row = u * 8 + (lane >> 3), sl = lane & 7;
+      if (row < p.Lk) {
+        const unsigned offK = (unsigned)(row * (int)p.k.sr + ((sl ^ ((row >> 1) & 7)) << 3)) * 2u;
+        const unsigned offV = (unsigned)(row * (int)p.v.sr + ((sl ^ vswz(row)) << 3)) * 2u;
+        __builtin_amdgcn_raw_ptr_buffer_load_lds(rsK, (lds_p)(sK + u * 1024), 16, offK, 0, 0, 0);
+        __builtin_amdgcn_raw_ptr_buffer_load_lds(rsV, (lds_p)(sVr + u * 1024), 16, offV, 0, 0, 0);
+      }
+    }
+    for (int i = tid; i < (nrows - p.Lk) * 8; i += nthr)
+      *(u32x4*)(sVr + (p.Lk + (i >> 3)) * 128 + ((i & 7) << 4)) = u32x4{0u, 0u, 0u, 0u};
+    asm volatile("s_waitcnt vmcnt(0)" ::: "memory");
+  } else {
+  if constexpr (VARLEN)
+    stage2<DH, KC, true, false, false, true, 3, true>(StageSrc{sK, nullptr, Kg, p.k.sr, 1.f, nch}, StageSrc{nullptr, sV, Vg, p.v.sr, 1.f, nch},
+                                                      0, p.Lk, tid, nthr, ((p.Lk + 31) >> 5) * 16 * CH);
+  else
+  stage2<DH, KC, true, false, false, true>(StageSrc{sK, nullptr, Kg, p.k.sr, 1.f, nch}, StageSrc{nullptr, sV, Vg, p.v.sr, 1.f, nch},
+                                           0, p.Lk, tid, nthr);
+  }
+  if constexpr (TAILQ) {
+    if constexpr (!PAD) *(u32x4*)(sTailQ + (tid & (CH - 1)) * 8) = tailraw;
+    else if (tid < CH) *(u32x4*)(sTailQ + tid * 8) = tailraw;
+  }
+  VL_PROF_STAMP(p, 1);
+  [[maybe_unused]] const int li = lane & 15, lb3 = (li >> 3) & 1;
+  [[maybe_unused]] const unsigned aTr = (unsigned)((fg * 4 + (li >> 2)) * 128) +
+                                        (((unsigned)(((lane >> 4) & 1) * 2 + ((li >> 1) & 1)) ^ (unsigned)((lb3 << 2) | fg)) << 4) + (unsigned)((li & 1) << 3);
+  auto trV = [&](int tile, int c, int t) {
+    typedef __attribute__((ext_vector_type(4))) short s16x4;
+    typedef __attribute__((address_space(3))) s16x4* lds_s16x4;
+    struct { s16x4 lo, hi; } f;
+    const unsigned a = (aTr + (unsigned)(tile * 4096)) ^ (unsigned)(t * 64);
+    f.lo = __builtin_amdgcn_ds_read_tr16_b64_v4i16((lds_s16x4)(sVr + a + c * 2048));
+    f.hi = __builtin_amdgcn_ds_read_tr16_b64_v4i16((lds_s16x4)(sVr + (a ^ 32u) + c * 2048 + 1024));
+    return __builtin_bit_cast(bf16x8, f);
+  };
+  bf16x8 qf[KS];
+#pragma unroll
+  for (int ks = 0; ks < KS; ++ks)
+    qf[ks] = __builtin_bit_cast(bf16x8, p.qscale != 1.0f ? scale_x8<F16>(qraw[ks], p.qscale) : qraw[ks]);
+
+  float m_run = 0.f;
+  vl_f32x2 l2 = {0.f, 0.f};
+  f32x16 negm;
+  f32x16 o[DT];
+#pragma unroll
+  for (int r = 0; r < 16; ++r) negm[r] = 0.f;
+#pragma unroll
+  for (int t = 0; t < DT; ++t)
+#pragma unroll
+    for (int r = 0; r < 16; ++r) o[t][r] = 0.f;
+  bool first = true;
+
+  auto tail_partials = [&]() {
+    if constexpr (TAILQ) {
+    const int qT = p.Lq - 1;
+    const int ntile = (p.Lk + 31) >> 5;
+    const int ksw = (fr >> RSH) & (CH - 1);
+    bf16x8 qa[KS];
+#pragma unroll
+    for (int ks = 0; ks < KS; ++ks) {
+#pragma unroll
+      for (int e = 0; e < 8; ++e) qa[ks][e] = (__bf16)0.f;
+      if (fr == 0) {
+        u32x4 raw = *(const u32x4*)(sTailQ + ks * 16 + fg * 8);
+        if (p.qscale != 1.0f) raw = scale_bf16x8(raw, p.qscale);
+        qa[ks] = __builtin_bit_cast(bf16x8, raw);
+      }
+    }
+    for (int kt = wid; kt < ntile; kt += nwq) {
+      f32x16 st;
+#pragma unroll
+      for (int r = 0; r < 16; ++r) st[r] = 0.f;
+      const unsigned char* kbase = sK + (kt * 32 + fr) * RB;
+#pragma unroll
+      for (int ks = 0; ks < KS; ++ks)
+        st = __builtin_amdgcn_mfma_f32_32x32x16_bf16(qa[ks], *(const bf16x8*)(kbase + (((ks * 2 + fg) ^ ksw) * 16)), st, 0, 0, 0);
+      const bool valid = fg == 0 && kt * 32 + fr < p.Lk;
+      const float sv = valid ? st[0] : -INFINITY;
+      const float mw = wave_max_dpp(sv);
+      const float pw = valid ? __builtin_amdgcn_exp2f(sv - mw) : 0.f;
+      const float lw = wave_sum_dpp(pw);
+      float* myP = sP + wid * 32;
+      if (fg == 0) myP[fr] = pw;
+      __builtin_amdgcn_fence(__ATOMIC_RELEASE, "wavefront");
+      __builtin_amdgcn_wave_barrier();
+      __builtin_amdgcn_fence(__ATOMIC_ACQUIRE, "wavefront");
+      f32x16 ot[DT];
+#pragma unroll
+      for (int t = 0; t < DT; ++t)
+#pragma unroll
+        for (int r = 0; r < 16; ++r) ot[t][r] = 0.f;
+#pragma unroll
+      for (int c = 0; c < 2; ++c) {
+        bf16x8 pa;
+#pragma unroll
+        for (int e = 0; e < 8; ++e) pa[e] = (__bf16)0.f;
+        if (fr == 0) {
+          const f32x4 lo = *(const f32x4*)(myP + c * 16 + fg * 4);
+          const f32x4 hi = *(const f32x4*)(myP + c * 16 + 8 + fg * 4);
+#pragma unroll
+          for (int e = 0; e < 4; ++e) { pa[e] = (__bf16)lo[e]; pa[4 + e] = (__bf16)hi[e]; }
+        }
+#pragma unroll
+        for (int t = 0; t < DT; ++t)
+          ot[t] = __builtin_amdgcn_mfma_f32_32x32x16_bf16(
+              pa, DMA ? trV(kt, c, t) : *(const bf16x8*)(sV + (t * 32 + fr) * VSP + kt * 32 + c * 16 + fg * 8), ot[t], 0, 0, 0);
+      }
+      __builtin_amdgcn_wave_barrier();
+      float* part = sPart + kt * (2 + DH);
+      if (lane == 0) { part[0] = mw; part[1] = lw; }
+      if (fg == 0) {
+#pragma unroll
+        for (int t = 0; t < DT; ++t) part[2 + t * 32 + fr] = ot[t][0];
+      }
+    }
+    }
+  };
+  auto tail_merge = [&]() {
+    if constexpr (TAILQ) {
+      const int qT = p.Lq - 1;
+      const int ntile = (p.Lk + 31) >> 5;
+      if (wid == 0) {
+        float M = -INFINITY;
+        for (int kt = 0; kt < ntile; ++kt) M = fmaxf(M, sPart[kt * (2 + DH)]);
+        for (int d = lane; d < dhr; d += 64) {
+          float L = 0.f, acc = 0.f;
+          for (int kt = 0; kt < ntile; ++kt) {
+            const float* part = sPart + kt * (2 + DH);
+            const float w = __builtin_amdgcn_exp2f(part[0] - M);
+            L = fmaf(part[1], w, L);
+            acc = fmaf(part[2 + d], w, acc);
+          }
+          p.out[((size_t)b * p.Lq + qT) * (p.H * dhr) + h * dhr + d] = f2bf(acc / L);
+          if (p.lse && d == 0) p.lse[bh * p.Lq + qT] = (M + __log2f(L)) * 0.6931471805599453f;
+        }
+      }
+    }
+  };
+  const int q_hi = q0 + 31;
+  const int blk_q_hi = min(p.lq_main - 1, (int)(blockIdx.x * nwq + nwq) * 32 - 1);
+
+  for (int kc0 = 0; kc0 < (MULTI ? p.Lk : 1); kc0 += KC) {
+    if (MULTI && p.causal && kc0 > blk_q_hi) break;
+    if constexpr (MULTI) {
+      if (kc0 > 0) {
+        __syncthreads();
+        stage2<DH, KC, true, false, false, true, 1>(StageSrc{sK, nullptr, Kg, p.k.sr, 1.f, nch},
+                                                    StageSrc{nullptr, sV, Vg, p.v.sr, 1.f, nch}, kc0, p.Lk, tid, nthr);
+      }
+    }
+    __syncthreads();
+    VL_PROF_STAMP(p, 2);
+    if constexpr (TAILQ) { tail_partials(); __syncthreads(); }
+    if (!wave_active) continue;
+
+    int ntile = (min(p.Lk - kc0, KC) + 31) >> 5;
+    if (p.causal) ntile = min(ntile, ((q_hi - kc0) >> 5) + 1);
+    const int ksw = (fr >> RSH) & (CH - 1);
+    for (int kt = 0; kt < ntile; ++kt) {
+      const unsigned char* kbase = sK + (kt * 32 + fr) * RB;
+      bf16x8 kf[KS];
+#pragma unroll
+      for (int ks = 0; ks < KS; ++ks) kf[ks] = *(const bf16x8*)(kbase + (((ks * 2 + fg) ^ ksw) * 16));
+      f32x16 s = mfma32<F16>(kf[0], qf[0], negm);
+#pragma unroll
+      for (int ks = 1; ks < KS; ++ks) s = mfma32<F16>(kf[ks], qf[ks], s);
+      bf16x8 vf0[DT];
+#pragma unroll
+      for (int t = 0; t < DT; ++t) {
+        if constexpr (DMA) vf0[t] = trV(kt, 0, t);
+        else vf0[t] = *(const bf16x8*)(sV + (t * 32 + fr) * VSP + kt * 32 + fg * 8);
+      }
+      const int key0 = kc0 + kt * 32 + fg * 4;
+      const bool need_mask = (key0 - fg * 4 + 32 > p.Lk) || (p.causal && key0 - fg * 4 + 31 > q0);
+      if (need_mask) {
+#pragma unroll
+        for (int r = 0; r < 16; ++r) {
+          const int key = key0 + (r & 3) + 8 * (r >> 2);
+          if (key >= p.Lk || (p.causal && key > qidx)) s[r] = -INFINITY;
+        }
+      }
+      float mx = fmaxf(fmaxf(s[0], s[1]), s[2]);
+#pragma unroll
+      for (int r = 3; r < 15; r += 2) mx = fmaxf(fmaxf(mx, s[r]), s[r + 1]);
+      mx = fmaxf(mx, s[15]);
+      mx = xhalf_max(mx);
+      if (__builtin_amdgcn_ballot_w64(first || mx > RESCALE_THR) != 0) {
+        const float d = first ? mx : fmaxf(mx, 0.f);
+        const float alpha = first ? 0.f : __builtin_amdgcn_exp2f(-d);
+        m_run += d;
+#pragma unroll
+        for (int r = 0; r < 16; ++r) { s[r] -= d; negm[r] -= d; }
+#pragma unroll
+        for (int t = 0; t < DT; ++t)
+#pragma unroll
+          for (int r = 0; r < 16; ++r) o[t][r] *= alpha;
+        l2 *= alpha;
+        first = false;
+      }
+      float pv[16];
+#pragma unroll
+      for (int r = 0; r < 16; ++r) pv[r] = __builtin_amdgcn_exp2f(s[r]);
+      {
+        vl_f32x2 a0 = {pv[0], pv[1]}, a1 = {pv[2], pv[3]}, a2 = {pv[4], pv[5]}, a3 = {pv[6], pv[7]};
+        const vl_f32x2 a4 = {pv[8], pv[9]}, a5 = {pv[10], pv[11]}, a6 = {pv[12], pv[13]}, a7 = {pv[14], pv[15]};
+        a0 += a4; a1 += a5; a2 += a6; a3 += a7;
+        a0 += a2; a1 += a3;
+        l2 += a0 + a1;
+      }
+      bf16x8 vf1[DT];
+#pragma unroll
+      for (int t = 0; t < DT; ++t) {
+        if constexpr (DMA) vf1[t] = trV(kt, 1, t);
+        else vf1[t] = *(const bf16x8*)(sV + (t * 32 + fr) * VSP + kt * 32 + 16 + fg * 8);
+      }
+      {
+        const bf16x8 pf = pack8x<F16>(pv);
+#pragma unroll
+        for (int t = 0; t < DT; ++t) o[t] = mfma32<F16>(vf0[t], pf, o[t]);
+      }
+      {
+        const bf16x8 pf = pack8x<F16>(pv + 8);
+#pragma unroll
+        for (int t = 0; t < DT; ++t) o[t] = mfma32<F16>(vf1[t], pf, o[t]);
+      }
+    }
+  }
+
+  VL_PROF_STAMP(p, 3);
+  if (wave_active) {
+    const float l_tot = xhalf_sum(l2[0] + l2[1]);
+    const float inv = 1.0f / l_tot;
+    if constexpr (VARLEN) {
+      store_rows_t<DT, F16>(o, inv, p.out + ((size_t)row0 + qrow) * (p.H * dhr) + h * dhr, fg, qidx < p.lq_main, nch);
+      if (p.lse && fg == 0 && qidx < p.lq_main)
+        p.lse[((size_t)row0 + qidx) * p.H + h] = (m_run + __log2f(l_tot)) * 0.6931471805599453f;
+    } else {
+    store_rows_t<DT, F16>(o, inv, p.out + ((size_t)b * p.Lq + qrow) * (p.H * dhr) + h * dhr, fg, qidx < p.lq_main, nch);
+    if (p.lse && fg == 0 && qidx < p.lq_main)
+      p.lse[bh * p.Lq + qidx] = (m_run + __log2f(l_tot)) * 0.6931471805599453f;
+    }
+  }
+
+  VL_PROF_STAMP(p, 4);
+  tail_merge();
+  VL_PROF_STAMP(p, 5);
diff --git a/vit-lens_amd/csrc/vl_text_pack.hip b/vit-lens_amd/csrc/vl_text_pack.hip
--- /dev/null
+++ b/vit-lens_amd/csrc/vl_text_pack.hip
@@ -0,0 +1,100 @@
+#include "vl_common.h"
+#include "vitlens_hip.h"
+
+namespace {
+
+__global__ void __launch_bounds__(256) text_len_kernel(const int64_t* ids, int* len, int B, int L) {
+  const int lane = threadIdx.x & 63;
+  const int b = blockIdx.x * 4 + (threadIdx.x >> 6);
+  if (b >= B) return;
+  const int64_t* row = ids + (long)b * L;
+  long long best = 0; int at = L;
+  for (int t = lane; t < L; t += 64) {
+    const long long v = row[t];
+    if (at == L || v > best) { best = v; at = t; }
+  }
+#pragma unroll
+  for (int o = 32; o > 0; o >>= 1) {
+    const long long ob = __shfl_xor(best, o, 64);
+    const int oa = __shfl_xor(at, o, 64);
+    if (oa < L && (at == L || ob > best || (ob == best && oa < at))) { best = ob; at = oa; }
+  }
+  if (lane == 0) len[b] = at + 1;
+}
+
+constexpr int SCAN_T = 1024;
+__global__ void __launch_bounds__(SCAN_T) text_scan_kernel(const int* len, int* start, int64_t* last_row, int* total, int B) {
+  __shared__ int s_sum[SCAN_T];
+  __shared__ int s_max[SCAN_T];
+  const int tid = threadIdx.x;
+  const int per = (B + SCAN_T - 1) / SCAN_T;
+  const int b0 = min(tid * per, B), b1 = min(b0 + per, B);
+  int sum = 0, mx = 0;
+  for (int b = b0; b < b1; ++b) { const int n = len[b]; sum += n; mx = max(mx, n); }
+  s_sum[tid] = sum; s_max[tid] = mx;
+  __syncthreads();
+  for (int o = 1; o < SCAN_T; o <<= 1) {
+    const int a = tid >= o ? s_sum[tid - o] : 0, m = tid >= o ? s_max[tid - o] : 0;
+    __syncthreads();
+    s_sum[tid] += a; s_max[tid] = max(s_max[tid], m);
+    __syncthreads();
+  }
+  int run = s_sum[tid] - sum;
+  for (int b = b0; b < b1; ++b) {
+    const int n = len[b];
+    start[b] = run; last_row[b] = (int64_t)(run + n - 1);
+    run += n;
+  }
+  if (tid == SCAN_T - 1) { start[B] = s_sum[tid]; total[0] = s_sum[tid]; total[1] = s_max[tid]; }
+}
+
+__global__ void __launch_bounds__(256) text_embed_packed_kernel(const int64_t* ids, const int* start, const int* len,
+                                                                const float* emb, const float* pos, float* out, int B, int L,
+                                                                int D, int vocab, int rows, int rows_pad) {
+  const int lane = threadIdx.x & 63;
+  const long w = (long)blockIdx.x * 4 + (threadIdx.x >> 6);
+  const long dense = (long)B * L;
+  if (w >= dense) {
+    const long r = rows + (w - dense);
+    if (r >= rows_pad) return;
+    for (int i = lane; i < D; i += 64) out[r * D + i] = 0.f;
+    return;
+  }
+  const int b = (int)(w / L), t = (int)(w - (long)b * L);
+  if (t >= len[b]) return;
+  const long r = (long)start[b] + t;
+  if (r >= rows) return;
+  long id = ids[w]; id = id < 0 ? 0 : (id >= vocab ? vocab - 1 : id);
+  const float* e = emb + id * D;
+  const float* ps = pos + (long)t * D;
+  for (int i = lane; i < D; i += 64) out[r * D + i] = e[i] + ps[i];
+}
+
+}
+
+extern "C" int vl_set_error(const char* msg);
+#define VL_HIP_OK(e) do { hipError_t _e = (e); if (_e != hipSuccess) return vl_set_error(hipGetErrorString(_e)); } while (0)
+
+extern "C" int vl_text_pack_plan(const int64_t* ids, int* len, int* start, int64_t* last_row, int* total, int B, int L,
+                                 hipStream_t stream) {
+  if (B <= 0 || L <= 0) return vl_set_error("vl_text_pack_plan: empty problem");
+  if ((long)B * L >= (1L << 31)) return vl_set_error("vl_text_pack_plan: B*L must stay below 2^31");
+  if (!ids || !len || !start || !last_row || !total) return vl_set_error("vl_text_pack_plan: null argument");
+  hipLaunchKernelGGL(text_len_kernel, dim3((B + 3) / 4), dim3(256), 0, stream, ids, len, B, L);
+  hipLaunchKernelGGL(text_scan_kernel, dim3(1), dim3(SCAN_T), 0, stream, (const int*)len, start, last_row, total, B);
+  VL_HIP_OK(hipGetLastError());
+  return 0;
+}
+
+extern "C" int vl_text_embed_packed(const int64_t* ids, const int* start, const int* len, const float* tok_emb, const float* pos,
+                                    float* out, int B, int L, int D, int vocab, int rows, int rows_pad, hipStream_t stream) {
+  if (B <= 0 || L <= 0 || D <= 0) return vl_set_error("vl_text_embed_packed: empty problem");
+  if ((long)B * L >= (1L << 31)) return vl_set_error("vl_text_embed_packed: B*L must stay below 2^31");
+  if (!ids || !start || !len || !tok_emb || !pos || !out) return vl_set_error("vl_text_embed_packed: null argument");
+  if (rows < B || rows > (long)B * L || rows_pad < rows) return vl_set_error("vl_text_embed_packed: need B <= rows <= B*L and rows_pad >= rows");
+  const long waves = (long)B * L + (rows_pad - rows);
+  hipLaunchKernelGGL(text_embed_packed_kernel, dim3((unsigned)((waves + 3) / 4)), dim3(256), 0, stream, ids, start, len, tok_emb, pos,
+                     out, B, L, D, vocab, rows, rows_pad);
+  VL_HIP_OK(hipGetLastError());
+  return 0;
+}
diff --git a/vit-lens_amd/vitlens_hip/_lib.py b/vit-lens_amd/vitlens_hip/_lib.py
--- a/vit-lens_amd/vitlens_hip/_lib.py
+++ b/vit-lens_amd/vitlens_hip/_lib.py
@@ -15,7 +15,7 @@
 
 P, I, L, F = C.c_void_p, C.c_int, C.c_long, C.c_float
 
-ABI_VERSION = 607
+ABI_VERSION = 608
 
 SIGNATURES = {
     "vl_version": [],
@@ -33,6 +33,9 @@
     "vl_group_max_f32": [P, L, P, L, L, I, I, P],
     "vl_pad3_f32": [P, P, L, I, P],
     "vl_attn_fwd_f16": [P, P, P, P, P, P, I, I, I, I, I, F, I, P],
+    "vl_text_pack_plan": [P, P, P, P, P, I, I, P],
+    "vl_text_embed_packed": [P, P, P, P, P, P, I, I, I, I, I, I, P],
+    "vl_attn_fwd_varlen_f16": [P, P, P, P, P, P, P, P, I, I, I, I, F, P],
     "vl_layernorm_fwd": [P, I, L, P, L, P, P, P, I, L, P, P, I, I, F, P],
     "vl_gemm_main_rows": [I, I],
     "vl_gemm_lnfold_bf16": [P, P, P, P, P, P, P, P, I, I, I, I, I, I, I, P],
diff --git a/vit-lens_amd/vitlens_hip/engine.py b/vit-lens_amd/vitlens_hip/engine.py
--- a/vit-lens_amd/vitlens_hip/engine.py
+++ b/vit-lens_amd/vitlens_hip/engine.py
@@ -280,6 +280,36 @@
         return ops.l2_normalize(f) if normalize else f
 
 
+PACK_TEXT = True
+
+
+def text_pack_mode(arith: str, text: torch.Tensor, device) -> str:
+    if not PACK_TEXT or arith != "f16" or torch.device(device).type != "cuda":
+        return "dense"
+    if torch.cuda.is_current_stream_capturing():
+        return "dense"
+    return "device" if text.is_cuda else "host"
+
+
+def text_pack_plan_host(text: torch.Tensor):
+    lens = text.argmax(dim=-1).to(torch.int64) + 1
+    start = torch.zeros(text.shape[0] + 1, dtype=torch.int64, device=text.device)
+    start[1:] = torch.cumsum(lens, 0)
+    last_row = start[:-1] + lens - 1
+    return lens.to(torch.int32), start.to(torch.int32), last_row, (int(start[-1]), int(lens.max()))
+
+
+@dataclass
+class TextPlan:
+    B: int
+    L: int
+    rows: int
+    max_len: int
+    lens: torch.Tensor
+    start: torch.Tensor
+    last_row: torch.Tensor
+
+
 def prep_block_f16(sd: Dict[str, torch.Tensor], p: str, device) -> Dict[str, torch.Tensor]:
     hf = torch.float16
     return {
@@ -306,6 +336,7 @@
         hv = lambda i: ops.heads_view(self.qkv, B, L, H, dh, i * D)
         self.q, self.k, self.v = hv(0), hv(1), hv(2)
         self.pooled = z(self.Bp, D)
+        self.f = None
 
 
 class TextEngine:
@@ -364,12 +395,88 @@
         ops.gemm_f16(ws.pooled, self.projT, None, out=f, res=f, epi=ops.EPI_RES_F32)
         return f[:B]
 
-    def encode_text(self, text: torch.Tensor, normalize: bool = False) -> torch.Tensor:
+    def plan_text(self, text: torch.Tensor) -> Optional[TextPlan]:
+        mode = text_pack_mode(self.arith, text, self.device)
+        if mode == "dense":
+            return None
+        B, L = text.shape
+        if mode == "host":
+            lens, start, last_row, (rows, max_len) = text_pack_plan_host(text.detach().long())
+            dv = lambda t: t.to(self.device)
+            return TextPlan(B, L, rows, max_len, dv(lens), dv(start), dv(last_row))
+        return self._plan_on_device(text, B, L)
+
+    def _plan_on_device(self, text, B, L) -> TextPlan:
+        dev = self.device
+        text = text.detach().to(dev, torch.int64).contiguous()
+        with torch.cuda.device(dev):
+            if getattr(self, "_plan_stream", None) is None:
+                self._plan_stream = torch.cuda.Stream(device=dev)
+                self._plan_pin = torch.empty(2, dtype=torch.int32).pin_memory()
+            cur = torch.cuda.current_stream(dev)
+            i32 = lambda n: torch.empty(n, device=dev, dtype=torch.int32)
+            lens, start, total = i32(B), i32(B + 1), i32(2)
+            last_row = torch.empty(B, device=dev, dtype=torch.int64)
+            asked = torch.cuda.Event()
+            asked.record(cur)
+            side = self._plan_stream
+            side.wait_event(asked)
+            with torch.cuda.stream(side):
+                ops.text_pack_plan(text, lens, start, last_row, total)
+                self._plan_pin.copy_(total, non_blocking=True)
+            side.synchronize()
+            rows, max_len = int(self._plan_pin[0]), int(self._plan_pin[1])
+        return TextPlan(B, L, rows, max_len, lens, start, last_row)
+
+    def _encode_f16_packed(self, text: torch.Tensor, plan: TextPlan) -> torch.Tensor:
+        cfg = self.cfg
+        B, L = text.shape
+        D, H = cfg.width, cfg.heads
+        if (plan.B, plan.L) != (B, L) or not (B <= plan.rows <= B * L) or not (1 <= plan.max_len <= L):
+            raise ValueError(f"encode_text: the plan was made for another batch ({plan.B} x {plan.L}, {plan.rows} rows, "
+                             f"longest {plan.max_len}; text {B} x {L})")
+        key = ("f16", B, L)
+        if key not in self._ws:
+            self._ws[key] = _WorkspaceF16(B, L, D, H, self.device)
+        ws = self._ws[key]
+        E = self.projT.shape[0]
+        if ws.f is None:
+            ws.f = torch.empty(ws.Bp, E, device=self.device, dtype=torch.float32)
+        cur = torch.cuda.current_stream(self.device)
+        for t in (plan.lens, plan.start, plan.last_row):
+            t.record_stream(cur)
+        rows = plan.rows
+        Mr = (rows + 255) // 256 * 256
+        x, h, qkv, a, hid = ws.x[:Mr], ws.h[:Mr], ws.qkv[:Mr], ws.a[:Mr], ws.hid[:Mr]
+        ops.text_embed_packed(text, plan.start, plan.lens, self.tok, self.pos, ws.x, rows, Mr)
+        qs = (D // H) ** -0.5 * ops.LOG2E
+        act = ops.mlp_act(cfg.quick_gelu)
+        for w in self.blocks:
+            ops.layernorm(x, w["ln1_w"], w["ln1_b"], h, rows, D)
+            ops.gemm_f16(h, w["in_w"], w["in_b"], out=qkv)
+            ops.attn_fwd_varlen(qkv, plan.start, plan.lens, a, H, plan.max_len, qscale=qs)
+            ops.gemm_f16(a, w["out_w"], w["out_b"], out=x, res=x, epi=ops.EPI_RES_F32)
+            ops.layernorm(x, w["ln2_w"], w["ln2_b"], h, rows, D)
+            ops.gemm_f16(h, w["fc_w"], w["fc_b"], out=hid, act=act)
+            ops.gemm_f16(hid, w["proj_w"], w["proj_b"], out=x, res=x, epi=ops.EPI_RES_F32)
+        ops.layernorm(ws.x, self.ln_final[0], self.ln_final[1], ws.pooled, B, D, x_row_stride=D, row_index=plan.last_row, row_mul=0)
+        ws.f.zero_()
+        ops.gemm_f16(ws.pooled, self.projT, None, out=ws.f, res=ws.f, epi=ops.EPI_RES_F32)
+        return ws.f[:B]
+
+    def encode_text(self, text: torch.Tensor, normalize: bool = False, plan=None) -> torch.Tensor:
         cfg = self.cfg
         B, L = text.shape
         D = cfg.width
+        if plan is False:
+            plan = None
+        elif self.arith == "f16" and plan is None:
+            plan = self.plan_text(text)
         text = text.to(self.device).contiguous()
         if self.arith == "f16":
+            if plan is not None and text_pack_mode(self.arith, text, self.device) != "dense":
+                f = self._encode_f16_packed(text if text.dtype == torch.int64 else text.long(), plan)
+                return ops.l2_normalize(f) if normalize else f.clone()
             f = self._encode_f16(text)
             return ops.l2_normalize(f) if normalize else f.contiguous()
         key = (B, L)
diff --git a/vit-lens_amd/vitlens_hip/ops.py b/vit-lens_amd/vitlens_hip/ops.py
--- a/vit-lens_amd/vitlens_hip/ops.py
+++ b/vit-lens_amd/vitlens_hip/ops.py
@@ -374,6 +374,55 @@
     return out
 
 
+def attn_fwd_varlen(qkv, start, lens, out, H, max_len, lse=None, qscale=1.0):
+    import ctypes
+    W = H * 64
+    if qkv.dtype != torch.float16 or out.dtype != torch.float16 or qkv.dim() != 2 or qkv.shape[1] != 3 * W or qkv.stride(1) != 1:
+        raise ValueError("attn_fwd_varlen: qkv must be an fp16 [rows, 3*H*64] matrix with unit column stride, out fp16")
+    if out.dim() != 2 or out.shape[1] != W or not out.is_contiguous() or out.shape[0] < qkv.shape[0]:
+        raise ValueError("attn_fwd_varlen: out must be a contiguous fp16 [rows, H*64] matrix")
+    for t, nm in ((start, "start"), (lens, "lens")):
+        if t.dtype != torch.int32 or not t.is_contiguous() or t.device != qkv.device:
+            raise ValueError(f"attn_fwd_varlen: {nm} must be a contiguous int32 tensor on the operands' device")
+    B = lens.numel()
+    if start.numel() < B + 1:
+        raise ValueError("attn_fwd_varlen: start needs B + 1 entries")
+    if lse is not None and (lse.dtype != torch.float32 or not lse.is_contiguous() or lse.numel() < qkv.shape[0] * H):
+        raise ValueError("attn_fwd_varlen: lse must be a contiguous f32 [rows, H]")
+    ld = qkv.stride(0)
+    st = (ctypes.c_long * 6)(64, ld, 64, ld, 64, ld)
+    es = qkv.element_size()
+    base = qkv.data_ptr()
+    check(_lib.vl_attn_fwd_varlen_f16(base, base + W * es, base + 2 * W * es, st, _p(start), _p(lens), _p(out), _p(lse), B, H,
+                                      int(max_len), 64, float(qscale), _stream()))
+    return out
+
+
+def text_pack_plan(ids, lens, start, last_row, total):
+    B, L = ids.shape
+    if ids.dtype != torch.int64 or not ids.is_contiguous():
+        raise ValueError("text_pack_plan: ids must be a contiguous int64 [B, L] tensor")
+    for t, dt, n, nm in ((lens, torch.int32, B, "lens"), (start, torch.int32, B + 1, "start"), (last_row, torch.int64, B, "last_row"),
+                         (total, torch.int32, 2, "total")):
+        if t.dtype != dt or not t.is_contiguous() or t.numel() < n or t.device != ids.device:
+            raise ValueError(f"text_pack_plan: {nm} must be a contiguous {dt} tensor of >= {n} entries on the ids' device")
+    check(_lib.vl_text_pack_plan(_p(ids), _p(lens), _p(start), _p(last_row), _p(total), B, L, _stream()))
+
+
+def text_embed_packed(ids, start, lens, tok_emb, pos, out, rows, rows_pad):
+    B, L = ids.shape
+    D = tok_emb.shape[1]
+    if ids.dtype != torch.int64 or not ids.is_contiguous() or out.dtype != torch.float32 or not out.is_contiguous():
+        raise ValueError("text_embed_packed: ids contiguous int64 [B, L], out contiguous f32")
+    if out.dim() != 2 or out.shape[1] != D or out.shape[0] < rows_pad or pos.shape[0] < L or pos.shape[1] != D:
+        raise ValueError("text_embed_packed: out must hold rows_pad rows of the embedding width, pos L rows")
+    if start.dtype != torch.int32 or lens.dtype != torch.int32 or start.numel() < B + 1 or lens.numel() < B:
+        raise ValueError("text_embed_packed: start int32 [B+1], lens int32 [B]")
+    check(_lib.vl_text_embed_packed(_p(ids), _p(start), _p(lens), _p(tok_emb), _p(pos), _p(out), B, L, D, tok_emb.shape[0],
+                                    int(rows), int(rows_pad), _stream()))
+    return out
+
+
 def _q1_rows(t, H, name):
     if t.dim() != 2 or t.stride(1) != 1 or t.dtype != torch.bfloat16 or t.shape[1] != H * 64:
         raise ValueError(f"{name}: need a bf16 [B, H*64] matrix with unit column stride, got {tuple(t.shape)} {t.dtype}")
diff --git a/vit-lens_amd/vitlens_hip/step.py b/vit-lens_amd/vitlens_hip/step.py
--- a/vit-lens_amd/vitlens_hip/step.py
+++ b/vit-lens_amd/vitlens_hip/step.py
@@ -192,6 +192,19 @@
     @property
     def _overlap_active(self) -> bool:
         return self.overlap_frozen and self.dev.type == "cuda"
+
+    pack_text = True
+
+    def _text_plan(self, texts):
+        plan_text = getattr(self.text, "plan_text", None)
+        if plan_text is None or not self.pack_text:
+            return None
+        return plan_text(texts)
+
+    def _encode_text(self, texts, plan):
+        if not hasattr(self.text, "plan_text"):
+            return self.text.encode_text(texts)
+        return self.text.encode_text(texts, plan=plan if plan is not None else False)
 
     def _side_by_side(self, beside, here):
         frozen, trainable = beside, here
@@ -530,6 +543,7 @@
             self._reduced_upto = l
 
     def forward_backward(self, images: torch.Tensor, texts: torch.Tensor, depths: torch.Tensor) -> torch.Tensor:
+        tplan = self._text_plan(texts)
         B = images.shape[0]
         mb = min(self.mb, B)
         assert B % mb == 0, "per-GPU batch must be a multiple of the micro-batch"
@@ -547,7 +561,7 @@
         fv = torch.empty(B, E, device=self.dev); vraw = torch.empty(B, E, device=self.dev)
         vnorm = torch.empty(B, device=self.dev)
         def frozen():
-            ops.l2_normalize(self.text.encode_text(texts), out=ft)
+            ops.l2_normalize(self._encode_text(texts, tplan), out=ft)
             for i in range(nmb):
                 s = slice(i * mb, (i + 1) * mb)
                 ops.l2_normalize(self.image.encode_image(images[s]), out=fi[s])
@@ -791,13 +805,14 @@
         ops.cast_bf16(self.masters["visual.visual_adapter.conv1.weight_gemm"], out=self.lens.conv_w)
 
     def forward_backward(self, audio: torch.Tensor, texts: torch.Tensor) -> torch.Tensor:
+        tplan = self._text_plan(texts)
         B = audio.shape[0]
         mb, nmb = self._prepare(B)
         E = self.lens.tower.embed_dim
         ft = torch.empty(B, E, device=self.dev); fv = torch.empty(B, E, device=self.dev)
         vraw = torch.empty(B, E, device=self.dev); vnorm = torch.empty(B, device=self.dev)
         def frozen():
-            ops.l2_normalize(self.text.encode_text(texts), out=ft)
+            ops.l2_normalize(self._encode_text(texts, tplan), out=ft)
 
         def trainable():
             for i in range(nmb):
@@ -870,7 +885,10 @@
         for t in self.trainers:
             t.tok.op = self.tok.op
 
+    pack_text = False
+
     def forward_backward(self, images, texts, points, fps_start=None) -> torch.Tensor:
+        tplan = self._text_plan(texts)
         B = images.shape[0]
         mb, nmb = self._prepare(B)
         E = self.image.cfg.embed_dim
@@ -878,7 +896,7 @@
         fv = torch.empty(B, E, device=self.dev); vraw = torch.empty(B, E, device=self.dev)
         vnorm = torch.empty(B, device=self.dev)
         def frozen():
-            ops.l2_normalize(self.text.encode_text(texts), out=ft)
+            ops.l2_normalize(self._encode_text(texts, tplan), out=ft)
             for i in range(nmb):
                 s = slice(i * mb, (i + 1) * mb)
                 ops.l2_normalize(self.image.encode_image(images[s]), out=fi[s])
```
